# jannerm/ddpo

Hardware: AMD Instinct MI355X
Metric: sampled images/sec (512^2, 50 DDIM steps) (higher is better)
Workload: dtype f32 (f16mx: f16 MFMA + MX-fp8 cross terms on the long-reduction conv/GEMM layers, bf16x3-split MFMA elsewhere); 1 GPU; BASELINE configs[1]: compressed-animals geometry, sd15 U-Net+VAE (random init), 512x512, 50 DDIM steps, CFG 5.0, eta 1.0, sample_batch_size 8/GPU, VAE decode included; parallelism=dp1, global_batch=8

## Files before the change

### ddpo_amd/csrc/common.h

```cpp
#pragma once
#include <hip/hip_runtime.h>
#include <stdint.h>
#include "../../include/ddpo_hip.h"

#define DDPO_LAUNCH_CHECK()                                   \
  do {                                                        \
    hipError_t e__ = hipGetLastError();                       \
    if (e__ != hipSuccess) return DDPO_ELAUNCH;               \
  } while (0)

__device__ __forceinline__ float wave_sum(float v) {
#pragma unroll
  for (int o = 32; o > 0; o >>= 1) v += __shfl_xor(v, o, 64);
  return v;
}
__device__ __forceinline__ uint32_t lane_xor1_u32(uint32_t x) { return __shfl_xor(x, 1, 64); }
__device__ __forceinline__ double wave_sum_d(double v) {
#pragma unroll
  for (int o = 32; o > 0; o >>= 1) v += __shfl_xor(v, o, 64);
  return v;
}
__device__ __forceinline__ float wave_max(float v) {
#pragma unroll
  for (int o = 32; o > 0; o >>= 1) v = fmaxf(v, __shfl_xor(v, o, 64));
// ... 13 lines not shown

__device__ __forceinline__ float silu_f(float x) { return x / (1.f + __expf(-x)); }

__device__ __forceinline__ float sigmoid_2u_fast(float u) { return __builtin_amdgcn_rcpf(1.0f + __builtin_amdgcn_exp2f(-2.8853900817779268f * u)); }
__device__ __forceinline__ float gelu_tanh_f(float x) {
  const float k0 = 0.7978845608028654f, k1 = 0.044715f;
  float u = k0 * (x + k1 * x * x * x);
  return x * sigmoid_2u_fast(u);
}

__device__ __forceinline__ uint32_t cvt_pk_bf16(float lo, float hi) {
  uint32_t r;
  asm("v_cvt_pk_bf16_f32 %0, %1, %2" : "=v"(r) : "v"(lo), "v"(hi));
  return r;
}

__device__ __forceinline__ void split4(const float4 v, uint2& hi, uint2& lo) {
  hi.x = cvt_pk_bf16(v.x, v.y);
  hi.y = cvt_pk_bf16(v.z, v.w);
  const float r0 = v.x - __uint_as_float(hi.x << 16), r1 = v.y - __uint_as_float(hi.x & 0xFFFF0000u);
  const float r2 = v.z - __uint_as_float(hi.y << 16), r3 = v.w - __uint_as_float(hi.y & 0xFFFF0000u);
  lo.x = cvt_pk_bf16(r0, r1);
  lo.y = cvt_pk_bf16(r2, r3);
}

__host__ __device__ __forceinline__ int64_t plane_off(int64_t row, int c, int ld, int64_t rows) {
  return ld ? row * ld + c : ((int64_t)(c >> 5) * rows + row) * 32 + (c & 31);
}

typedef _Float16 mx_half2 __attribute__((ext_vector_type(2)));
__device__ __forceinline__ void mx_split4(const float4 v, uint2& h16, uint32_t& h8, uint32_t& l8) {
  const float lim = 65504.f, lim8 = 57344.f;
  const float vx = fminf(fmaxf(v.x, -lim), lim), vy = fminf(fmaxf(v.y, -lim), lim), vz = fminf(fmaxf(v.z, -lim), lim), vw = fminf(fmaxf(v.w, -lim), lim);
  const _Float16 a = (_Float16)vx, b = (_Float16)vy, c = (_Float16)vz, e = (_Float16)vw;
  h16.x = __builtin_bit_cast(uint32_t, mx_half2{a, b});
  h16.y = __builtin_bit_cast(uint32_t, mx_half2{c, e});
  const float ha = (float)a, hb = (float)b, hc = (float)c, he = (float)e;
  int p = __builtin_amdgcn_cvt_pk_bf8_f32(fminf(fmaxf(ha, -lim8), lim8), fminf(fmaxf(hb, -lim8), lim8), 0, false);
  h8 = (uint32_t)__builtin_amdgcn_cvt_pk_bf8_f32(fminf(fmaxf(hc, -lim8), lim8), fminf(fmaxf(he, -lim8), lim8), p, true);
  p = __builtin_amdgcn_cvt_pk_bf8_f32((vx - ha) * 2048.f, (vy - hb) * 2048.f, 0, false);
  l8 = (uint32_t)__builtin_amdgcn_cvt_pk_bf8_f32((vz - hc) * 2048.f, (vw - he) * 2048.f, p, true);
}
__device__ __forceinline__ void mx_store4(uint16_t* __restrict__ p16, uint16_t* __restrict__ p8, int64_t row, int c, int ld, int64_t rows,
                                          const float4 v) {
  uint2 h16;
  uint32_t h8, l8;
  mx_split4(v, h16, h8, l8);
  *reinterpret_cast<uint2*>(p16 + plane_off(row, c, ld, rows)) = h16;
  char* b = reinterpret_cast<char*>(p8 + plane_off(row, c & ~31, ld, rows)) + 2 * (c & 16) + (c & 15);
  *reinterpret_cast<uint32_t*>(b) = h8;
  *reinterpret_cast<uint32_t*>(b + 16) = l8;
}

static inline hipStream_t as_stream(void* s) { return reinterpret_cast<hipStream_t>(s); }
```

### ddpo_amd/csrc/gemm_bf16.hip

```cpp
#include "gemm_bf16_common.h"
#include <cstdlib>
#include <type_traits>

#ifdef DDPO_KLOOP_TIMING
__device__ unsigned long long ddpo_dbg_t[2 * 16384 * 8];
#define DBG_T(i)                                                                                      \
  do {                                                                                                \
    if (threadIdx.x == 0) {                                                                           \
      const int w_ = (blockIdx.x + gridDim.x * blockIdx.y) & 16383;                                   \
      ddpo_dbg_t[w_ * 8 + (i)] = __builtin_amdgcn_s_memtime();                                        \
      ddpo_dbg_t[w_ * 8 + 4 + (i)] = __builtin_amdgcn_s_memrealtime();                                \
    }                                                                                                 \
  } while (0)
#define DBG_ABL(bit) ((d.splits >> 4) & (bit))
#define DBG_WDECL unsigned long long dbg_w0_ = 0, dbg_wacc_ = 0, dbg_bacc_ = 0
#define DBG_W0() do { dbg_w0_ = __builtin_amdgcn_s_memtime(); } while (0)
#define DBG_WMID() do { const unsigned long long n_ = __builtin_amdgcn_s_memtime(); dbg_wacc_ += n_ - dbg_w0_; dbg_w0_ = n_; } while (0)
#define DBG_W1() do { dbg_bacc_ += __builtin_amdgcn_s_memtime() - dbg_w0_; } while (0)
#define DBG_WSTORE()                                                                 \
  do {                                                                               \
    if (threadIdx.x == 0) {                                                          \
      const int w_ = (blockIdx.x + gridDim.x * blockIdx.y) & 16383;                  \
      ddpo_dbg_t[(16384 + w_) * 8 + 0] = dbg_wacc_;                                  \
      ddpo_dbg_t[(16384 + w_) * 8 + 1] = dbg_bacc_;                                  \
// ... 105 lines not shown
      const int rowc = min(row_base + rr, d.M - 1) % d.res_rows, colc = min(col_base + (e - rr * LPR) * 4, d.N - 4);
      ex[i] = *reinterpret_cast<const float4*>(d.residual + (int64_t)rowc * d.ld_res + colc);
    }
  }
  __device__ __forceinline__ void combine(const ddpo_gemm_desc& d, float* cw, int b0, int row_base, int col_base, int lane) {
    const bool both = d.residual && d.rowbias;
    asm volatile("" : "+v"(lane));
#pragma unroll
    for (int i = 0; i < NB; ++i) {
      const int it = b0 + i;
      const int e = it * 64 + lane, rr = e / LPR, lcol = (e - rr * LPR) * 4;
      float4 v = *reinterpret_cast<const float4*>(cw + rr * WTN + lcol);
      const float4 b4 = bv[it % PER];
      v.x = d.alpha * v.x + b4.x; v.y = d.alpha * v.y + b4.y; v.z = d.alpha * v.z + b4.z; v.w = d.alpha * v.w + b4.w;
      if (both) {
        const int rowc = min(row_base + rr, d.M - 1), colc = min(col_base + lcol, d.N - 4);
        const float4 rb = *reinterpret_cast<const float4*>(d.rowbias + (int64_t)(rowc / d.rows_per_batch) * d.ld_rowbias + colc);
        v.x += rb.x; v.y += rb.y; v.z += rb.z; v.w += rb.w;
      }
      if (d.residual || d.rowbias) { v.x += ex[i].x; v.y += ex[i].y; v.z += ex[i].z; v.w += ex[i].w; }
      *reinterpret_cast<float4*>(cw + rr * WTN + lcol) = v;
    }
  }
  __device__ __forceinline__ void combine_all(const ddpo_gemm_desc& d, float* cw, int row_base, int col_base, int lane) {
    if (!any) return;
#pragma unroll
    for (int b0 = 0; b0 < NIT; b0 += NB) {
      if (b0) fetch(d, b0, row_base, col_base, lane);
      combine(d, cw, b0, row_base, col_base, lane);
    }
  }
  template <bool FOLD = false>
  __device__ __forceinline__ static void emit(const ddpo_gemm_desc& d, const float* cw, int row_base, int col_base, int lane, int ph = 0) {
#pragma unroll
    for (int b0 = 0; b0 < NIT; b0 += LB) {
      asm volatile("" : "+v"(lane));
      float4 v[LB];
#pragma unroll
      for (int i = 0; i < LB; ++i) {
        const int e = (b0 + i) * 64 + lane, rr = e / LPR;
        v[i] = *reinterpret_cast<const float4*>(cw + rr * WTN + (e - rr * LPR) * 4);
      }
#pragma unroll
      for (int i = 0; i < LB; ++i) {
        const int e = (b0 + i) * 64 + lane, rr = e / LPR;
        const int row = row_base + rr, col = col_base + (e - rr * LPR) * 4;
        if (row >= d.M || col >= d.N) continue;
        if constexpr (FOLD) { st_out4(d.out + fold_row(d, row, ph) * d.ld_out + col, v[i]); continue; }
        if (d.out) st_out4(d.out + (int64_t)row * d.ld_out + col, v[i]);
        if (d.out_hi) store_planes4(d, row, col, v[i]);
      }
    }
  }
  __device__ __forceinline__ static void partials(const ddpo_gemm_desc& d, const float* cw, float* pp, int row_base, int col_base, int lane) {
#pragma unroll
    for (int it = 0; it < NIT; ++it) {
      const int e = it * 64 + lane, rr = e / LPR, lcol = (e - rr * LPR) * 4;
      const int row = row_base + rr, col = col_base + lcol;
      if (row >= d.M || col >= d.N) continue;
      *reinterpret_cast<float4*>(pp + (int64_t)row * d.N + col) = *reinterpret_cast<const float4*>(cw + rr * WTN + lcol);
    }
  }
};

template <int BM, int BN, Datapath DP, bool AFFINE>
__global__ void __launch_bounds__(BF_THREADS) gemm_conv_bf16_kernel(const ddpo_gemm_desc d, const uint16_t* __restrict__ w_hi,
                                                                   const uint16_t* __restrict__ w_lo, int ldw, int tiles_m,
                                                                   int tiles_n, int nblk, int kt_per_split,
                                                                   float* __restrict__ part) {
  constexpr int BK = BF_BK;
  constexpr int TM = BM / 64, TN = BN / 64;
  constexpr int AROWS = BM / 32;
  constexpr int BCH = BN / 64;
  constexpr int NPL = (DP == Datapath::bf16x3) ? 2 : 1;
  constexpr int A_BYTES = BM * 64, B_BYTES = BN * 64;
  extern __shared__ __attribute__((aligned(16))) char smem[];
  constexpr int STAGE = NPL * (A_BYTES + B_BYTES);
  const int t = threadIdx.x, lane = t & 63, wid = t >> 6;
  const int wm = wid >> 1, wn = wid & 1;

  int bid = blockIdx.x;
  {
    const int xcd = bid & 7, idx = bid >> 3;
    const int q = nblk >> 3, r = nblk & 7;
    bid = (xcd < r ? xcd * (q + 1) : r * (q + 1) + (xcd - r) * q) + idx;
  }
  constexpr int GROUP_M = 8;
  const int per_group = GROUP_M * tiles_n;
  const int group = bid / per_group, in_group = bid - group * per_group;
  const int gm0 = group * GROUP_M;
  const int gsz = min(tiles_m - gm0, GROUP_M);
  const int tile_n = in_group / gsz, tile_m = gm0 + (in_group - tile_n * gsz);
  const int m0 = tile_m * BM, n0 = tile_n * BN;

  const bool conv = d.ksize > 0;
  const int VH = d.upsample ? d.H * 2 : d.H, VW = d.upsample ? d.W * 2 : d.W;
  const bool zins = d.upsample == 2;

  const int kq = t & 7;
  const float* arow_ptr[AROWS];
  uint32_t amask[AROWS];
  int aiy0[AROWS], aix0[AROWS];
  int64_t abase[AROWS];
#pragma unroll
  for (int i = 0; i < AROWS; ++i) {
    const int m = m0 + (t >> 3) + 32 * i;
    const bool valid = m < d.M;
    amask[i] = 0;
    if (conv) {
      const int ohw = d.OH * d.OW;
      const int mm = valid ? m : 0;
      const int b = mm / ohw, rem = mm - b * ohw;
      const int oy = rem / d.OW, ox = rem - oy * d.OW;
      const int iy0 = oy * d.stride - d.pad, ix0 = ox * d.stride - d.pad;
      abase[i] = (int64_t)b * d.H * d.W;
      aiy0[i] = iy0; aix0[i] = ix0;
// ... 159 lines not shown
  store_tile(0, s0);
  load_tile(1, s0);
  __syncthreads();
  const int nk2 = (nk + 1) & ~1;
#pragma unroll 1
  for (int kt = 0; kt < nk2; kt += 2) {
    load_tile(kt + 2, s1);
    compute(0);
    store_tile(1, s0);
    __syncthreads();
    load_tile(kt + 3, s0);
    compute(1);
    store_tile(0, s1);
    __syncthreads();
  }

  if (part) {
    float* pp = part + (int64_t)blockIdx.y * d.M * d.N;
#pragma unroll
    for (int i = 0; i < TM; ++i)
#pragma unroll
      for (int j = 0; j < TN; ++j) {
        const int col = n0 + wn * (BN / 2) + j * 32 + (lane & 31);
        if (col >= d.N) continue;
#pragma unroll
        for (int r = 0; r < 16; ++r) {
          const int row = m0 + wm * (BM / 2) + i * 32 + (r & 3) + 8 * (r >> 2) + 4 * khalf;
          if (row < d.M) pp[(int64_t)row * d.N + col] = acc[i][j][r];
        }
      }
    return;
  }
#pragma unroll
  for (int i = 0; i < TM; ++i) {
#pragma unroll
    for (int j = 0; j < TN; ++j) {
      const int col = n0 + wn * (BN / 2) + j * 32 + (lane & 31);
      if (col >= d.N) continue;
      const float bv = d.bias ? d.bias[col] : 0.f;
#pragma unroll
      for (int r = 0; r < 16; ++r) {
        const int row = m0 + wm * (BM / 2) + i * 32 + (r & 3) + 8 * (r >> 2) + 4 * khalf;
        if (row >= d.M) continue;
        float v = d.alpha * acc[i][j][r] + bv;
        if (d.rowbias) v += d.rowbias[(int64_t)(row / d.rows_per_batch) * d.ld_rowbias + col];
        if (d.residual) v += d.residual[(int64_t)res_row(d, row) * d.ld_res + col];
        d.out[(int64_t)row * d.ld_out + col] = v;
      }
    }
  }
}

template <int BM, int BN, Datapath DP, int WM = 2, int WN = 2, KLoop KL = KLoop::regs, bool FOLD = false>
__global__ void __launch_bounds__(64 * WM * WN, (BM * BN <= 128 * 64 ? 3 : 1)) gemm_conv_bf16_buf_kernel(const ddpo_gemm_desc d, const uint16_t* __restrict__ w_hi_,
                                                                       const uint16_t* __restrict__ w_lo_, int ldw, int tiles_m,
                                                                       int tiles_n, int nblk, int kt_per_split,
                                                                       float* __restrict__ part) {
  constexpr int BK = BF_BK;
  constexpr int THREADS = 64 * WM * WN;
  constexpr int WTM = BM / WM, WTN = BN / WN;
  constexpr int TM = WTM / 32, TN = WTN / 32;
  constexpr int AR = THREADS / 8, BR = THREADS / 4;
  constexpr int AROWS = BM / AR;
  constexpr int BCH = (BN + BR - 1) / BR;
  constexpr bool BFULL = (BN % BR) == 0;
  static_assert(BM % AR == 0 && WTM % 32 == 0 && WTN % 32 == 0, "tile / wave-grid mismatch");
  constexpr bool MX = DP == Datapath::f16mx;
  static_assert(!MX || KL == KLoop::planes3w || KL == KLoop::tall_mx, "the f16mx datapath exists on the plane-fed 128-row tiles and on the tall tile");
  static_assert(!FOLD || (KL != KLoop::regs && KL != KLoop::tall_geglu), "folded up-sampler phases exist on the plane-fed kernels");
  const int ph = FOLD ? (int)blockIdx.z : 0;
  const uint16_t* __restrict__ w_hi = FOLD ? w_hi_ + (int64_t)ph * d.K * d.N : w_hi_;
  const uint16_t* __restrict__ w_lo = (FOLD && w_lo_) ? w_lo_ + (int64_t)ph * d.K * d.N : w_lo_;
  constexpr int NPL = (DP == Datapath::bf16x3 || DP == Datapath::f16mx) ? 2 : 1;
  constexpr int A_BYTES = BM * 64, B_BYTES = BN * 64;
  extern __shared__ __attribute__((aligned(16))) char smem[];
  constexpr int STAGE = NPL * (A_BYTES + B_BYTES);
  const int t = threadIdx.x, lane = t & 63, wid = t >> 6;
  const int wm = wid / WN, wn = wid % WN;
  DBG_T(0);
  DBG_WDECL;

  int bid = blockIdx.x;
  {
    const int xcd = bid & 7, idx = bid >> 3;
    const int q = nblk >> 3, r = nblk & 7;
    bid = (xcd < r ? xcd * (q + 1) : r * (q + 1) + (xcd - r) * q) + idx;
  }
  constexpr int GROUP_M = 8;
  const int per_group = GROUP_M * tiles_n;
  const int group = bid / per_group, in_group = bid - group * per_group;
  const int gm0 = group * GROUP_M;
  const int gsz = min(tiles_m - gm0, GROUP_M);
  const int tile_n = in_group / gsz, tile_m = gm0 + (in_group - tile_n * gsz);
  const int m0 = tile_m * BM, n0 = tile_n * BN;

  const bool conv = d.ksize > 0;
  const int VH = (!FOLD && d.upsample) ? d.H * 2 : d.H, VW = (!FOLD && d.upsample) ? d.W * 2 : d.W;
  const bool zins = !FOLD && d.upsample == 2;
  const int cin = conv ? d.Cin : d.K;
  const int ntaps = conv ? d.ksize * d.ksize : 1;

  f32x16 acc[TM][TN];
#pragma unroll
  for (int i = 0; i < TM; ++i)
#pragma unroll
    for (int j = 0; j < TN; ++j)
#pragma unroll
// ... 569 lines not shown
      constexpr int LPR = WTN / 4;
      constexpr int NIT = 32 * LPR / 64;
      static_assert((32 * LPR) % 64 == 0, "32-row pass must be a whole number of wave instructions");
      __syncthreads();
      float* cw = reinterpret_cast<float*>(smem) + wid * (32 * WTN);
      float* pp = part ? part + ((int64_t)ph * gridDim.y + blockIdx.y) * d.M * d.N : nullptr;
      using Epi = EpiRows<NIT, LPR, WTN, 5>;
      Epi ep;
      const int colb = n0 + wn * WTN;
      static_assert(TM == 2, "the tall tile's output stage is written for two 32-row passes per wave");
      if constexpr (KL == KLoop::tall_geglu) {
        static_assert(WN == 2 && WTN == 160, "value / gate wave pairs of 160 columns");
        const int oc0 = (n0 / 320) * 160;
        float bj[TN];
#pragma unroll
        for (int j = 0; j < TN; ++j) bj[j] = d.bias ? d.bias[colb + j * 32 + (lane & 31)] : 0.f;
        const float* ca = reinterpret_cast<const float*>(smem) + (wid & ~1) * (32 * WTN);
        const float* cg = ca + 32 * WTN;
        auto gpass = [&](auto IH) {
          constexpr int ih = decltype(IH)::value;
          if (ih > 0) __syncthreads();
#pragma unroll
          for (int j = 0; j < TN; ++j)
#pragma unroll
            for (int r = 0; r < 16; ++r) {
              cw[((r & 3) + 8 * (r >> 2) + 4 * khalf) * WTN + j * 32 + (lane & 31)] = acc[ih][j][r] + bj[j];
            }
          __syncthreads();
          constexpr int GL = WTN / 4;
          int ln = lane;
          asm volatile("" : "+v"(ln));
#pragma unroll
          for (int it = 0; it < 16 * GL / 64; ++it) {
            const int e = it * 64 + ln, rr = wn * 16 + e / GL, c4 = (e - (e / GL) * GL) * 4;
            const float4 a = *reinterpret_cast<const float4*>(ca + rr * WTN + c4);
            const float4 g = *reinterpret_cast<const float4*>(cg + rr * WTN + c4);
            const float4 o = make_float4(a.x * gelu_tanh_f(g.x), a.y * gelu_tanh_f(g.y), a.z * gelu_tanh_f(g.z), a.w * gelu_tanh_f(g.w));
            const int row = m0 + wm * WTM + ih * 32 + rr, col = oc0 + c4;
            if (row >= d.M) continue;
            if (d.aux_out) {
              float* pa = d.aux_out + (int64_t)row * d.N + col;
              *reinterpret_cast<float4*>(pa) = a;
              *reinterpret_cast<float4*>(pa + (d.N >> 1)) = g;
            }
            if (d.out) st_out4(d.out + (int64_t)row * d.ld_out + col, o);
            if (d.out_hi) store_planes4(d, row, col, o);
          }
        };
        gpass(std::integral_constant<int, 0>{});
        gpass(std::integral_constant<int, 1>{});
        DBG_T(3);
        return;
      }
      auto pass = [&](auto IH) {
        constexpr int ih = decltype(IH)::value;
        const int rowb = m0 + wm * WTM + ih * 32;
        if (ih > 0 && !pp) ep.fetch(d, 0, rowb, colb, lane);
#pragma unroll
        for (int j = 0; j < TN; ++j)
#pragma unroll
          for (int r = 0; r < 16; ++r)
            cw[((r & 3) + 8 * (r >> 2) + 4 * khalf) * WTN + j * 32 + (lane & 31)] = acc[ih][j][r];
        if (pp) {
          Epi::partials(d, cw, pp, rowb, colb, lane);
        } else {
          if (ih == 0) { ep.init(d, colb, lane); ep.fetch(d, 0, rowb, colb, lane); }
          ep.combine_all(d, cw, rowb, colb, lane);
          Epi::template emit<FOLD>(d, cw, rowb, colb, lane, ph);
        }
      };
      pass(std::integral_constant<int, 0>{});
      pass(std::integral_constant<int, 1>{});
      DBG_T(3);
      return;
    }
  }
  if (vec_ok && BM != 256) {
    constexpr int LPR = WTN / 4;
    constexpr int NIT = WTM * LPR / 64;
    static_assert((WTM * LPR) % 64 == 0, "wave sub-tile must be a whole number of 1 KiB rows");
    __syncthreads();
    float* cw = reinterpret_cast<float*>(smem) + wid * (WTM * WTN);
    using Epi = EpiRows<NIT, LPR, WTN>;
    Epi ep;
    const int rowb = m0 + wm * WTM, colb = n0 + wn * WTN;
    const bool plain = !part && !(BN == 128 && WN == 2 && WM == 2 && d.epilogue == 1);
    if (plain) { ep.init(d, colb, lane); ep.fetch(d, 0, rowb, colb, lane); }
#pragma unroll
    for (int i = 0; i < TM; ++i)
#pragma unroll
      for (int j = 0; j < TN; ++j)
#pragma unroll
        for (int r = 0; r < 16; ++r)
          cw[(i * 32 + (r & 3) + 8 * (r >> 2) + 4 * khalf) * WTN + j * 32 + (lane & 31)] = acc[i][j][r];
    if (BN == 128 && WN == 2 && WM == 2 && d.epilogue == 1) {
      const int q = (n0 + wn * 64) >> 6;
      const int gc = (lane & 7) * 4, grow = lane >> 3;
      const float4 ba = d.bias ? *reinterpret_cast<const float4*>(d.bias + q * 64 + gc) : make_float4(0.f, 0.f, 0.f, 0.f);
      const float4 bg = d.bias ? *reinterpret_cast<const float4*>(d.bias + q * 64 + 32 + gc) : make_float4(0.f, 0.f, 0.f, 0.f);
#pragma unroll
      for (int it = 0; it < 8; ++it) {
        const int rr = it * 8 + grow;
        const int row = m0 + wm * 64 + rr;
        if (row >= d.M) continue;
        const float4 a = *reinterpret_cast<const float4*>(cw + rr * 64 + gc);
        const float4 g = *reinterpret_cast<const float4*>(cw + rr * 64 + 32 + gc);
        float4 o;
        o.x = (a.x + ba.x) * gelu_tanh_f(g.x + bg.x); o.y = (a.y + ba.y) * gelu_tanh_f(g.y + bg.y);
        o.z = (a.z + ba.z) * gelu_tanh_f(g.z + bg.z); o.w = (a.w + ba.w) * gelu_tanh_f(g.w + bg.w);
        if (d.aux_out) {
          float* pa = d.aux_out + (int64_t)row * d.N + q * 32 + gc;
          *reinterpret_cast<float4*>(pa) = make_float4(a.x + ba.x, a.y + ba.y, a.z + ba.z, a.w + ba.w);
          *reinterpret_cast<float4*>(pa + (d.N >> 1)) = make_float4(g.x + bg.x, g.y + bg.y, g.z + bg.z, g.w + bg.w);
        }
        if (d.out) st_out4(d.out + (int64_t)row * d.ld_out + q * 32 + gc, o);
        if (d.out_hi) store_planes4(d, row, q * 32 + gc, o);
      }
      DBG_T(3);
      return;
    }
    if (part) {
      Epi::partials(d, cw, part + ((int64_t)ph * gridDim.y + blockIdx.y) * d.M * d.N, rowb, colb, lane);
    } else {
      ep.combine_all(d, cw, rowb, colb, lane);
      Epi::template emit<FOLD>(d, cw, rowb, colb, lane, ph);
    }
    DBG_T(3);
    return;
  }
  if (part) {
    float* pp = part + ((int64_t)ph * gridDim.y + blockIdx.y) * d.M * d.N;
#pragma unroll
    for (int i = 0; i < TM; ++i)
#pragma unroll
      for (int j = 0; j < TN; ++j) {
        const int col = n0 + wn * WTN + j * 32 + (lane & 31);
        if (col >= d.N) continue;
#pragma unroll
        for (int r = 0; r < 16; ++r) {
          const int row = m0 + wm * WTM + i * 32 + (r & 3) + 8 * (r >> 2) + 4 * khalf;
          if (row < d.M) pp[(int64_t)row * d.N + col] = acc[i][j][r];
        }
      }
    DBG_T(3);
    return;
  }
#pragma unroll
  for (int i = 0; i < TM; ++i) {
#pragma unroll
    for (int j = 0; j < TN; ++j) {
      const int col = n0 + wn * WTN + j * 32 + (lane & 31);
      if (col >= d.N) continue;
      const float bv = d.bias ? d.bias[col] : 0.f;
#pragma unroll
      for (int r = 0; r < 16; ++r) {
        const int row = m0 + wm * WTM + i * 32 + (r & 3) + 8 * (r >> 2) + 4 * khalf;
        if (row >= d.M) continue;
        float v = d.alpha * acc[i][j][r] + bv;
        if (d.rowbias) v += d.rowbias[(int64_t)(row / d.rows_per_batch) * d.ld_rowbias + col];
        if (d.residual) v += d.residual[(int64_t)res_row(d, row) * d.ld_res + col];
        d.out[(FOLD ? fold_row(d, row, ph) : (int64_t)row) * d.ld_out + col] = v;
      }
    }
  }
  DBG_T(3);
}

__global__ void __launch_bounds__(256) splitk_reduce_kernel(const ddpo_gemm_desc d, const float* __restrict__ part, int splits) {
  const int n4 = d.N >> 2;
  const int64_t total = (int64_t)d.M * n4, mn = (int64_t)d.M * d.N;
  const bool fold = d.upsample == 3;
  const int ph = blockIdx.y;
  part += (int64_t)ph * splits * mn;
  for (int64_t i = (int64_t)blockIdx.x * blockDim.x + threadIdx.x; i < total; i += (int64_t)gridDim.x * blockDim.x) {
    const int row = (int)(i / n4), col = (int)(i - (int64_t)row * n4) << 2;
    float4 a = *reinterpret_cast<const float4*>(part + (int64_t)row * d.N + col);
    for (int s = 1; s < splits; ++s) {
      const float4 b = *reinterpret_cast<const float4*>(part + s * mn + (int64_t)row * d.N + col);
      a.x += b.x; a.y += b.y; a.z += b.z; a.w += b.w;
    }
    float v[4] = {a.x, a.y, a.z, a.w};
    const int rrow = res_row(d, row);
#pragma unroll
    for (int e = 0; e < 4; ++e) {
      float x = d.alpha * v[e] + (d.bias ? d.bias[col + e] : 0.f);
      if (d.rowbias) x += d.rowbias[(int64_t)(row / d.rows_per_batch) * d.ld_rowbias + col + e];
      if (d.residual) x += d.residual[(int64_t)rrow * d.ld_res + col + e];
      v[e] = x;
      if (d.out) d.out[(fold ? fold_row(d, row, ph) : (int64_t)row) * d.ld_out + col + e] = x;
    }
    if (d.out_hi) store_planes4(d, row, col, make_float4(v[0], v[1], v[2], v[3]));
  }
}

constexpr int SPLITK_MIN_KTILES_128 = 32;
constexpr int SPLITK_MIN_KTILES_WIDE = 16;
extern "C" int ddpo_gemm_splitk_min_ktiles(void) { return SPLITK_MIN_KTILES_WIDE < SPLITK_MIN_KTILES_128 ? SPLITK_MIN_KTILES_WIDE : SPLITK_MIN_KTILES_128; }

static bool res_rows_ok(const ddpo_gemm_desc& d) {
  return d.res_rows == 0 || (d.res_rows > 0 && d.residual && d.M > 0 && d.M % d.res_rows == 0);
}

static bool planes_out_ok(const ddpo_gemm_desc& d) {
  if (!d.out_hi) return d.out != nullptr && !d.out_lo;
  if (!d.out_lo || d.ld_planes < 0 || (d.ld_planes & 3)) return false;
  if ((reinterpret_cast<uintptr_t>(d.out_hi) | reinterpret_cast<uintptr_t>(d.out_lo)) & 7) return false;
  const int ncols = d.epilogue != 0 ? d.N / 2 : d.N;
  if (d.ld_planes == 0 ? (ncols & 31) != 0 : d.ld_planes < ncols) return false;
  if (d.planes_fmt != 0 && (d.planes_fmt != 1 || (ncols & 31) || (d.ld_planes & 31))) return false;
  if (d.N & 3) return false;
  if (d.out && ((d.ld_out & 3) || (reinterpret_cast<uintptr_t>(d.out) & 15))) return false;
  if (d.residual && ((d.ld_res & 3) || (reinterpret_cast<uintptr_t>(d.residual) & 15))) return false;
  if (d.rowbias && ((d.ld_rowbias & 3) || (reinterpret_cast<uintptr_t>(d.rowbias) & 15))) return false;
  if (d.bias && (reinterpret_cast<uintptr_t>(d.bias) & 15)) return false;
  return true;
}

enum { TC_TALL = 0, TC_WIDE = 1, TC_128 = 2, TC_64 = 3, TC_GENERIC = 4, TC_SPLITK_REDUCE = 5, TC_MX = 6, TC_COUNT = 8 };
static unsigned long long g_tile_launches[TC_COUNT] = {0, 0, 0, 0, 0, 0, 0, 0};
extern "C" int ddpo_gemm_tile_launch_counts(unsigned long long* out_host, int n) {
  if (!out_host || n < TC_COUNT) return DDPO_EINVAL;
  for (int i = 0; i < TC_COUNT; ++i) out_host[i] = __atomic_load_n(&g_tile_launches[i], __ATOMIC_RELAXED);
  return DDPO_OK;
}
static inline void count_tile(int cls) { __atomic_fetch_add(&g_tile_launches[cls], 1ull, __ATOMIC_RELAXED); }

static bool g_force_generic = false;
static bool buf_path_ok(const ddpo_gemm_desc& d, int ldw) {
  if (g_force_generic) return false;
  const int64_t lim = 0x7FFFFFFF;
  if (d.w_layout == 1) ldw = (d.K + 31) / 32 * 32;
  if (d.ksize > 0) {
    if (d.Cin % BF_BK) return false;
    if ((int64_t)d.B * d.H * d.W * (d.ld_src ? d.ld_src : d.Cin) * 4 >= lim) return false;
    const int64_t wbytes = d.w_dgrad ? (int64_t)d.K * d.N * 2 : (int64_t)d.N * ldw * 2;
    if (wbytes >= lim) return false;
  } else {
    if (d.K % BF_BK) return false;
    if ((int64_t)d.M * (d.ld_src ? d.ld_src : d.K) * 4 >= lim || (int64_t)d.N * ldw * 2 >= lim) return false;
  }
  return true;
}
#ifdef DDPO_DEBUG_HOOKS
extern "C" void ddpo_debug_force_generic_gemm(int on) { g_force_generic = on != 0; }
#endif

template <int BM_, int BN_, int WM_, int WN_, int TC_, size_t EPI_BYTES_, bool SPLITK_>
struct Tile {
  static constexpr int BM = BM_, BN = BN_, WM = WM_, WN = WN_, TC = TC_;
  static constexpr bool SPLITK = SPLITK_;
  static constexpr size_t lds_bytes(Datapath dp, KLoop kl) {
    const size_t npl = (dp == Datapath::bf16x3 || dp == Datapath::f16mx) ? 2 : 1;
    const size_t stages = kl == KLoop::planes3w ? npl * (2 * BM + 3 * BN) * 64 : 2 * npl * (BM + BN) * 64;
    return stages < EPI_BYTES_ ? EPI_BYTES_ : stages;
  }
};
using Tile128x128 = Tile<128, 128, 2, 2, TC_128, 128 * 128 * 4, true>;
using Tile128x64 = Tile<128, 64, 2, 2, TC_64, 128 * 64 * 4, true>;
using TileWide = Tile<128, 320, 4, 2, TC_WIDE, 128 * 320 * 4, true>;
using TileTall = Tile<256, 320, 4, 2, TC_TALL, 8 * 32 * 160 * 4, false>;

template <class T, Datapath DP, KLoop KL, bool FOLD>
constexpr bool kernel_exists() {
  if (FOLD && (DP == Datapath::f16x1 || KL == KLoop::regs || KL == KLoop::tall_geglu)) return false;
  if (T::BM == 256) {
    if (DP == Datapath::bf16x3) return KL == KLoop::tall || KL == KLoop::tall_geglu;
    return KL == (DP == Datapath::f16mx ? KLoop::tall_mx : KLoop::tall_ring);
  }
  return KL == KLoop::planes3w || (KL == KLoop::regs && (DP == Datapath::bf16x1 || DP == Datapath::bf16x3));
}

static int splits_128(const ddpo_gemm_desc& d, int ngrid, bool have_ws, size_t ws_bytes, int nph) {
  const int nk_total = (d.K + BF_BK - 1) / BF_BK;
  int splits = 1;
  if (have_ws && ngrid < 192 && nk_total >= SPLITK_MIN_KTILES_128 && (d.N & 3) == 0 && d.epilogue == 0) {
    splits = (384 + ngrid - 1) / ngrid;
    if (splits > 8) splits = 8;
    if (splits > nk_total / 8) splits = nk_total / 8;
    while (splits > 1 && (size_t)nph * splits * d.M * d.N * sizeof(float) > ws_bytes) --splits;
  }
  return splits;
}
static int wide_splits(const ddpo_gemm_desc& d, bool have_ws, size_t ws_bytes, int nph = 1) {
  const int nblk = nph * ((d.M + 127) / 128) * ((d.N + 319) / 320);
  const int nk_total = d.K / BF_BK;
  int splits = 1;
  if (have_ws && nblk <= 192 && nk_total >= SPLITK_MIN_KTILES_WIDE) {
    splits = (256 + nblk / 2) / nblk;
    if (splits > 8) splits = 8;
    if (splits > nk_total / 8) splits = nk_total / 8;
    if (splits < 1) splits = 1;
    while (splits > 1 && (size_t)nph * splits * d.M * d.N * sizeof(float) > ws_bytes) --splits;
  }
  return splits;
}
static int ktiles_per_split(int nk_total, int& splits) {
  int ktps = (nk_total + splits - 1) / splits;
  ktps = (ktps + 1) & ~1;
  splits = (nk_total + ktps - 1) / ktps;
  return ktps;
}

static int launch_splitk_reduce(const ddpo_gemm_desc& d, const float* part, int splits, int nph, hipStream_t st) {
  int64_t blocks = ((int64_t)d.M * (d.N >> 2) + 255) / 256;
  if (blocks > 4096) blocks = 4096;
  count_tile(TC_SPLITK_REDUCE);
  hipLaunchKernelGGL(splitk_reduce_kernel, dim3((int)blocks, nph), dim3(256), 0, st, d, part, splits);
  DDPO_LAUNCH_CHECK();
  return DDPO_OK;
}

template <class T, Datapath DP, KLoop KL, bool FOLD>
static int launch_tile(const ddpo_gemm_desc& d, const uint16_t* w_hi, const uint16_t* w_lo, int ldw, float* ws, int splits, hipStream_t st) {
  if constexpr (!kernel_exists<T, DP, KL, FOLD>()) {
    return DDPO_EINVAL;
  } else {
    constexpr int NPH = FOLD ? 4 : 1;
    constexpr bool GENERIC = KL == KLoop::regs && T::BN <= 128;
    constexpr size_t lds = T::lds_bytes(DP, KL);
    const auto kernel = &gemm_conv_bf16_buf_kernel<T::BM, T::BN, DP, T::WM, T::WN, KL, FOLD>;
    const int tiles_m = (d.M + T::BM - 1) / T::BM, tiles_n = (d.N + T::BN - 1) / T::BN;
    const int nblk = tiles_m * tiles_n;
    const int nk_total = (d.K + BF_BK - 1) / BF_BK;
    if (!T::SPLITK) splits = 1;
    const int ktps = T::SPLITK ? ktiles_per_split(nk_total, splits) : nk_total;
    float* part = splits > 1 ? ws : nullptr;
    static bool attr_set = false;
    if (!attr_set) {
      if constexpr (GENERIC) {
        (void)hipFuncSetAttribute(reinterpret_cast<const void*>(&gemm_conv_bf16_kernel<T::BM, T::BN, DP, true>), hipFuncAttributeMaxDynamicSharedMemorySize, (int)lds);
        (void)hipFuncSetAttribute(reinterpret_cast<const void*>(&gemm_conv_bf16_kernel<T::BM, T::BN, DP, false>), hipFuncAttributeMaxDynamicSharedMemorySize, (int)lds);
      }
      (void)hipFuncSetAttribute(reinterpret_cast<const void*>(kernel), hipFuncAttributeMaxDynamicSharedMemorySize, (int)lds);
      attr_set = true;
    }
    count_tile(T::TC);
    if constexpr (DP == Datapath::f16mx) count_tile(TC_MX);
    bool generic = false;
    if constexpr (GENERIC) generic = !buf_path_ok(d, ldw);
    if (!generic) {
      hipLaunchKernelGGL(kernel, dim3(nblk, splits, NPH), dim3(64 * T::WM * T::WN), lds, st, d, w_hi, w_lo, ldw, tiles_m, tiles_n, nblk, ktps, part);
    } else if constexpr (GENERIC) {
      count_tile(TC_GENERIC);
      if (d.upsample == 0)
        hipLaunchKernelGGL((gemm_conv_bf16_kernel<T::BM, T::BN, DP, true>), dim3(nblk, splits), dim3(BF_THREADS), lds, st, d, w_hi, w_lo, ldw, tiles_m, tiles_n, nblk, ktps, part);
      else
        hipLaunchKernelGGL((gemm_conv_bf16_kernel<T::BM, T::BN, DP, false>), dim3(nblk, splits), dim3(BF_THREADS), lds, st, d, w_hi, w_lo, ldw, tiles_m, tiles_n, nblk, ktps, part);
    }
    DDPO_LAUNCH_CHECK();
    return splits > 1 ? launch_splitk_reduce(d, part, splits, NPH, st) : DDPO_OK;
  }
}

enum RouteTile { RT_TALL, RT_TALL_GEGLU, RT_WIDE, RT_128, RT_64 };
struct Route { RouteTile tile; int splits; };

template <bool PLANES, bool FOLD, Datapath DP>
static int launch_route(const Route& r, const ddpo_gemm_desc& d, const uint16_t* w_hi, const uint16_t* w_lo, int ldw, float* ws, hipStream_t st) {
  constexpr KLoop KL = PLANES ? KLoop::planes3w : KLoop::regs;
  constexpr KLoop KT = !PLANES ? KLoop::regs : (DP == Datapath::bf16x3 ? KLoop::tall : (DP == Datapath::f16mx ? KLoop::tall_mx : KLoop::tall_ring));
  switch (r.tile) {
    case RT_TALL: return launch_tile<TileTall, DP, KT, FOLD>(d, w_hi, w_lo, ldw, ws, r.splits, st);
    case RT_TALL_GEGLU: return launch_tile<TileTall, DP, PLANES && DP == Datapath::bf16x3 ? KLoop::tall_geglu : KLoop::regs, FOLD>(d, w_hi, w_lo, ldw, ws, r.splits, st);
    case RT_WIDE: return launch_tile<TileWide, DP, KL, FOLD>(d, w_hi, w_lo, ldw, ws, r.splits, st);
    case RT_128: return launch_tile<Tile128x128, DP, KL, FOLD>(d, w_hi, w_lo, ldw, ws, r.splits, st);
    default: return launch_tile<Tile128x64, DP, KL, FOLD>(d, w_hi, w_lo, ldw, ws, r.splits, st);
  }
}
template <bool PLANES, bool FOLD>
static int launch_npass(int npass, const Route& r, const ddpo_gemm_desc& d, const uint16_t* w_hi, const uint16_t* w_lo, int ldw, float* ws, hipStream_t st) {
  switch (npass) {
    case 1: return launch_route<PLANES, FOLD, Datapath::bf16x1>(r, d, w_hi, w_lo, ldw, ws, st);
    case 3: return launch_route<PLANES, FOLD, Datapath::bf16x3>(r, d, w_hi, w_lo, ldw, ws, st);
    case 4: return launch_route<PLANES, FOLD, Datapath::f16mx>(r, d, w_hi, w_lo, ldw, ws, st);
    case 5: return launch_route<PLANES, FOLD, Datapath::f16x1>(r, d, w_hi, w_lo, ldw, ws, st);
    default: return DDPO_EINVAL;
  }
}

template <bool PLANES, bool FOLD = false>
static int dispatch_bf16(const ddpo_gemm_desc& d, const uint16_t* w_hi, const uint16_t* w_lo, int ldw, int npass, void* ws, size_t ws_bytes,
                         hipStream_t st) {
  static_assert(!FOLD || PLANES, "folded up-sampler phases exist on the plane-fed kernels");
  constexpr int NPH = FOLD ? 4 : 1;
  if (FOLD && (d.epilogue != 0 || (npass != 1 && npass != 3 && npass != 4))) return DDPO_EINVAL;
  if (d.epilogue != 0) {
    if ((d.epilogue != 1 && d.epilogue != 2) || (d.N & 127) || !buf_path_ok(d, ldw) || d.rowbias || d.residual || d.alpha != 1.0f || d.w_dgrad) return DDPO_EINVAL;
    if ((d.ld_out & 3) || (reinterpret_cast<uintptr_t>(d.out) & 15) || (d.bias && (reinterpret_cast<uintptr_t>(d.bias) & 15))) return DDPO_EINVAL;
    if (reinterpret_cast<uintptr_t>(d.aux_out) & 15) return DDPO_EINVAL;
    if (d.epilogue == 2 && (!PLANES || npass != 3 || d.N % 320 || ((d.N >> 1) & 3))) return DDPO_EINVAL;
    return launch_npass<PLANES, FOLD>(npass, Route{d.epilogue == 2 ? RT_TALL_GEGLU : RT_128, 1}, d, w_hi, w_lo, ldw, nullptr, st);
  }
  float* wsf = (ws && !(reinterpret_cast<uintptr_t>(ws) & 15)) ? reinterpret_cast<float*>(ws) : nullptr;
  Route r;
  const long ntall = (long)NPH * ((d.M + 255) / 256) * (d.N / 320), nwide = (long)NPH * ((d.M + 127) / 128) * (d.N / 320);
  const double eff_tall = (double)ntall / (double)(((ntall + 255) / 256) * 256), eff_wide = (double)nwide / (double)(((nwide + 255) / 256) * 256);
  bool tall = PLANES && d.N % 320 == 0 && ntall >= 200 && eff_tall * 1.08 >= eff_wide;
  if (tall && npass == 4) {
    const char* mx_tall_env = getenv("DDPO_MX_TALL");
    tall = !(mx_tall_env && mx_tall_env[0] == '0');
  }
  const int wsplits = wide_splits(d, wsf != nullptr, ws_bytes, NPH);
  if (tall) {
    r = Route{RT_TALL, 1};
  } else if (d.N % 320 == 0 && (long)NPH * d.M >= 512 && buf_path_ok(d, ldw) && !(d.K / BF_BK < 16 && d.N > 1280) &&
             (long)NPH * ((d.M + 127) / 128) * (d.N / 320) * wsplits >= 200 &&
             !(wsplits > 1 && d.K / BF_BK < 64)) {
    r = Route{RT_WIDE, wsplits};
  } else {
    const long t128 = (long)NPH * ((d.M + 127) / 128) * ((d.N + 127) / 128);
    const bool mid_short = t128 < 512 && d.K / BF_BK <= 64;
    const bool big = (d.N % 128 == 0) && t128 >= 256 && !mid_short;
    const int ngrid = NPH * ((d.M + 127) / 128) * ((d.N + (big ? 127 : 63)) / (big ? 128 : 64));
    r = Route{big ? RT_128 : RT_64, splits_128(d, ngrid, wsf != nullptr, ws_bytes, NPH)};
  }
  return launch_npass<PLANES, FOLD>(npass, r, d, w_hi, w_lo, ldw, wsf, st);
}

static bool conv_geometry_ok(const ddpo_gemm_desc& d) {
  if (d.M <= 0 || d.N <= 0 || d.K <= 0 || !planes_out_ok(d) || !res_rows_ok(d)) return false;
  if (d.ksize > 0) {
    if (d.ksize != 1 && d.ksize != 3) return false;
    if (d.K != d.ksize * d.ksize * d.Cin || d.M != d.B * d.OH * d.OW || d.upsample < 0 || d.upsample > 2) return false;
  }
  return true;
}

extern "C" int ddpo_gemm_conv_fwd_bf16(const ddpo_gemm_desc* dp, const uint16_t* w_hi, const uint16_t* w_lo, int ldw, int npass,
                                       void* ws, size_t ws_bytes, void* stream) {
  if (!dp || !w_hi) return DDPO_EINVAL;
  const ddpo_gemm_desc& d = *dp;
  if (npass != 1 && npass != 3) return DDPO_EINVAL;
  if (npass == 3 && !w_lo) return DDPO_EINVAL;
  if (!d.src || d.ld_src <= 0 || (d.ld_src & 3) || (reinterpret_cast<uintptr_t>(d.src) & 15)) return DDPO_EINVAL;
  if ((reinterpret_cast<uintptr_t>(w_hi) & 15) || (w_lo && (reinterpret_cast<uintptr_t>(w_lo) & 15))) return DDPO_EINVAL;
  if (!conv_geometry_ok(d) || (d.out_hi && !buf_path_ok(d, ldw))) return DDPO_EINVAL;
  if ((d.ksize > 0 ? d.Cin : d.K) & 7) return DDPO_EINVAL;
  if (d.w_layout != 0 && (d.w_layout != 1 || d.w_dgrad)) return DDPO_EINVAL;
  if (d.w_dgrad) {
    if (d.ksize <= 0) return DDPO_EINVAL;
  } else if (d.w_layout == 0 && (ldw < d.K || (ldw & 7))) {
    return DDPO_EINVAL;
  }
  return dispatch_bf16<false>(d, w_hi, w_lo, ldw, npass, ws, ws_bytes, as_stream(stream));
}

static bool plane_operands_ok(ddpo_gemm_desc& d, const uint16_t* a0, const uint16_t* a1, int lda, int lda_mult, const uint16_t* w0, const uint16_t* w1, int ldw) {
  if (!a0 || !w0 || (a1 == nullptr) != (w1 == nullptr)) return false;
  if ((reinterpret_cast<uintptr_t>(a0) | reinterpret_cast<uintptr_t>(a1) | reinterpret_cast<uintptr_t>(w0) | reinterpret_cast<uintptr_t>(w1)) & 15) return false;
  if (lda < 0 || (lda & (lda_mult - 1)) || (lda && lda < (d.ksize > 0 ? d.Cin : d.K))) return false;
  d.src = reinterpret_cast<const float*>(a0);
  d.w = reinterpret_cast<const float*>(a1);
  d.ld_src = lda;
  d.splits = 1;
  return buf_path_ok(d, ldw);
}

extern "C" int ddpo_gemm_conv_fwd_bf16_planes(const ddpo_gemm_desc* dp, const uint16_t* a_hi, const uint16_t* a_lo, int lda,
                                              const uint16_t* w_hi, const uint16_t* w_lo, int ldw, void* ws, size_t ws_bytes,
                                              void* stream) {
  if (!dp) return DDPO_EINVAL;
  const int npass = a_lo ? 3 : 1;
  ddpo_gemm_desc d = *dp;
  if (!conv_geometry_ok(d) || d.w_dgrad || (d.w_layout != 0 && d.w_layout != 1)) return DDPO_EINVAL;
  if (d.w_layout == 0 && (ldw < d.K || (ldw & 7))) return DDPO_EINVAL;
  if (npass == 1 && d.epilogue == 2) return DDPO_EINVAL;
  if (!plane_operands_ok(d, a_hi, a_lo, lda, 8, w_hi, w_lo, ldw)) return DDPO_EINVAL;
  dbg_abl_from_env(d);
  return dispatch_bf16<true>(d, w_hi, w_lo, ldw, npass, ws, ws_bytes, as_stream(stream));
}

extern "C" int ddpo_gemm_conv_fwd_f16mx_planes(const ddpo_gemm_desc* dp, const uint16_t* a16, const uint16_t* a8, int lda,
                                               const uint16_t* w16, const uint16_t* w8, void* ws, size_t ws_bytes, void* stream) {
  if (!dp || (a8 && !dp->w_scale)) return DDPO_EINVAL;
  const int npass = a8 ? 4 : 5;
  ddpo_gemm_desc d = *dp;
  if (!conv_geometry_ok(d) || d.w_dgrad || d.w_layout != 1) return DDPO_EINVAL;
  if (npass == 5 && d.epilogue == 2) return DDPO_EINVAL;
  if (!plane_operands_ok(d, a16, a8, lda, 32, w16, w8, 0)) return DDPO_EINVAL;
  dbg_abl_from_env(d);
  return dispatch_bf16<true>(d, w16, w8, 0, npass, ws, ws_bytes, as_stream(stream));
}

extern "C" int ddpo_conv_up2x_folded_fwd(const ddpo_gemm_desc* dp, const uint16_t* a_hi, const uint16_t* a_lo, int lda, const uint16_t* w_hi,
                                         const uint16_t* w_lo, int f16mx, void* ws, size_t ws_bytes, void* stream) {
  if (!dp) return DDPO_EINVAL;
  if (f16mx && (!a_lo || !dp->w_scale)) return DDPO_EINVAL;
  const int npass = f16mx ? 4 : (a_lo ? 3 : 1);
  ddpo_gemm_desc d = *dp;
  if (d.B <= 0 || d.H <= 0 || d.W <= 0 || d.Cin <= 0 || d.N <= 0 || (d.Cin % BF_BK) || (d.N & 3)) return DDPO_EINVAL;
  if ((int64_t)d.B * d.H * d.W * 4 > 0x7FFFFFFF || (int64_t)d.Cin * 4 > 0x7FFFFFFF) return DDPO_EINVAL;
  if (!d.out || d.out_hi || d.out_lo || d.rowbias || d.residual || d.res_rows || d.epilogue || d.w_dgrad || d.aux_out) return DDPO_EINVAL;
  if (d.ld_out < d.N || (d.ld_out & 3) || (reinterpret_cast<uintptr_t>(d.out) & 15) || (d.bias && (reinterpret_cast<uintptr_t>(d.bias) & 15))) return DDPO_EINVAL;
  d.M = d.B * d.H * d.W; d.K = 4 * d.Cin;
  d.alpha = 1.0f;
  d.OH = d.H; d.OW = d.W;
  d.ksize = 2; d.stride = 1; d.pad = 1; d.upsample = 3;
  d.w_layout = 1; d.planes_fmt = 0; d.ld_planes = 0;
  if (!f16mx) d.w_scale = nullptr;
  if (!plane_operands_ok(d, a_hi, a_lo, lda, f16mx ? 32 : 8, w_hi, w_lo, 0) || (int64_t)4 * d.K * d.N * 2 >= 0x7FFFFFFF) return DDPO_EINVAL;
  return dispatch_bf16<true, true>(d, w_hi, w_lo, 0, npass, ws, ws_bytes, as_stream(stream));
}
```

### ddpo_amd/csrc/norm.hip

```cpp
#include "common.h"

#define GN_THREADS 256
#define GN_MAXCOL 4
#define GN_MAXC 4096
#define GN_MAXG 64
#define GN_PPB 32

__global__ void __launch_bounds__(GN_THREADS) gn_stats_kernel(const float* __restrict__ x, int ldx, int HW, int C, int G,
                                                              int pix_per_block, double* __restrict__ part) {
  __shared__ float s_sum[GN_MAXC], s_sq[GN_MAXC];
  const int b = blockIdx.y;
  const int C4 = C >> 2;
  const int cpg = C / G;
  const int t = threadIdx.x;
  const int p0 = blockIdx.x * pix_per_block;
  const int p1 = min(p0 + pix_per_block, HW);
  float sum[GN_MAXCOL][4], sq[GN_MAXCOL][4];
#pragma unroll
  for (int j = 0; j < GN_MAXCOL; ++j)
#pragma unroll
    for (int e = 0; e < 4; ++e) { sum[j][e] = 0.f; sq[j][e] = 0.f; }
  int ppi, col0, poff, ncol;
  if (C4 <= GN_THREADS) {
    ppi = GN_THREADS / C4;
// ... 150 lines not shown
  if (var < 0.0) var = 0.0;
  const float rstd = (float)(1.0 / sqrt(var + (double)eps));
  const float meanf = (float)mean;
  if (t == 0) { mr[2 * (b * G + g)] = meanf; mr[2 * (b * G + g) + 1] = rstd; }
  if (!lane_on) return;
  const float4 gm = *reinterpret_cast<const float4*>(gamma + c);
  const float4 bt = *reinterpret_cast<const float4*>(beta + c);
  const float kx = rstd * gm.x, ky = rstd * gm.y, kz = rstd * gm.z, kw = rstd * gm.w;
  const float sx = bt.x - meanf * kx, sy = bt.y - meanf * ky, sz = bt.z - meanf * kz, sw = bt.w - meanf * kw;
  if (ps == 0) {
    float* o = ab + 2 * ((int64_t)b * C + c);
    *reinterpret_cast<float4*>(o) = make_float4(kx, sx, ky, sy);
    *reinterpret_cast<float4*>(o + 4) = make_float4(kz, sz, kw, sw);
  }
#pragma unroll
  for (int i = 0; i < GNF_MAXP; ++i) {
    const int p = ps + i * pps;
    if (p >= HW) continue;
    const int64_t row = (int64_t)b * HW + p;
    float4 o;
    o.x = v[i].x * kx + sx; o.y = v[i].y * ky + sy; o.z = v[i].z * kz + sz; o.w = v[i].w * kw + sw;
    if (SILU) { o.x = silu_f(o.x); o.y = silu_f(o.y); o.z = silu_f(o.z); o.w = silu_f(o.w); }
    if (MODE == 2) {
      mx_store4(y_hi, y_lo, row, c, ldy, rows_total, o);
    } else if (MODE == 1) {
      uint2 h, l;
      split4(o, h, l);
      *reinterpret_cast<uint2*>(y_hi + plane_off(row, c, ldy, rows_total)) = h;
      *reinterpret_cast<uint2*>(y_lo + plane_off(row, c, ldy, rows_total)) = l;
    } else {
      *reinterpret_cast<float4*>(y + row * ldy + c) = o;
    }
  }
}
static inline bool gn_fused_small_ok(int HW, int C, int G) {
  const int cpg = C / G;
  return HW <= 256 && (cpg & 3) == 0 && cpg <= 4 * GNF_MAXQ && (C & 3) == 0;
}

static inline int gn_ppb(int C) {
  const int C4 = C >> 2;
  const int ppi = C4 <= GN_THREADS ? GN_THREADS / C4 : 1;
  int ppb = GN_PPB < ppi ? ppi : GN_PPB;
  return ((ppb + ppi - 1) / ppi) * ppi;
}

extern "C" size_t ddpo_groupnorm_ws_bytes(int B, int HW, int C, int G) {
  if (B <= 0 || HW <= 0 || C <= 0 || G <= 0) return 0;
  const int chunks = (HW + gn_ppb(C) - 1) / gn_ppb(C);
  return (size_t)B * chunks * G * 2 * sizeof(double);
}
extern "C" size_t ddpo_groupnorm_stats_floats(int B, int C, int G) { return (size_t)B * C * 2 + (size_t)B * G * 2; }

static int groupnorm_fwd_impl(const float* x, int ldx, float* y, uint16_t* y_hi, uint16_t* y_lo, int ldy, const float* gamma,
                              const float* beta, int B, int HW, int C, int G, float eps, int fuse_silu, void* ws, float* stats,
                              void* stream) {
  const bool planes = y == nullptr;
  const bool mx = (fuse_silu & 2) != 0;
  fuse_silu &= 1;
  if (mx && (!planes || (C & 31) || (ldy & 31))) return DDPO_EINVAL;
  if (!x || !gamma || !beta || !ws || !stats || B <= 0 || HW <= 0 || C <= 0 || G <= 0 || G > GN_MAXG) return DDPO_EINVAL;
  if (planes ? (!y_hi || !y_lo) : false) return DDPO_EINVAL;
  if ((C & 3) || (C % G) || (ldx & 3) || (ldy & 3) || C > GN_MAXC || B > 65535) return DDPO_EINVAL;
  if (ldy == 0 && (!planes || (C & 31))) return DDPO_EINVAL;
  if ((reinterpret_cast<uintptr_t>(x) | reinterpret_cast<uintptr_t>(ws) | reinterpret_cast<uintptr_t>(stats)) & 15) return DDPO_EINVAL;
  if (planes ? ((reinterpret_cast<uintptr_t>(y_hi) | reinterpret_cast<uintptr_t>(y_lo)) & 7) != 0 : (reinterpret_cast<uintptr_t>(y) & 15) != 0)
    return DDPO_EINVAL;
  hipStream_t st = as_stream(stream);
  const int C4 = C >> 2;
  const int ppb = gn_ppb(C);
  const int chunks = (HW + ppb - 1) / ppb;
  double* part = reinterpret_cast<double*>(ws);
  float* ab = stats;
  float* mr = stats + (size_t)B * C * 2;
  if (gn_fused_small_ok(HW, C, G) && ((reinterpret_cast<uintptr_t>(gamma) | reinterpret_cast<uintptr_t>(beta)) & 15) == 0) {
    const dim3 grid(G, B), blk(256);
    const int64_t rt = (int64_t)B * HW;
    const int mode = planes ? (mx ? 2 : 1) : 0;
#define GNF_LAUNCH(S, M) hipLaunchKernelGGL((gn_fused_small_kernel<S, M>), grid, blk, 0, st, x, ldx, y, y_hi, y_lo, ldy, gamma, beta, ab, mr, HW, C, G, eps, rt)
    if (fuse_silu) { if (mode == 0) GNF_LAUNCH(true, 0); else if (mode == 1) GNF_LAUNCH(true, 1); else GNF_LAUNCH(true, 2); }
    else { if (mode == 0) GNF_LAUNCH(false, 0); else if (mode == 1) GNF_LAUNCH(false, 1); else GNF_LAUNCH(false, 2); }
#undef GNF_LAUNCH
    DDPO_LAUNCH_CHECK();
    return DDPO_OK;
  }
  hipLaunchKernelGGL(gn_stats_kernel, dim3(chunks, B), dim3(GN_THREADS), 0, st, x, ldx, HW, C, G, ppb, part);
  DDPO_LAUNCH_CHECK();
  hipLaunchKernelGGL(gn_finalize_kernel, dim3(B * G), dim3(64), 0, st, part, gamma, beta, ab, mr, chunks, C, G, HW, eps);
  DDPO_LAUNCH_CHECK();
  int64_t blocks = ((int64_t)B * HW * C4 + 255) / 256;
  if (blocks > 16384) blocks = 16384;
  uint16_t* const no = nullptr;
  if (planes) {
    const int pair = mx ? 2 : ((C & 7) == 0 && (ldy & 7) == 0 &&
                                ((reinterpret_cast<uintptr_t>(y_hi) | reinterpret_cast<uintptr_t>(y_lo)) & 15) == 0) ? 1 : 0;
    if (fuse_silu)
      hipLaunchKernelGGL((gn_apply_kernel<true, true>), dim3((int)blocks), dim3(256), 0, st, x, ldx, y, ldy, ab, B, HW, C, y_hi, y_lo, pair);
    else
      hipLaunchKernelGGL((gn_apply_kernel<false, true>), dim3((int)blocks), dim3(256), 0, st, x, ldx, y, ldy, ab, B, HW, C, y_hi, y_lo, pair);
  } else if (fuse_silu) {
    hipLaunchKernelGGL((gn_apply_kernel<true, false>), dim3((int)blocks), dim3(256), 0, st, x, ldx, y, ldy, ab, B, HW, C, no, no, 0);
  } else {
    hipLaunchKernelGGL((gn_apply_kernel<false, false>), dim3((int)blocks), dim3(256), 0, st, x, ldx, y, ldy, ab, B, HW, C, no, no, 0);
  }
  DDPO_LAUNCH_CHECK();
  return DDPO_OK;
}

extern "C" int ddpo_groupnorm_fwd(const float* x, int ldx, float* y, int ldy, const float* gamma, const float* beta, int B,
                                  int HW, int C, int G, float eps, int fuse_silu, void* ws, float* stats, void* stream) {
  if (!y) return DDPO_EINVAL;
  return groupnorm_fwd_impl(x, ldx, y, nullptr, nullptr, ldy, gamma, beta, B, HW, C, G, eps, fuse_silu, ws, stats, stream);
}

extern "C" int ddpo_groupnorm_fwd_planes(const float* x, int ldx, uint16_t* y_hi, uint16_t* y_lo, int ldy, const float* gamma,
                                         const float* beta, int B, int HW, int C, int G, float eps, int fuse_silu, void* ws,
                                         float* stats, void* stream) {
  if (!y_hi || !y_lo) return DDPO_EINVAL;
  return groupnorm_fwd_impl(x, ldx, nullptr, y_hi, y_lo, ldy, gamma, beta, B, HW, C, G, eps, fuse_silu, ws, stats, stream);
}

#define LN_MAXV 10
#define LN_RPW 4
template <bool PL, int NV>
__device__ __forceinline__ void ln_row(const float4 (&v)[NV], int lane, int C4, int C, float eps, int64_t row, int64_t rows, float* __restrict__ y,
                                       const float* __restrict__ gamma, const float* __restrict__ beta, uint16_t* __restrict__ y_hi,
                                       uint16_t* __restrict__ y_lo, int pair, int ldy) {
  float s = 0.f;
#pragma unroll
  for (int j = 0; j < NV; ++j) {
    const int c4 = lane + j * 64;
    if (c4 < C4) s += (v[j].x + v[j].y) + (v[j].z + v[j].w);
  }
  const float mean = wave_sum(s) / (float)C;
  float q = 0.f;
#pragma unroll
  for (int j = 0; j < NV; ++j) {
    const int c4 = lane + j * 64;
    if (c4 < C4) {
      const float a = v[j].x - mean, b = v[j].y - mean, c = v[j].z - mean, d = v[j].w - mean;
      q += (a * a + b * b) + (c * c + d * d);
    }
  }
  const float rstd = rsqrtf(wave_sum(q) / (float)C + eps);
  float* yr = PL ? nullptr : y + row * C;
#pragma unroll
  for (int j = 0; j < NV; ++j) {
    const int c4 = lane + j * 64;
    if (c4 < C4) {
      const float4 g = *reinterpret_cast<const float4*>(gamma + (c4 << 2));
      const float4 bt = *reinterpret_cast<const float4*>(beta + (c4 << 2));
      float4 o;
      o.x = (v[j].x - mean) * rstd * g.x + bt.x;
      o.y = (v[j].y - mean) * rstd * g.y + bt.y;
      o.z = (v[j].z - mean) * rstd * g.z + bt.z;
      o.w = (v[j].w - mean) * rstd * g.w + bt.w;
      if (PL && pair == 2) {
        mx_store4(y_hi, y_lo, row, c4 << 2, ldy, rows, o);
      } else if (PL) {
        uint2 h, l;
        split4(o, h, l);
        if (pair) {
          const bool odd = lane & 1;
          const uint32_t rx = lane_xor1_u32(odd ? h.x : l.x), ry = lane_xor1_u32(odd ? h.y : l.y);
          if (!odd) *reinterpret_cast<uint4*>(y_hi + plane_off(row, c4 << 2, ldy, rows)) = make_uint4(h.x, h.y, rx, ry);
          else *reinterpret_cast<uint4*>(y_lo + plane_off(row, (c4 << 2) - 4, ldy, rows)) = make_uint4(rx, ry, l.x, l.y);
        } else {
          *reinterpret_cast<uint2*>(y_hi + plane_off(row, c4 << 2, ldy, rows)) = h;
          *reinterpret_cast<uint2*>(y_lo + plane_off(row, c4 << 2, ldy, rows)) = l;
        }
      } else {
        *reinterpret_cast<float4*>(yr + (c4 << 2)) = o;
// ... 171 lines not shown
```

### ddpo_amd/lib.py

```python
import contextlib
import ctypes
import functools
import math
import os
import threading
from ctypes import c_void_p, c_int, c_int32, c_int64, c_uint32, c_float, c_double, c_size_t, POINTER, byref

import torch

_HERE = os.path.dirname(os.path.abspath(__file__))
LIB_PATH = os.path.join(_HERE, "libddpo_hip.so")

PRED_TYPES = {"epsilon": 0, "v_prediction": 1, "sample": 2}


class LoraLayer(ctypes.Structure):
    _fields_ = [("w0", c_void_p), ("w", c_void_p), ("a", c_void_p), ("b", c_void_p), ("K", c_int), ("N", c_int), ("r", c_int), ("s", c_float)]


class DdimConsts(ctypes.Structure):
    _fields_ = [("alphas_cumprod", c_void_p), ("num_train_timesteps", c_int), ("step_ratio", c_int),
                ("final_alpha_cumprod", c_float), ("eta", c_float), ("pred_type", c_int)]


# ... 10 lines not shown
                ("B", c_int), ("H", c_int), ("W", c_int), ("Cin", c_int),
                ("OH", c_int), ("OW", c_int),
                ("w_dgrad", c_int), ("ld_w", c_int), ("splits", c_int), ("accumulate", c_int), ("epilogue", c_int),
                ("out_hi", c_void_p), ("out_lo", c_void_p), ("ld_planes", c_int), ("w_layout", c_int),
                ("w_scale", c_void_p), ("planes_fmt", c_int), ("colsum", c_void_p), ("aux_out", c_void_p), ("res_rows", c_int)]


ABI_VERSION = 14

_SIGS = {
    "ddpo_abi_version": (c_int, []),
    "ddpo_sizeof_gemm_desc": (c_size_t, []),
    "ddpo_sizeof_ddim_consts": (c_size_t, []),
    "ddpo_gemm_tile_launch_counts": (c_int, [c_void_p, c_int]),
    "ddpo_gemm_splitk_min_ktiles": (c_int, []),
    "ddpo_threefry_bits_host": (c_int, [c_uint32, c_uint32, c_int64, c_void_p]),
    "ddpo_threefry_normal": (c_int, [c_uint32, c_uint32, c_void_p, c_void_p, c_int64, c_void_p]),
    "ddpo_ddim_step_fwd": (c_int, [c_void_p, c_void_p, c_void_p, c_void_p, c_void_p, c_float, POINTER(DdimConsts),
                                   c_void_p, c_void_p, c_int, c_int, c_void_p]),
    "ddpo_ddim_logprob_ppo_fwd_bwd": (c_int, [c_void_p, c_void_p, c_void_p, c_void_p, c_void_p, c_void_p, c_void_p,
                                              c_float, c_float, c_int, POINTER(DdimConsts), c_void_p, c_void_p,
                                              c_void_p, c_void_p, c_int, c_int, c_void_p]),
    "ddpo_ddim_logprob_ppo_fwd_bwd_grouped": (c_int, [c_void_p, c_void_p, c_void_p, c_void_p, c_void_p, c_void_p, c_void_p,
                                                      c_float, c_float, c_int, POINTER(DdimConsts), c_void_p, c_void_p,
                                                      c_void_p, c_void_p, c_int, c_int, c_int, c_void_p]),
    "ddpo_rwr_noisy_latents": (c_int, [c_void_p, c_void_p, c_void_p, c_void_p, c_void_p, c_int, c_float, c_void_p, c_void_p, c_int, c_int, c_int,
                                       c_void_p]),
    "ddpo_rwr_mse_fwd_bwd": (c_int, [c_void_p, c_void_p, c_void_p, c_void_p, c_float, c_int, c_void_p, c_void_p, c_void_p, c_void_p, c_int, c_int,
                                     c_void_p]),
    "ddpo_grad_sqnorm": (c_int, [c_void_p, c_int64, c_void_p, c_int, c_void_p]),
    "ddpo_adamw_bf16mu_step": (c_int, [c_void_p, c_void_p, c_void_p, c_void_p, c_int64, c_void_p, c_double, c_double,
                                       c_double, c_double, c_double, c_double, c_double, c_int, c_int, c_int, c_void_p]),
    "ddpo_groupnorm_ws_bytes": (c_size_t, [c_int, c_int, c_int, c_int]),
    "ddpo_groupnorm_fwd": (c_int, [c_void_p, c_int, c_void_p, c_int, c_void_p, c_void_p, c_int, c_int, c_int, c_int,
                                   c_float, c_int, c_void_p, c_void_p, c_void_p]),
    "ddpo_layernorm_fwd": (c_int, [c_void_p, c_void_p, c_void_p, c_void_p, c_int, c_int, c_float, c_void_p]),
    "ddpo_gemm_conv_fwd": (c_int, [POINTER(GemmDesc), c_void_p]),
    "ddpo_gemm_conv_wgrad": (c_int, [POINTER(GemmDesc), c_void_p]),
    "ddpo_gemm_conv_fwd_bf16": (c_int, [POINTER(GemmDesc), c_void_p, c_void_p, c_int, c_int, c_void_p, c_size_t, c_void_p]),
    "ddpo_gemm_conv_wgrad_bf16x3": (c_int, [POINTER(GemmDesc), c_void_p]),
    "ddpo_gemm_conv_wgrad_bf16x3_planes": (c_int, [POINTER(GemmDesc), c_void_p, c_void_p, c_void_p, c_void_p, c_void_p]),
    "ddpo_gemm_conv_fwd_bf16_planes": (c_int, [POINTER(GemmDesc), c_void_p, c_void_p, c_int, c_void_p, c_void_p, c_int, c_void_p, c_size_t,
                                               c_void_p]),
    "ddpo_split_planes_bf16": (c_int, [c_void_p, c_int, c_void_p, c_void_p, c_int, c_int64, c_int, c_void_p]),
    "ddpo_groupnorm_fwd_planes": (c_int, [c_void_p, c_int, c_void_p, c_void_p, c_int, c_void_p, c_void_p, c_int, c_int, c_int, c_int,
                                          c_float, c_int, c_void_p, c_void_p, c_void_p]),
    "ddpo_layernorm_fwd_planes": (c_int, [c_void_p, c_void_p, c_void_p, c_void_p, c_void_p, c_int, c_int, c_float, c_int, c_void_p]),
    "ddpo_pack_weights_bf16": (c_int, [c_void_p, c_int, c_int, c_int, c_void_p, c_void_p, c_void_p, c_void_p, c_void_p]),
    "ddpo_pack_weights_bf16_kblocked": (c_int, [c_void_p, c_int, c_int, c_void_p, c_void_p, c_void_p]),
    "ddpo_pack_weights_bf16_kblocked_dgrad": (c_int, [c_void_p, c_int, c_int, c_int, c_void_p, c_void_p, c_void_p]),
    "ddpo_pack_weights_f16mx": (c_int, [c_void_p, c_int, c_int, c_void_p, c_void_p, c_void_p, c_void_p]),
    "ddpo_split_planes_f16mx": (c_int, [c_void_p, c_int, c_void_p, c_void_p, c_int, c_int64, c_int, c_void_p]),
    "ddpo_gemm_conv_fwd_f16mx_planes": (c_int, [POINTER(GemmDesc), c_void_p, c_void_p, c_int, c_void_p, c_void_p, c_void_p, c_size_t, c_void_p]),
    "ddpo_fold_up2x_weights": (c_int, [c_void_p, c_int, c_int, c_void_p, c_void_p]),
    "ddpo_conv_up2x_folded_fwd": (c_int, [POINTER(GemmDesc), c_void_p, c_void_p, c_int, c_void_p, c_void_p, c_int, c_void_p, c_size_t, c_void_p]),
    "ddpo_attention_fwd": (c_int, [c_void_p, c_int, c_void_p, c_int, c_void_p, c_int, c_void_p, c_int, c_void_p, c_int, c_int,
                                   c_int, c_int, c_int, c_float, c_void_p]),
    "ddpo_attention_kv_images_bytes": (c_size_t, [c_int, c_int, c_int, c_int]),
    "ddpo_attention_pack_kv_bf16x3": (c_int, [c_void_p, c_int, c_void_p, c_int, c_void_p, c_size_t, c_int, c_int, c_int, c_int, c_void_p]),
    "ddpo_attention_fwd_bf16x3_images": (c_int, [c_void_p, c_int, c_void_p, c_size_t, c_void_p, c_int, c_void_p, c_int, c_int, c_int, c_int, c_int,
                                                 c_float, c_void_p]),
    "ddpo_attention_fwd_bf16x3": (c_int, [c_void_p, c_int, c_void_p, c_int, c_void_p, c_int, c_void_p, c_int, c_void_p, c_int, c_int,
                                          c_int, c_int, c_int, c_float, c_void_p, c_size_t, c_void_p]),
    "ddpo_attention_fwd_bf16x3_ws_bytes": (c_size_t, [c_int, c_int, c_int, c_int]),
    "ddpo_attention_fwd_f16p": (c_int, [c_void_p, c_int, c_void_p, c_int, c_void_p, c_int, c_void_p, c_int, c_void_p, c_int, c_int,
                                        c_int, c_int, c_int, c_float, c_void_p, c_size_t, c_void_p]),
    "ddpo_attention_pack_kv_f16p": (c_int, [c_void_p, c_int, c_void_p, c_int, c_void_p, c_size_t, c_int, c_int, c_int, c_int, c_void_p]),
    "ddpo_attention_fwd_f16p_images": (c_int, [c_void_p, c_int, c_void_p, c_size_t, c_void_p, c_int, c_void_p, c_int, c_int, c_int, c_int, c_int,
                                               c_float, c_void_p]),
    **{f"ddpo_attention_fwd_{v}_po": (c_int, [c_void_p, c_int, c_void_p, c_int, c_void_p, c_int, c_void_p, c_void_p, c_int, c_void_p, c_int, c_int,
                                              c_int, c_int, c_int, c_float, c_void_p, c_size_t, c_void_p]) for v in ("bf16x3", "f16p")},
    **{f"ddpo_attention_fwd_{v}_images_po": (c_int, [c_void_p, c_int, c_void_p, c_size_t, c_void_p, c_void_p, c_int, c_void_p, c_int, c_int, c_int,
                                                     c_int, c_int, c_float, c_void_p]) for v in ("bf16x3", "f16p")},
    "ddpo_attention_fwd_shared_q": (c_int, [c_void_p, c_int, c_int, c_void_p, c_int, c_void_p, c_int, c_void_p, c_int, c_void_p, c_int, c_int,
                                            c_int, c_int, c_int, c_float, c_void_p]),
    "ddpo_attention_fwd_x16_shared_q": (c_int, [c_int, c_void_p, c_int, c_int, c_void_p, c_int, c_void_p, c_int, c_void_p, c_int, c_void_p, c_void_p,
                                                c_int, c_void_p, c_int, c_int, c_int, c_int, c_int, c_float, c_void_p, c_size_t, c_void_p]),
    "ddpo_attention_fwd_images_shared_q": (c_int, [c_int, c_void_p, c_int, c_int, c_void_p, c_size_t, c_void_p, c_int, c_void_p, c_void_p, c_int,
                                                   c_void_p, c_int, c_int, c_int, c_int, c_int, c_float, c_void_p]),
    "ddpo_attention_bwd_f16p": (c_int, [c_void_p, c_int, c_void_p, c_int, c_void_p, c_int, c_void_p, c_void_p, c_void_p, c_void_p,
                                        c_void_p, c_void_p, c_void_p, c_int, c_int, c_int, c_int, c_int, c_float, c_void_p]),
    "ddpo_attention_bwd": (c_int, [c_void_p, c_int, c_void_p, c_int, c_void_p, c_int, c_void_p, c_void_p, c_void_p, c_void_p,
                                   c_void_p, c_void_p, c_void_p, c_int, c_int, c_int, c_int, c_int, c_float, c_void_p]),
    "ddpo_attention_bwd_bf16x3": (c_int, [c_void_p, c_int, c_void_p, c_int, c_void_p, c_int, c_void_p, c_void_p, c_void_p, c_void_p,
                                          c_void_p, c_void_p, c_void_p, c_int, c_int, c_int, c_int, c_int, c_float, c_void_p]),
    "ddpo_groupnorm_stats_floats": (c_size_t, [c_int, c_int, c_int]),
    "ddpo_groupnorm_bwd_ws_bytes": (c_size_t, [c_int, c_int, c_int, c_int]),
    "ddpo_groupnorm_bwd": (c_int, [c_void_p, c_int, c_void_p, c_int, c_void_p, c_void_p, c_int, c_int, c_int, c_int, c_int,
                                   c_void_p, c_int, c_void_p, c_int, c_void_p, c_void_p, c_void_p, c_void_p]),
    "ddpo_layernorm_bwd": (c_int, [c_void_p, c_void_p, c_void_p, c_int, c_int, c_float, c_void_p, c_void_p, c_void_p, c_void_p, c_void_p, c_void_p]),
    "ddpo_layernorm_bwd_ws_bytes": (c_size_t, [c_int, c_int]),
    "ddpo_geglu_bwd": (c_int, [c_void_p, c_void_p, c_void_p, c_int64, c_int, c_void_p]),
    "ddpo_silu_bwd": (c_int, [c_void_p, c_void_p, c_void_p, c_int64, c_void_p]),
    "ddpo_colsum_accum": (c_int, [c_void_p, c_int, c_int64, c_int, c_int, c_void_p, c_void_p]),
    "ddpo_sumpool2x2": (c_int, [c_void_p, c_void_p, c_int, c_int, c_int, c_int, c_void_p]),
    "ddpo_add": (c_int, [c_void_p, c_void_p, c_void_p, c_int64, c_void_p]),
    "ddpo_geglu_fwd": (c_int, [c_void_p, c_void_p, c_int64, c_int, c_void_p]),
    "ddpo_silu_fwd": (c_int, [c_void_p, c_void_p, c_int64, c_void_p]),
    "ddpo_quick_gelu_fwd": (c_int, [c_void_p, c_void_p, c_int64, c_void_p]),
    "ddpo_l2_normalize_rows": (c_int, [c_void_p, c_void_p, c_int, c_int, c_void_p]),
    "ddpo_timestep_embedding": (c_int, [c_void_p, c_void_p, c_int, c_int, c_void_p]),
    "ddpo_nchw_to_nhwc": (c_int, [c_void_p, c_void_p, c_int, c_int, c_int, c_void_p]),
    "ddpo_nhwc_to_nchw": (c_int, [c_void_p, c_void_p, c_int, c_int, c_int, c_void_p]),
    "ddpo_copy_cols": (c_int, [c_void_p, c_int, c_void_p, c_int, c_int64, c_int, c_void_p]),
    "ddpo_stage_cfg_inputs": (c_int, [c_void_p, c_void_p, c_int64, c_void_p, c_void_p, c_int, c_void_p, c_void_p, c_int, c_void_p]),
    "ddpo_softmax_rows": (c_int, [c_void_p, c_int64, c_int, c_float, c_void_p]),
# ... 413 lines not shown
                      mu_decay_in_bf16=True, zero_grad=True):
    assert mu.dtype == torch.bfloat16 and nu.dtype == torch.float32 and sqnorm.dtype == torch.float64
    _check(load().ddpo_adamw_bf16mu_step(_p(p), _p(g), _p(mu), _p(nu), p.numel(), _p(sqnorm), float(inv_n_acc), float(lr),
                                         float(b1), float(b2), float(eps), float(weight_decay), float(max_grad_norm),
                                         int(step_t), int(mu_decay_in_bf16), int(zero_grad), _stream()), "ddpo_adamw_bf16mu_step")


_ws_cache = {}


def _scratch(nbytes, device, tag):
    key = (tag, str(device), torch.cuda.current_stream().cuda_stream)
    ws = _ws_cache.get(key)
    if ws is None or ws.numel() < nbytes:
        ws = torch.empty(max(int(nbytes), 1 << 20), dtype=torch.uint8, device=device)
        _ws_cache[key] = ws
    return ws


def _conv_geom(B, H, W, Cin, ksize, stride, pad, upsample):
    if pad is None:
        pad = ksize // 2
    VH, VW = (2 * H, 2 * W) if upsample else (H, W)
    OH = (VH + 2 * pad - ksize) // stride + 1
    OW = (VW + 2 * pad - ksize) // stride + 1
    return dict(ksize=ksize, stride=stride, pad=pad, upsample=int(upsample), B=B, H=H, W=W, Cin=Cin, OH=OH, OW=OW)


def _gemm_desc(M, N, K, *, conv=None, src=None, ld_src=0, out=None, ld_out=None, bias=None, residual=None, ld_res=None, res_rows=0, alpha=1.0,
               out_planes=None, aux_out=None, **fields):
    d = GemmDesc()
    d.M, d.N, d.K = int(M), int(N), int(K)
    d.alpha = float(alpha)
    for k, v in (conv or {}).items():
        setattr(d, k, int(v))
    if src is not None:
        d.src = src.data_ptr()
    d.ld_src = int(ld_src)
    if out is not None:
        d.out = out.data_ptr(); d.ld_out = int(ld_out if ld_out is not None else N)
    d.bias = bias.data_ptr() if bias is not None else None
    if residual is not None:
        d.residual = residual.data_ptr(); d.ld_res = int(ld_res if ld_res is not None else N)
    d.res_rows = int(res_rows)
    if out_planes is not None:
        hi, lo, d.ld_planes, d.planes_fmt = out_planes
        d.out_hi, d.out_lo = hi.data_ptr(), lo.data_ptr()
    d.aux_out = aux_out.data_ptr() if aux_out is not None else None
    for k, v in fields.items():
        setattr(d, k, v)
    return d


def _launch_fwd(d, act, weights, *, w_layout=0, cross=None, ws_device=None, tag=""):
    lib = load()
    a_hi, a_lo, a_ld = (act.hi, act.lo, act.ld) if isinstance(act, Planes) else (act or (None, None, 0))
    ws = None if ws_device is None else _scratch(SPLITK_WS_BYTES, ws_device, "splitk")
    ws_args = (_p(ws), SPLITK_WS_BYTES if ws is not None else 0, _stream())
    if weights is None:
        name, rc = "ddpo_gemm_conv_fwd", lib.ddpo_gemm_conv_fwd(byref(d), _stream())
    elif isinstance(weights, dict):
        cross = MX_CROSS if cross is None else cross
        d.w_layout = 1
        d.w_scale = weights["scale"].data_ptr()
        name, rc = "ddpo_gemm_conv_fwd_f16mx_planes", lib.ddpo_gemm_conv_fwd_f16mx_planes(
            byref(d), _p(a_hi), _p(a_lo) if cross else None, a_ld, _p(weights["w16"]), _p(weights["w8"]) if cross else None, *ws_args)
    else:
        hi, lo, ldw, npass = weights
        d.w_layout = w_layout
        if a_hi is None:
            name, rc = "ddpo_gemm_conv_fwd_bf16", lib.ddpo_gemm_conv_fwd_bf16(byref(d), _p(hi), _p(lo), ldw, npass, *ws_args)
        else:
            one = npass == 1
            name, rc = "ddpo_gemm_conv_fwd_bf16_planes", lib.ddpo_gemm_conv_fwd_bf16_planes(
                byref(d), _p(a_hi), None if one else _p(a_lo), a_ld, _p(hi), None if one else _p(lo), ldw, *ws_args)
    _check(rc, name + tag)


def _family(fp32=False, mx=False):
    return "fp32" if fp32 else ("f16mx" if mx else ("bf16x3" if _x3() else current_datapath()))


@contextlib.contextmanager
def _profiled(flops, io_bytes, family):
    if PROFILE is None:
        yield
        return
    e0, e1 = torch.cuda.Event(enable_timing=True), torch.cuda.Event(enable_timing=True)
    e0.record()
    yield
    e1.record()
    PROFILE.append((e0, e1, flops, family, io_bytes))


def groupnorm(x, B, HW, gamma, beta, groups, eps, silu, out=None, ld_x=None, ld_out=None, return_stats=False, planes=False):
    C = gamma.numel()
    if ld_x is None and x.dim() == 2 and x.stride(0) != C:
        ld_x = x.stride(0)
    if planes:
        pl = Planes(B * HW, C, x.device, fmt=1 if planes == 2 else 0)
        ws = _scratch(load().ddpo_groupnorm_ws_bytes(B, HW, C, groups), x.device, "gn")
        stats = torch.empty(load().ddpo_groupnorm_stats_floats(B, C, groups), dtype=torch.float32, device=x.device)
        _check(load().ddpo_groupnorm_fwd_planes(_pr(x, ld_x), int(ld_x or C), _p(pl.hi), _p(pl.lo), pl.ld, _p(gamma), _p(beta), B, HW, C, groups,
                                                float(eps), int(bool(silu)) | (2 * pl.fmt), _p(ws), _p(stats), _stream()), "ddpo_groupnorm_fwd_planes")
        return (pl, stats) if return_stats else pl
    if out is None:
        out = torch.empty(B * HW, C, dtype=torch.float32, device=x.device)
    ws = _scratch(load().ddpo_groupnorm_ws_bytes(B, HW, C, groups), x.device, "gn")
    stats = torch.empty(load().ddpo_groupnorm_stats_floats(B, C, groups), dtype=torch.float32, device=x.device)
    _check(load().ddpo_groupnorm_fwd(_pr(x, ld_x), int(ld_x or C), _p(out), int(ld_out or C), _p(gamma), _p(beta), B, HW, C, groups,
                                     float(eps), int(bool(silu)), _p(ws), _p(stats), _stream()), "ddpo_groupnorm_fwd")
    return (out, stats) if return_stats else out


def groupnorm_bwd(x, dy, stats, gamma, B, HW, groups, silu, dgamma, dbeta, dx_add=None, ld_x=None, ld_dy=None):
    C = gamma.numel()
    dx = torch.empty(B * HW, C, dtype=torch.float32, device=x.device)
    ws = _scratch(load().ddpo_groupnorm_bwd_ws_bytes(B, HW, C, groups), x.device, "gnb")
    _check(load().ddpo_groupnorm_bwd(_p(x), int(ld_x or C), _p(dy), int(ld_dy or C), _p(stats), _p(gamma), B, HW, C, groups,
                                     int(bool(silu)), _p(dx_add), C, _p(dx), C, _p(dgamma), _p(dbeta), _p(ws), _stream()),
           "ddpo_groupnorm_bwd")
    return dx


def layernorm(x, gamma, beta, eps=1e-5, out=None, planes=False):
    rows, C = x.shape
    if planes:
        pl = Planes(rows, C, x.device, fmt=1 if planes == 2 else 0)
        _check(load().ddpo_layernorm_fwd_planes(_p(x), _p(pl.hi), _p(pl.lo), _p(gamma), _p(beta), rows, C, float(eps), int(pl.kblocked) | (2 * pl.fmt), _stream()),
               "ddpo_layernorm_fwd_planes")
        return pl
    if out is None:
        out = torch.empty_like(x)
    _check(load().ddpo_layernorm_fwd(_p(x), _p(out), _p(gamma), _p(beta), rows, C, float(eps), _stream()), "ddpo_layernorm_fwd")
    return out


def pack_weights(w, bwd=True):
    N = w.shape[-1]
    K = w.numel() // N
    Kp = (K + 7) // 8 * 8
    ent = PACKED.get(w.data_ptr())
    mk = lambda *s: torch.zeros(*s, dtype=torch.int16, device=w.device)
    lay = 1 if (W_KBLOCKED and N % 4 == 0) else 0
    if lay:
        Kp = (K + 31) // 32 * 32
    if ent is None or ent["K"] != K or ent["N"] != N or ent.get("w_layout", 0) != lay:
        ent = dict(K=K, N=N, fwd=(mk(N, Kp), mk(N, Kp), Kp), bwd=None, w_layout=lay)
        PACKED[w.data_ptr()] = ent
    n_dg = w.shape[2] if w.dim() == 4 else K
    dg_ok = bool(bwd and DGRAD_FWD and _x3() and W_KBLOCKED and w.dim() in (2, 4) and N % 32 == 0 and n_dg % 4 == 0)
# ... 251 lines not shown
    N = w.shape[1]
    if not _fits_buf(M * K * 4):
        return None
    pl = x if isinstance(x, Planes) else None
    mxl = _mx() and "mx" in g
    if pl is None and mxl:
        pl = x = split_planes(x, fmt=1)
    if pl is not None and (not _planes_dp() or K % 32 or (pl.fmt == 1) != mxl):
        raise DdpoHipError("plane-fed linear_geglu needs the bf16x3 / f16mx datapath, K % 32 == 0 and planes of the layer's format "
                           "(ask planes_pay / norm_planes for it)")
    opl = None
    if planes_out:
        if not _planes_dp():
            raise DdpoHipError("plane-emitting linear_geglu needs the bf16x3 / f16mx datapath")
        opl = Planes(M, N // 2, x.device, fmt=1 if planes_out == 2 else 0)
    elif out is None:
        out = torch.empty(M, N // 2, dtype=torch.float32, device=x.device)
    tall = pl is not None and pl.fmt == 0 and geglu_tall_pays(w, M)
    gw = g["tall"] if tall else g
    pre = torch.empty(M, N, dtype=torch.float32, device=x.device) if pre_out else None
    d = _gemm_desc(M, N, K, src=x, ld_src=K, out=None if planes_out else out, ld_out=N // 2, bias=gw["bias"], aux_out=pre,
                   out_planes=opl and (opl.hi, opl.lo, opl.ld, opl.fmt), epilogue=2 if tall else 1)
    with _profiled(2.0 * M * N * K, 4.0 * (M * K + K * N + M * N // 2), _family(mx=mxl)):
        if mxl:
            _launch_fwd(d, pl, g["mx"])
        elif pl is not None:
            _launch_fwd(d, pl, (gw["hi"], gw["lo"], K, 3 if _x3() else 1), w_layout=1 if tall else g["w_layout"])
        else:
            _launch_fwd(d, None, (g["hi"], g["lo"], K, 3 if _x3() else 1), w_layout=g["w_layout"])
    res = opl if planes_out else out
    return (res, pre) if pre_out else res


def _bf16_route(w, K, N, conv, dgrad):
    if current_datapath() == "fp32":
        return None
    ent = PACKED.get(w.data_ptr())
    if ent is None:
        return None
    cin = conv["Cin"] if conv else K
    if cin % 8:
        return None
    npass = 3 if _x3() else 1
    if dgrad:
        if ent["bwd"] is None or not conv:
            return None
        return ent["bwd"][0], ent["bwd"][1], 0, npass
    if ent["K"] != K or ent["N"] != N:
        return None
    return ent["fwd"][0], ent["fwd"][1], ent["fwd"][2], npass


def gemm_conv(src, w, *, M, N, K, bias=None, rowbias=None, rows_per_batch=0, residual=None, out=None, alpha=1.0,
              w_trans=False, ld_src=None, ld_out=None, ld_res=None, conv=None, planes_out=None, planes_fmt=0, res_rows=0):
    pl = src if isinstance(src, Planes) else None
    mxl = (not w_trans) and mx_layer(w)
    if mxl:
        cin_ = conv["Cin"] if conv else K
        rows_ = conv["B"] * conv["H"] * conv["W"] if conv else M
        if not planes_ok(w, cin_, rows_):
            mxl = False
        elif pl is None:
            if not (src.dim() == 2 and src.shape[0] == rows_ and src.shape[1] == cin_ and src.stride(1) == 1 and
                    (ld_src is None or ld_src == src.stride(0))):
                raise DdpoHipError("an f16mx layer needs its fp32 input as a (rows, channels) tensor or row-strided view")
            pl = src = split_planes(src, fmt=1)
            ld_src = None
    if pl is not None and (pl.fmt == 1) != bool(mxl):
        raise DdpoHipError("activation planes of the wrong format for this layer (ask planes_pay / norm_planes: 1 = bf16 hi / lo, 2 = f16mx)")
    opl = None
    if planes_out is not None:
        if planes_out not in ("both", "only"):
            raise ValueError(planes_out)
        opl = Planes(M, N, src.device, fmt=1 if planes_fmt == 2 else 0)
    if out is None and planes_out != "only":
        out = torch.empty(M, N, dtype=torch.float32, device=src.device)
    cin = conv["Cin"] if conv else K
    d = _gemm_desc(M, N, K, conv=conv, src=src, ld_src=ld_src if ld_src is not None else cin, out=out, ld_out=ld_out, bias=bias, residual=residual,
                   ld_res=ld_res, res_rows=res_rows, alpha=alpha, out_planes=opl and (opl.hi, opl.lo, opl.ld, opl.fmt),
                   w=w.data_ptr(), w_trans=int(bool(w_trans)))
    if rowbias is not None:
        d.rowbias = rowbias.data_ptr(); d.rows_per_batch = int(rows_per_batch); d.ld_rowbias = int(rowbias.shape[-1])
    route = None if w_trans else _bf16_route(w, K, N, conv, False)
    if opl is not None and (route is None or not _planes_dp()):
        raise DdpoHipError("a plane-emitting GEMM needs the bf16x3 / f16mx datapath and registered weight planes (check planes_out_ok)")
    if pl is not None and (route is None or not _planes_dp() or cin % 32 or ld_src is not None):
        raise DdpoHipError("a plane-fed GEMM needs the bf16x3 / f16mx datapath, registered weight planes (of the planes' format) and 32-channel "
                           "k-tiles (check planes_ok before asking a producer for planes)")
    a_bytes = 4.0 * (conv["B"] * conv["H"] * conv["W"] * conv["Cin"] if conv else M * K)
    w_bytes = (4.0 if route is None else (4.0 if _x3() else 2.0)) * K * N
    io_bytes = a_bytes + w_bytes + 4.0 * N * (M + (0 if residual is None else (res_rows or M)))
    with _profiled(2.0 * M * N * K, io_bytes, _family(fp32=route is None, mx=mxl)):
        if mxl:
            _launch_fwd(d, pl, PACKED[w.data_ptr()]["mx"], ws_device=src.device)
        elif route is None:
            _launch_fwd(d, None, None)
        else:
            _launch_fwd(d, pl, route, w_layout=PACKED[w.data_ptr()].get("w_layout", 0), ws_device=src.device)
    if planes_out == "only":
        return opl
    return (out, opl) if planes_out == "both" else out


def conv2d(x, w, bias, B, H, W, Cin, Cout, ksize, stride=1, pad=None, upsample=False, **kw):
    conv = _conv_geom(B, H, W, Cin, ksize, stride, pad, upsample)
    out = gemm_conv(x, w, M=B * conv["OH"] * conv["OW"], N=Cout, K=ksize * ksize * Cin, bias=bias, conv=conv, **kw)
    return out, conv["OH"], conv["OW"]


def linear(x, w, bias=None, **kw):
    M, K = x.shape
    N = w.shape[0] if kw.get("w_trans") else w.shape[1]
    return gemm_conv(x, w, M=M, N=N, K=K, bias=bias, **kw)


def attention_planes_ok(d):
    return current_datapath() != "fp32" and _x3() and d in (8, 16, 40, 64, 80)


def attention(q, k, v, B, heads, Nq, Nk, d, scale=None, out=None, ldq=None, ldk=None, ldv=None, ldo=None, return_lse=False, planes_out=False,
              q_batches=None):
    sc = float(scale if scale is not None else d ** -0.5)
    return _attention_shared_q(q, B if q_batches is None else q_batches, k, v, None, B, heads, Nq, Nk, d, sc, out, ldq, ldk, ldv, ldo, return_lse,
                               planes_out)


def _attention_shared_q(q, q_batches, k, v, images, B, heads, Nq, Nk, d, sc, out, ldq, ldk, ldv, ldo, return_lse, planes_out):
    C = heads * d
    x16 = current_datapath() != "fp32" and d in (8, 16, 40, 64, 80)
    if planes_out and (not attention_planes_ok(d) or out is not None or return_lse):
        raise DdpoHipError("plane-emitting attention needs the bf16x3 / f16mx datapath and a supported head dim, and writes planes only")
    opl = Planes(B * Nq, C, q.device) if planes_out else None
    if opl is None and out is None:
        out = torch.empty(B * Nq, C, dtype=torch.float32, device=q.device)
    lse = torch.empty(B * heads * Nq, dtype=torch.float32, device=q.device) if return_lse else None
    o_args = (None, 0, _p(opl.hi), _p(opl.lo), opl.ld) if opl is not None else (_p(out), int(ldo or C), None, None, 0)
    if images is not None:
        _check(load().ddpo_attention_fwd_images_shared_q(int(_mx()), _pr(q, ldq), int(ldq or C), int(q_batches), _p(images), images.numel(), *o_args,
                                                         _p(lse), B, heads, Nq, Nk, d, sc, _stream()), "ddpo_attention_fwd_images_shared_q")
    elif x16:
        nb = int(load().ddpo_attention_fwd_bf16x3_ws_bytes(B, heads, Nk, d))
        ws = _scratch(nb, q.device, "attn_kv") if nb else None
        _check(load().ddpo_attention_fwd_x16_shared_q(int(_mx()), _pr(q, ldq), int(ldq or C), int(q_batches), _pr(k, ldk), int(ldk or C), _pr(v, ldv),
                                                      int(ldv or C), *o_args, _p(lse), B, heads, Nq, Nk, d, sc, _p(ws), nb, _stream()),
               "ddpo_attention_fwd_x16_shared_q")
    else:
        _check(load().ddpo_attention_fwd_shared_q(_pr(q, ldq), int(ldq or C), int(q_batches), _pr(k, ldk), int(ldk or C), _pr(v, ldv), int(ldv or C),
                                                  _p(out), int(ldo or C), _p(lse), B, heads, Nq, Nk, d, sc, _stream()), "ddpo_attention_fwd_shared_q")
    res = opl if opl is not None else out
    return (res, lse) if return_lse else res


CAUSAL_MAX_N = 80

# ... 764 lines not shown
```

### ddpo_amd/models/unet.py

```python
import math
import re
from collections import OrderedDict
from dataclasses import dataclass
from typing import Tuple

import os

import torch

from .. import lib as L


@dataclass(frozen=True)
class UNetConfig:
    in_channels: int = 4
    out_channels: int = 4
    block_out_channels: Tuple[int, ...] = (320, 640, 1280, 1280)
    cross_attn_down: Tuple[bool, ...] = (True, True, True, False)
    layers_per_block: int = 2
    num_heads: Tuple[int, ...] = (8, 8, 8, 8)
    cross_attention_dim: int = 768
    use_linear_projection: bool = False
    norm_groups: int = 32
    prediction_type: str = "epsilon"
# ... 127 lines not shown
        _add_dense(d, f"{tb}.{attn}.to_q", c, c, bias=False)
        _add_dense(d, f"{tb}.{attn}.to_k", kv, c, bias=False)
        _add_dense(d, f"{tb}.{attn}.to_v", kv, c, bias=False)
        _add_dense(d, f"{tb}.{attn}.to_out_0", c, c)
    _add_dense(d, tb + ".ff.net_0.proj", c, 8 * c)
    _add_dense(d, tb + ".ff.net_2", 4 * c, c)
    for n in ("norm1", "norm2", "norm3"):
        _add_norm(d, f"{tb}.{n}", c)
    (_add_dense if linear else lambda dd, n, a, b: _add_conv(dd, n, a, b, 1))(d, name + ".proj_out", c, c)


def unet_param_shapes(cfg: UNetConfig):
    d = OrderedDict()
    boc = cfg.block_out_channels
    nlev = len(boc)
    temb = 4 * boc[0]
    _add_conv(d, "conv_in", cfg.in_channels, boc[0], 3)
    _add_dense(d, "time_embedding.linear_1", boc[0], temb)
    _add_dense(d, "time_embedding.linear_2", temb, temb)
    ch = boc[0]
    for i in range(nlev):
        for j in range(cfg.layers_per_block):
            add_resnet(d, f"down_blocks_{i}.resnets_{j}", ch, boc[i], temb)
            ch = boc[i]
            if cfg.cross_attn_down[i]:
                _add_transformer(d, f"down_blocks_{i}.attentions_{j}", ch, cfg.cross_attention_dim, cfg.use_linear_projection)
        if i < nlev - 1:
            _add_conv(d, f"down_blocks_{i}.downsamplers_0.conv", ch, ch, 3)
    add_resnet(d, "mid_block.resnets_0", ch, ch, temb)
    _add_transformer(d, "mid_block.attentions_0", ch, cfg.cross_attention_dim, cfg.use_linear_projection)
    add_resnet(d, "mid_block.resnets_1", ch, ch, temb)
    rev = boc[::-1]
    for i in range(nlev):
        out_c = rev[i]
        skip_last = rev[min(i + 1, nlev - 1)]
        for j in range(cfg.layers_per_block + 1):
            skip = skip_last if j == cfg.layers_per_block else out_c
            add_resnet(d, f"up_blocks_{i}.resnets_{j}", ch + skip, out_c, temb)
            ch = out_c
            if cfg.cross_attn_down[nlev - 1 - i]:
                _add_transformer(d, f"up_blocks_{i}.attentions_{j}", ch, cfg.cross_attention_dim, cfg.use_linear_projection)
        if i < nlev - 1:
            _add_conv(d, f"up_blocks_{i}.upsamplers_0.conv", ch, ch, 3)
    _add_norm(d, "conv_norm_out", boc[0])
    _add_conv(d, "conv_out", boc[0], cfg.out_channels, 3)
    return d


SKIP_INPLACE = os.environ.get("DDPO_SKIP_INPLACE", "1") == "1"
H3_PLANES = os.environ.get("DDPO_H3_PLANES", "1") == "1"
ATTN_PLANES = os.environ.get("DDPO_ATTN_PLANES", "1") == "1"
CFG_SHARED_FRONT = os.environ.get("DDPO_CFG_SHARED_FRONT", "1") == "1"
QKV_FUSED = os.environ.get("DDPO_QKV_FUSED", "1") == "1"


class Act:
    __slots__ = ("t", "B", "H", "W", "C", "pl")

    def __init__(self, t, B, H, W, C, pl=None):
        self.t, self.B, self.H, self.W, self.C, self.pl = t, B, H, W, C, pl

    @property
    def ld(self):
        return int(self.t.stride(0)) if (self.t.dim() == 2 and self.t.shape[0] > 1 and self.t.stride(0) != self.C) else None

    @property
    def HW(self):
        return self.H * self.W

    @property
    def M(self):
        return self.B * self.H * self.W


def resnet_forward(P, name, x: Act, temb_act, groups, eps, tape=None, emit_planes=0, dest=None):
    cout = P[name + ".conv1.bias"].numel()
    ldx = x.ld
    okw = {} if dest is None else dict(out=dest, ld_out=int(dest.stride(0)))
    pl1 = L.norm_planes(P[name + ".conv1.kernel"], x.C, x.M, tape is not None)
    pl2 = L.norm_planes(P[name + ".conv2.kernel"], cout, x.M, tape is not None)
    h1, st1 = L.groupnorm(x.t, x.B, x.HW, P[name + ".norm1.scale"], P[name + ".norm1.bias"], groups, eps, True, return_stats=True,
                          planes=pl1)
    rowbias, rpb = None, x.HW
    if isinstance(temb_act, dict):
        rowbias, rpb = temb_act[name], x.M
    elif temb_act is not None:
        rowbias = L.linear(temb_act, P[name + ".time_emb_proj.kernel"], P[name + ".time_emb_proj.bias"])
    c1, _, _ = L.conv2d(h1, P[name + ".conv1.kernel"], P[name + ".conv1.bias"], x.B, x.H, x.W, x.C, cout, 3,
                        rowbias=rowbias, rows_per_batch=rpb)
    h2, st2 = L.groupnorm(c1, x.B, x.HW, P[name + ".norm2.scale"], P[name + ".norm2.bias"], groups, eps, True, return_stats=True,
                          planes=pl2)
    res = x.t
    shortcut = (name + ".conv_shortcut.kernel") in P
    if shortcut:
        res, _, _ = L.conv2d(x.t, P[name + ".conv_shortcut.kernel"], P[name + ".conv_shortcut.bias"], x.B, x.H, x.W, x.C, cout, 1,
                             **({} if ldx is None else dict(ld_src=ldx)))
    elif ldx is not None:
        okw["ld_res"] = ldx
    opl = None
    if emit_planes and tape is None and L.planes_out_ok(P[name + ".conv2.kernel"], cout, x.M, cout):
        (out, opl), _, _ = L.conv2d(h2, P[name + ".conv2.kernel"], P[name + ".conv2.bias"], x.B, x.H, x.W, cout, cout, 3, residual=res,
                                    planes_out="both", planes_fmt=emit_planes, **okw)
    else:
        out, _, _ = L.conv2d(h2, P[name + ".conv2.kernel"], P[name + ".conv2.bias"], x.B, x.H, x.W, cout, cout, 3, residual=res, **okw)
    if tape is not None:
        tape.append(("resnet", dict(name=name, x=x, st1=st1, h1=h1, c1=c1, st2=st2, h2=h2, cout=cout, shortcut=shortcut,
                                    temb=temb_act is not None, groups=groups)))
    return Act(out, x.B, x.H, x.W, cout, opl)


class LoraGrads:

    def __init__(self, shapes, device):
        self.shapes = shapes
        cmax = max(s[0] for n, s in shapes.items() if n.endswith(".scale"))
        self.sink = torch.zeros(2, cmax, dtype=torch.float32, device=device)

    def trains(self, name):
        return False

    def __getitem__(self, name):
        stem, leaf = name.rsplit(".", 1)
        if leaf == "scale" or (leaf == "bias" and stem + ".scale" in self.shapes):
            return self.sink[0 if leaf == "scale" else 1, :self.shapes[name][0]]
        raise KeyError(f"{name}: frozen under LoRA (no gradient)")


def _trains(G):
    return not isinstance(G, LoraGrads)


def resnet_backward(P, G, r, d_out, tctx):
    name, x, cout = r["name"], r["x"], r["cout"]
    B, H, W, HW = x.B, x.H, x.W, x.HW
    tr = _trains(G)
    if tr:
        L.conv2d_wgrad(r["h2"], d_out, G[name + ".conv2.kernel"], B, H, W, cout, cout, 3, dbias=G[name + ".conv2.bias"])
    d_h2 = L.conv2d_dgrad(d_out, P[name + ".conv2.kernel"], B, H, W, cout, cout, 3)
    if r["shortcut"]:
        if tr:
            L.conv2d_wgrad(x.t, d_out, G[name + ".conv_shortcut.kernel"], B, H, W, x.C, cout, 1, dbias=G[name + ".conv_shortcut.bias"])
        d_res = L.conv2d_dgrad(d_out, P[name + ".conv_shortcut.kernel"], B, H, W, x.C, cout, 1)
    else:
        d_res = d_out
    d_c1 = L.groupnorm_bwd(r["c1"], d_h2, r["st2"], P[name + ".norm2.scale"], B, HW, r["groups"], True,
                           G[name + ".norm2.scale"], G[name + ".norm2.bias"])
    if tr:
        L.conv2d_wgrad(r["h1"], d_c1, G[name + ".conv1.kernel"], B, H, W, x.C, cout, 3)
        if r["temb"]:
            d_tproj = torch.zeros(B, cout, dtype=torch.float32, device=d_c1.device)
            L.colsum_accum(d_c1, d_tproj, rows_per_seg=HW)
            L.colsum_accum(d_tproj, G[name + ".conv1.bias"])
            L.linear_wgrad(tctx["temb_act"], d_tproj, G[name + ".time_emb_proj.kernel"], dbias=G[name + ".time_emb_proj.bias"])
            tctx["d_temb_act"] = L.linear_dgrad(d_tproj, P[name + ".time_emb_proj.kernel"], residual=tctx["d_temb_act"])
        else:
            L.colsum_accum(d_c1, G[name + ".conv1.bias"])
    d_h1 = L.conv2d_dgrad(d_c1, P[name + ".conv1.kernel"], B, H, W, x.C, cout, 3)
    return L.groupnorm_bwd(x.t, d_h1, r["st1"], P[name + ".norm1.scale"], B, HW, r["groups"], True,
                           G[name + ".norm1.scale"], G[name + ".norm1.bias"], dx_add=d_res)


# ... 20 lines not shown
        if self.grads is None:
            self.grads = ParamStore(self.params.shapes, self.device)
        return self.grads

    def _attention(self, name, x, B, N, C, heads, ctx, ctx_len, rec=None, q_batches=None, plan_B=None):
        P = self.params
        po = bool(rec is None and ATTN_PLANES and L.PLANES_OUT and L.attention_planes_ok(C // heads) and
                  L.planes_pay(P[name + ".to_out_0.kernel"], C, (plan_B or B) * N) == 1)
        qkw = {} if q_batches is None else dict(q_batches=q_batches)
        fq = P.fused_qkv.get(name + ".") if (QKV_FUSED and ctx is None and rec is None and L.current_datapath() != "fp32") else None
        if fq is not None and L.PACKED.get(fq.data_ptr()) is not None:
            qkv = L.linear(x, fq)
            return L.attention(qkv[:, :C], qkv[:, C:2 * C], qkv[:, 2 * C:], B, heads, N, N, C // heads, planes_out=po, ldq=3 * C, ldk=3 * C, ldv=3 * C)
        q = L.linear(x, P[name + ".to_q.kernel"])
        cached = self._ctx_kv.get((name, ctx.shape[0])) if (ctx is not None and rec is None and self._ctx_kv_active) else None
        if cached is not None:
            k, v = cached[0], cached[1]
            if len(cached) > 2 and L.kv_images_valid(cached[2]):
                return L.attention_from_images(q, cached[2], B, heads, N, ctx_len, C // heads, planes_out=po, **qkw)
        else:
            kv_src = x if ctx is None else ctx
            k = L.linear(kv_src, P[name + ".to_k.kernel"])
            v = L.linear(kv_src, P[name + ".to_v.kernel"])
        Nk = N if ctx is None else ctx_len
        if rec is None:
            return L.attention(q, k, v, B, heads, N, Nk, C // heads, planes_out=po, **qkw)
        o, lse = L.attention(q, k, v, B, heads, N, Nk, C // heads, return_lse=True)
        rec.update(q=q, k=k, v=v, o=o, lse=lse, Nk=Nk)
        return o

    def _attention_backward(self, name, rec, x_in, kv_in, d_o, B, N, C, heads, self_attn):
        P, G = self.params, self._grad_view()
        dq, dk, dv = L.attention_bwd(rec["q"], rec["k"], rec["v"], rec["o"], d_o, rec["lse"], B, heads, N, rec["Nk"], C // heads)
        if _trains(G):
            L.linear_wgrad(x_in, dq, G[name + ".to_q.kernel"])
            L.linear_wgrad(kv_in, dk, G[name + ".to_k.kernel"])
            L.linear_wgrad(kv_in, dv, G[name + ".to_v.kernel"])
        else:
            self._lora_wgrad(x_in, dq, name + ".to_q.kernel")
            self._lora_wgrad(kv_in, dk, name + ".to_k.kernel")
            self._lora_wgrad(kv_in, dv, name + ".to_v.kernel")
        d_x = L.linear_dgrad(dq, P[name + ".to_q.kernel"])
        if self_attn:
            d_x = L.linear_dgrad(dk, P[name + ".to_k.kernel"], residual=d_x)
            d_x = L.linear_dgrad(dv, P[name + ".to_v.kernel"], residual=d_x)
        return d_x

    def _lora_wgrad(self, x, dy, kernel_name):
        A, B_, dA, dB = self.lora.layer(kernel_name)
        if isinstance(x, L.Planes) and x.fmt != 0:
            x = x.float()
        L.lora_wgrad(x, dy, A, B_, dA, dB, self.lora.scale)

    def _transformer(self, name, x: Act, ctx, ctx_len, heads, tape=None, emit_planes=0, dest=None, full_B=None):
        P, cfg = self.params, self.cfg
        C, Bx, N = x.C, x.B, x.HW
        B = Bx if full_B is None else full_B
        if full_B is not None and (tape is not None or ctx is None or full_B % Bx):
            raise ValueError("full_B: sampling forward only, a multiple of x.B")
        qb = dict(q_batches=Bx) if B != Bx else {}
        rr = dict(res_rows=Bx * N) if B != Bx else {}
        rec = None if tape is None else dict(name=name, x=x, heads=heads, ctx=ctx, ctx_len=ctx_len)
        tb = name + ".transformer_blocks_0"
        inf = tape is None
        npf = lambda n: L.norm_planes(P[n], C, B * N, not inf)
        pl_in = npf(name + ".proj_in.kernel")
        pl_1 = min(npf(f"{tb}.attn1.{n}.kernel") for n in ("to_q", "to_k", "to_v"))
        if len({npf(f"{tb}.attn1.{n}.kernel") for n in ("to_q", "to_k", "to_v")}) > 1:
            pl_1 = 0
        pl_2 = npf(tb + ".attn2.to_q.kernel")
        pl_3 = npf(tb + ".ff.net_0.proj.kernel")
        if inf and pl_3 != 1 and L.geglu_tall_pays(P[tb + ".ff.net_0.proj.kernel"], B * N):
            pl_3 = 1
        F = P[tb + ".ff.net_2.kernel"].shape[0]
        pl_ff2 = inf and L.PLANES_OUT and L.planes_pay(P[tb + ".ff.net_2.kernel"], F, B * N)
        pl_out = inf and emit_planes and L.planes_out_ok(P[name + ".proj_out.kernel"], C, B * N, C)
        pl_h3 = L.planes_pay(P[name + ".proj_out.kernel"], C, B * N) if inf and L.PLANES_OUT and H3_PLANES else 0
        if pl_h3 and not L.planes_out_ok(P[tb + ".ff.net_2.kernel"], F, B * N, C):
            pl_h3 = 0
        hn, st = L.groupnorm(x.t, Bx, N, P[name + ".norm.scale"], P[name + ".norm.bias"], cfg.norm_groups, 1e-5, False, return_stats=True,
                             planes=pl_in)
        if cfg.use_linear_projection:
            h0 = L.linear(hn, P[name + ".proj_in.kernel"], P[name + ".proj_in.bias"])
        else:
            h0, _, _ = L.conv2d(hn, P[name + ".proj_in.kernel"], P[name + ".proj_in.bias"], Bx, x.H, x.W, C, C, 1)
        ln = lambda n, t, pl=False: L.layernorm(t, P[f"{tb}.{n}.scale"], P[f"{tb}.{n}.bias"], 1e-5, planes=pl)
        a1r = None if rec is None else {}
        a2r = None if rec is None else {}
        l1 = ln("norm1", h0, pl_1)
        a1 = self._attention(tb + ".attn1", l1, Bx, N, C, heads, None, 0, a1r, plan_B=B)
        h1 = L.linear(a1, P[tb + ".attn1.to_out_0.kernel"], P[tb + ".attn1.to_out_0.bias"], residual=h0)
        l2 = ln("norm2", h1, pl_2)
        a2 = self._attention(tb + ".attn2", l2, B, N, C, heads, ctx, ctx_len, a2r, **qb)
        h2 = L.linear(a2, P[tb + ".attn2.to_out_0.kernel"], P[tb + ".attn2.to_out_0.bias"], residual=h1, **rr)
        l3 = ln("norm3", h2, pl_3)
        f = None
        if tape is None:
            gg = L.linear_geglu(l3, P[tb + ".ff.net_0.proj.kernel"], planes_out=pl_ff2)
        else:
            r_ = L.linear_geglu(l3, P[tb + ".ff.net_0.proj.kernel"], pre_out=True)
            gg, f = r_ if r_ is not None else (None, None)
        if gg is None:
            f = L.linear(l3, P[tb + ".ff.net_0.proj.kernel"], P[tb + ".ff.net_0.proj.bias"])
            gg = L.geglu(f)
        h3 = L.linear(gg, P[tb + ".ff.net_2.kernel"], P[tb + ".ff.net_2.bias"], residual=h2,
                      **(dict(planes_out="only", planes_fmt=pl_h3) if pl_h3 else {}))
        po = dict(planes_out="both", planes_fmt=emit_planes) if pl_out else {}
        if dest is not None:
            po.update(out=dest, ld_out=int(dest.stride(0)))
        if x.ld is not None:
            po["ld_res"] = x.ld
        po.update(rr)
        if cfg.use_linear_projection:
            out = L.linear(h3, P[name + ".proj_out.kernel"], P[name + ".proj_out.bias"], residual=x.t, **po)
        else:
            out, _, _ = L.conv2d(h3, P[name + ".proj_out.kernel"], P[name + ".proj_out.bias"], B, x.H, x.W, C, C, 1, residual=x.t, **po)
        out, opl = out if pl_out else (out, None)
        if rec is not None:
            rec.update(st=st, hn=hn, h0=h0, l1=l1, a1r=a1r, h1=h1, l2=l2, a2r=a2r, h2=h2, l3=l3, f=f, gg=gg, h3=h3)
            tape.append(("transformer", rec))
        return Act(out, B, x.H, x.W, C, opl)

    def _transformer_backward(self, r, d_out):
        P, G, cfg = self.params, self._grad_view(), self.cfg
        name, x, heads = r["name"], r["x"], r["heads"]
        C, B, N, H, W = x.C, x.B, x.HW, x.H, x.W
        tb = name + ".transformer_blocks_0"
        gw = lambda n: G[n + ".kernel"]
        tr = _trains(G)
        if cfg.use_linear_projection:
            if tr:
                L.linear_wgrad(r["h3"], d_out, gw(name + ".proj_out"), dbias=G[name + ".proj_out.bias"])
            d_h3 = L.linear_dgrad(d_out, P[name + ".proj_out.kernel"])
        else:
            if tr:
                L.conv2d_wgrad(r["h3"], d_out, gw(name + ".proj_out"), B, H, W, C, C, 1, dbias=G[name + ".proj_out.bias"])
            d_h3 = L.conv2d_dgrad(d_out, P[name + ".proj_out.kernel"], B, H, W, C, C, 1)
        if tr:
            L.linear_wgrad(r["gg"], d_h3, gw(tb + ".ff.net_2"), dbias=G[tb + ".ff.net_2.bias"])
        d_gg = L.linear_dgrad(d_h3, P[tb + ".ff.net_2.kernel"])
        d_f = L.geglu_bwd(r["f"], d_gg)
        if tr:
            L.linear_wgrad(r["l3"], d_f, gw(tb + ".ff.net_0.proj"), dbias=G[tb + ".ff.net_0.proj.bias"])
        d_l3 = L.linear_dgrad(d_f, P[tb + ".ff.net_0.proj.kernel"])
        d_h2 = L.layernorm_bwd(r["h2"], d_l3, P[tb + ".norm3.scale"], G[tb + ".norm3.scale"], G[tb + ".norm3.bias"], 1e-5, dx_add=d_h3)
        if tr:
            L.linear_wgrad(r["a2r"]["o"], d_h2, gw(tb + ".attn2.to_out_0"), dbias=G[tb + ".attn2.to_out_0.bias"])
        else:
            self._lora_wgrad(r["a2r"]["o"], d_h2, tb + ".attn2.to_out_0.kernel")
        d_a2 = L.linear_dgrad(d_h2, P[tb + ".attn2.to_out_0.kernel"])
        d_l2 = self._attention_backward(tb + ".attn2", r["a2r"], r["l2"], r["ctx"], d_a2, B, N, C, heads, False)
        d_h1 = L.layernorm_bwd(r["h1"], d_l2, P[tb + ".norm2.scale"], G[tb + ".norm2.scale"], G[tb + ".norm2.bias"], 1e-5, dx_add=d_h2)
        if tr:
            L.linear_wgrad(r["a1r"]["o"], d_h1, gw(tb + ".attn1.to_out_0"), dbias=G[tb + ".attn1.to_out_0.bias"])
        else:
            self._lora_wgrad(r["a1r"]["o"], d_h1, tb + ".attn1.to_out_0.kernel")
        d_a1 = L.linear_dgrad(d_h1, P[tb + ".attn1.to_out_0.kernel"])
        d_l1 = self._attention_backward(tb + ".attn1", r["a1r"], r["l1"], r["l1"], d_a1, B, N, C, heads, True)
        d_h0 = L.layernorm_bwd(r["h0"], d_l1, P[tb + ".norm1.scale"], G[tb + ".norm1.scale"], G[tb + ".norm1.bias"], 1e-5, dx_add=d_h1)
        if cfg.use_linear_projection:
            if tr:
                L.linear_wgrad(r["hn"], d_h0, gw(name + ".proj_in"), dbias=G[name + ".proj_in.bias"])
            d_hn = L.linear_dgrad(d_h0, P[name + ".proj_in.kernel"])
        else:
            if tr:
                L.conv2d_wgrad(r["hn"], d_h0, gw(name + ".proj_in"), B, H, W, C, C, 1, dbias=G[name + ".proj_in.bias"])
            d_hn = L.conv2d_dgrad(d_h0, P[name + ".proj_in.kernel"], B, H, W, C, C, 1)
        return L.groupnorm_bwd(x.t, d_hn, r["st"], P[name + ".norm.scale"], B, N, cfg.norm_groups, False,
                               G[name + ".norm.scale"], G[name + ".norm.bias"], dx_add=d_out)

    def forward(self, sample, timesteps, context, tape=None, cfg_dup=False):
        P, cfg = self.params, self.cfg
        B, Cin, H, W = sample.shape
        boc = cfg.block_out_channels
# ... 14 lines not shown
        else:
            emb = L.timestep_embedding(timesteps, boc[0])
            t1 = L.linear(emb, P["time_embedding.linear_1.kernel"], P["time_embedding.linear_1.bias"])
            s1 = L.silu(t1)
            temb = L.linear(s1, P["time_embedding.linear_2.kernel"], P["time_embedding.linear_2.bias"])
            temb_act = L.silu(temb)

        dup = bool(cfg_dup) and tape is None and B % 2 == 0 and cfg.cross_attn_down[0]
        Bh = B // 2 if dup else B
        front = dup and CFG_SHARED_FRONT and boc[0] // 32 < L.splitk_min_ktiles()
        def twice(a):
            if not dup:
                return a
            n, c = a.shape
            out2 = torch.empty(2 * n, c, dtype=a.dtype, device=a.device)
            L.copy_cols(a, out2[:n], 0, n, c)
            L.copy_cols(a, out2[n:], 0, n, c)
            return out2
        inplace = tape is None and SKIP_INPLACE
        plan = self._concat_plan() if inplace else None
        cat_bufs = []

        def skip_dest(rows):
            if not inplace:
                return None
            c0, c1 = plan[len(plan) - 1 - len(cat_bufs)]
            buf = torch.empty(rows, c0 + c1, dtype=torch.float32, device=self.device)
            cat_bufs.append(buf)
            return buf[:, c0:]

        def up_dest(k):
            if not inplace or k >= len(plan):
                return None
            return cat_bufs[-1][:, :plan[k][0]]

        x = L.nchw_to_nhwc(sample[:Bh].contiguous())
        d0 = skip_dest(B * H * W)
        if d0 is not None:
            t, _, _ = L.conv2d(x, P["conv_in.kernel"], P["conv_in.bias"], Bh, H, W, Cin, boc[0], 3, out=d0[:Bh * H * W], ld_out=int(d0.stride(0)))
            if dup:
                n0 = Bh * H * W
                L.copy_cols(d0[:n0], d0[n0:], 0, n0, boc[0], ld_src=int(d0.stride(0)), ld_dst=int(d0.stride(0)))
            t_full = d0
        else:
            t, _, _ = L.conv2d(x, P["conv_in.kernel"], P["conv_in.bias"], Bh, H, W, Cin, boc[0], 3)
            t_full = twice(t)
        if tape is not None:
            tape.append(("head", dict(emb=emb, t1=t1, s1=s1, temb=temb, temb_act=temb_act, x=Act(x, B, H, W, Cin))))
        h_half = Act(t, Bh, H, W, boc[0])
        h = Act(t_full, B, H, W, boc[0])
        skips = [h]
        for i in range(nlev):
            for j in range(cfg.layers_per_block):
                if dup and i == 0 and j == 0:
                    r = resnet_forward(P, "down_blocks_0.resnets_0", h_half, temb_act if shared_t else temb_act[:Bh], G, 1e-5, None)
                    h = r if front else Act(twice(r.t), B, r.H, r.W, r.C)
                else:
                    emit = 0
                    if tape is None and i < nlev - 1 and j == cfg.layers_per_block - 1:
                        emit = L.planes_pay(P[f"down_blocks_{i}.downsamplers_0.conv.kernel"], boc[i], h.M)
                    h = resnet_forward(P, f"down_blocks_{i}.resnets_{j}", h, temb_act, G, 1e-5, tape,
                                       emit_planes=0 if cfg.cross_attn_down[i] else emit,
                                       dest=None if cfg.cross_attn_down[i] else skip_dest(h.M))
                if cfg.cross_attn_down[i]:
                    emit_t = 0
                    if tape is None and i < nlev - 1 and j == cfg.layers_per_block - 1:
                        emit_t = L.planes_pay(P[f"down_blocks_{i}.downsamplers_0.conv.kernel"], boc[i], B * h.HW)
                    h = self._transformer(f"down_blocks_{i}.attentions_{j}", h, ctx, Lc, cfg.num_heads[i], tape, emit_planes=emit_t,
                                          dest=skip_dest(B * h.HW), full_B=B if h.B != B else None)
                skips.append(h)
                if tape is not None:
                    tape.append(("skip_push", None))
            if i < nlev - 1:
                name = f"down_blocks_{i}.downsamplers_0.conv"
                src = h.pl if (h.pl is not None and L.planes_pay(P[name + ".kernel"], h.C, h.M) == h.pl.fmt + 1) else h.t
                skw = {} if (src is not h.t or h.ld is None) else dict(ld_src=h.ld)
                dd = skip_dest(B * (h.H // 2) * (h.W // 2))
                if dd is not None:
                    skw.update(out=dd, ld_out=int(dd.stride(0)))
                t, OH, OW = L.conv2d(src, P[name + ".kernel"], P[name + ".bias"], B, h.H, h.W, h.C, h.C, 3, stride=2, pad=1, **skw)
                if tape is not None:
                    tape.append(("down", dict(name=name, x=h)))
                    tape.append(("skip_push", None))
                h = Act(t, B, OH, OW, h.C)
                skips.append(h)
        h = resnet_forward(P, "mid_block.resnets_0", h, temb_act, G, 1e-5, tape)
        h = self._transformer("mid_block.attentions_0", h, ctx, Lc, cfg.num_heads[-1], tape)
        h = resnet_forward(P, "mid_block.resnets_1", h, temb_act, G, 1e-5, tape, dest=up_dest(0))
        kblk = 0
        for i in range(nlev):
            lvl = nlev - 1 - i
            for j in range(cfg.layers_per_block + 1):
                s = skips.pop()
                if inplace:
                    cat = cat_bufs.pop()
                    assert cat.shape == (B * h.HW, h.C + s.C) and h.t.data_ptr() == cat.data_ptr() and s.t.data_ptr() == cat.data_ptr() + 4 * h.C
                else:
                    cat = torch.empty(B * h.HW, h.C + s.C, dtype=torch.float32, device=self.device)
                    L.copy_cols(h.t, cat, 0, B * h.HW, h.C)
                    L.copy_cols(s.t, cat, h.C, B * h.HW, s.C)
                if tape is not None:
                    tape.append(("concat", dict(c0=h.C, c1=s.C)))
                kblk += 1
                emit = 0
                last_of_level = j == cfg.layers_per_block
                if tape is None and i < nlev - 1 and last_of_level:
                    emit = L.up2x_planes_pay(P[f"up_blocks_{i}.upsamplers_0.conv.kernel"], boc[lvl], B * h.HW)
                nxt = None if last_of_level else up_dest(kblk)
                h = resnet_forward(P, f"up_blocks_{i}.resnets_{j}", Act(cat, B, h.H, h.W, h.C + s.C), temb_act, G, 1e-5, tape,
                                   emit_planes=0 if cfg.cross_attn_down[lvl] else emit, dest=None if cfg.cross_attn_down[lvl] else nxt)
                if cfg.cross_attn_down[lvl]:
                    h = self._transformer(f"up_blocks_{i}.attentions_{j}", h, ctx, Lc, cfg.num_heads[lvl], tape, emit_planes=emit, dest=nxt)
            if i < nlev - 1:
                name = f"up_blocks_{i}.upsamplers_0.conv"
                src = h.pl if (h.pl is not None and L.up2x_planes_pay(P[name + ".kernel"], h.C, h.M) == h.pl.fmt + 1) else h.t
                dd = up_dest(kblk)
                dkw = {} if dd is None else dict(out=dd, ld_out=int(dd.stride(0)))
                if L.up2x_fold_ok(P[name + ".kernel"], h.C, h.M):
                    t, OH, OW = L.conv2d_up2x_folded(src, P[name + ".kernel"], P[name + ".bias"], B, h.H, h.W, h.C, h.C, **dkw)
                else:
                    t, OH, OW = L.conv2d(src, P[name + ".kernel"], P[name + ".bias"], B, h.H, h.W, h.C, h.C, 3, upsample=True, **dkw)
                if tape is not None:
                    tape.append(("up", dict(name=name, x=h)))
                h = Act(t, B, OH, OW, h.C)
        hn, st = L.groupnorm(h.t, B, h.HW, P["conv_norm_out.scale"], P["conv_norm_out.bias"], G, 1e-5, True, return_stats=True,
                             planes=L.norm_planes(P["conv_out.kernel"], h.C, h.M, tape is not None) if tape is None else 0)
        t, _, _ = L.conv2d(hn, P["conv_out.kernel"], P["conv_out.bias"], B, h.H, h.W, h.C, cfg.out_channels, 3)
        if tape is not None:
            tape.append(("tail", dict(x=h, hn=hn, st=st)))
        return L.nhwc_to_nchw(t, B, cfg.out_channels, h.H, h.W)

    __call__ = forward

    def _concat_plan(self):
        cfg = self.cfg
        boc = cfg.block_out_channels
        nlev = len(boc)
        pushed = [boc[0]]
        for i in range(nlev):
            pushed += [boc[i]] * cfg.layers_per_block
            if i < nlev - 1:
                pushed.append(boc[i])
        plan, ch, rev = [], boc[-1], boc[::-1]
        for i in range(nlev):
            for _ in range(cfg.layers_per_block + 1):
                plan.append((ch, pushed.pop()))
                ch = rev[i]
        assert not pushed
        return plan

    def cross_attention_names(self):
        return [n[:-len(".to_k.kernel")] for n in self.params.views if n.endswith(".attn2.to_k.kernel")]

    def precompute_context(self, context):
        B, Lc, D = context.shape
        ctx = context.reshape(B * Lc, D).contiguous()
        for name in self.cross_attention_names():
            wk, wv = self.params[name + ".to_k.kernel"], self.params[name + ".to_v.kernel"]
            ent = self._ctx_kv.get((name, B * Lc))
            heads = self._heads_of(name)
            nb = 0
            if L.current_datapath() != "fp32" and (wk.shape[1] // heads) in (8, 16, 40, 64, 80) and os.environ.get("DDPO_CTX_IMAGES", "1") != "0":
                nb = int(L.load().ddpo_attention_kv_images_bytes(B, heads, Lc, wk.shape[1] // heads))
            if ent is None:
                kbuf = torch.empty(B * Lc, wk.shape[1], dtype=torch.float32, device=self.device)
                vbuf = torch.empty(B * Lc, wv.shape[1], dtype=torch.float32, device=self.device)
                ent = (kbuf, vbuf, torch.empty(nb, dtype=torch.uint8, device=self.device) if nb else None)
                self._ctx_kv[(name, B * Lc)] = ent
            elif ent[2] is None and nb:
                ent = (ent[0], ent[1], torch.empty(nb, dtype=torch.uint8, device=self.device))
                self._ctx_kv[(name, B * Lc)] = ent
            L.linear(ctx, wk, out=ent[0])
            L.linear(ctx, wv, out=ent[1])
            if ent[2] is not None:
                L.attention_kv_images(ent[0], ent[1], B, heads, Lc, wk.shape[1] // heads, out=ent[2])
        self._ctx_kv_active = True

    def release_context(self):
# ... 194 lines not shown
```

### include/ddpo_hip.h

```cpp
#ifndef DDPO_HIP_H
#define DDPO_HIP_H
#include <stddef.h>
#include <stdint.h>
#ifdef __cplusplus
extern "C" {
#endif

#define DDPO_OK 0
#define DDPO_EINVAL (-1)
#define DDPO_ELAUNCH (-2)

#define DDPO_PRED_EPSILON 0
#define DDPO_PRED_V 1
#define DDPO_PRED_SAMPLE 2

int ddpo_abi_version(void);
size_t ddpo_sizeof_gemm_desc(void);
size_t ddpo_sizeof_ddim_consts(void);
int ddpo_gemm_tile_launch_counts(unsigned long long* out_host, int n);
int ddpo_gemm_splitk_min_ktiles(void);

int ddpo_threefry_bits_host(uint32_t k0, uint32_t k1, int64_t n, uint32_t* out_host);
int ddpo_threefry_normal(uint32_t k0, uint32_t k1, float* out, uint32_t* bits_out, int64_t n, void* stream);

typedef struct {
  const float* alphas_cumprod;
  int num_train_timesteps;
  int step_ratio;
  float final_alpha_cumprod;
  float eta;
  int pred_type;
} ddpo_ddim_consts;

int ddpo_ddim_step_fwd(const float* eps_u, const float* eps_c, const float* x, const float* z,
                       const int32_t* ts, float guidance_scale, const ddpo_ddim_consts* c,
                       float* x_next, float* logp, int B, int chw, void* stream);

int ddpo_ddim_logprob_ppo_fwd_bwd(const float* eps_c, const float* eps_u, const float* x,
                                  const float* x_next, const int32_t* ts, const float* old_logp,
                                  const float* advantages, float guidance_scale, float clip_range,
                                  int train_cfg, const ddpo_ddim_consts* c, float* d_eps_c,
                                  float* d_eps_u, float* per_sample, float* info, int B, int chw,
                                  void* stream);
int ddpo_ddim_logprob_ppo_fwd_bwd_grouped(const float* eps_c, const float* eps_u, const float* x,
                                          const float* x_next, const int32_t* ts, const float* old_logp,
                                          const float* advantages, float guidance_scale, float clip_range,
                                          int train_cfg, const ddpo_ddim_consts* c, float* d_eps_c,
                                          float* d_eps_u, float* per_sample, float* info, int B, int group,
                                          int chw, void* stream);

int ddpo_rwr_noisy_latents(const float* moments, const float* e1, const float* noise, const int32_t* ts,
                           const float* alphas_cumprod, int num_train_timesteps, float scale, float* latents, float* noisy,
                           int B, int C, int hw, void* stream);
int ddpo_rwr_mse_fwd_bwd(const float* eps_c, const float* eps_u, const float* noise, const float* weights, float guidance_scale,
                         int train_cfg, float* d_eps_c, float* d_eps_u, float* per_sample, float* loss, int B, int chw,
                         void* stream);
int ddpo_grad_sqnorm(const float* g, int64_t n, double* out_sq, int zero_first, void* stream);
int ddpo_adamw_bf16mu_step(float* p, float* g, uint16_t* mu, float* nu, int64_t n,
                           const double* sqnorm_of_sum, double inv_n_acc, double lr, double b1, double b2,
                           double eps, double weight_decay, double max_grad_norm, int step_t,
                           int mu_decay_in_bf16, int zero_grad, void* stream);


size_t ddpo_groupnorm_ws_bytes(int B, int HW, int C, int G);
size_t ddpo_groupnorm_stats_floats(int B, int C, int G);
int ddpo_groupnorm_fwd(const float* x, int ldx, float* y, int ldy, const float* gamma, const float* beta,
                       int B, int HW, int C, int G, float eps, int fuse_silu, void* ws, float* stats, void* stream);
int ddpo_groupnorm_fwd_planes(const float* x, int ldx, uint16_t* y_hi, uint16_t* y_lo, int ldy, const float* gamma,
                              const float* beta, int B, int HW, int C, int G, float eps, int fuse_silu, void* ws,
                              float* stats, void* stream);
size_t ddpo_groupnorm_bwd_ws_bytes(int B, int HW, int C, int G);
int ddpo_groupnorm_bwd(const float* x, int ldx, const float* dy, int lddy, const float* stats, const float* gamma,
                       int B, int HW, int C, int G, int fuse_silu, const float* dx_add, int ld_add, float* dx, int lddx,
                       float* dgamma, float* dbeta, void* ws, void* stream);
int ddpo_layernorm_fwd(const float* x, float* y, const float* gamma, const float* beta, int rows, int C,
                       float eps, void* stream);
int ddpo_layernorm_fwd_planes(const float* x, uint16_t* y_hi, uint16_t* y_lo, const float* gamma, const float* beta,
                              int rows, int C, float eps, int kblocked, void* stream);
size_t ddpo_layernorm_bwd_ws_bytes(int rows, int C);
int ddpo_layernorm_bwd(const float* x, const float* dy, const float* gamma, int rows, int C, float eps,
                       const float* dx_add, float* dx, float* dgamma, float* dbeta, void* ws, void* stream);

typedef struct {
  const float* src; int ld_src;
  const float* w; int w_trans;
  const float* bias;
  const float* rowbias; int rows_per_batch; int ld_rowbias;
  const float* residual; int ld_res;
  float* out; int ld_out;
  float alpha;
  int M, N, K;
  int ksize, stride, pad, upsample;
  int B, H, W, Cin;
  int OH, OW;
  int w_dgrad;
  int ld_w;
  int splits;
  int accumulate;
  int epilogue;
  uint16_t* out_hi; uint16_t* out_lo; int ld_planes;
  int w_layout;
  const uint8_t* w_scale;
  int planes_fmt;
  float* colsum;
  float* aux_out;
  int res_rows;
} ddpo_gemm_desc;
int ddpo_gemm_conv_fwd(const ddpo_gemm_desc* d, void* stream);
int ddpo_gemm_conv_wgrad(const ddpo_gemm_desc* d, void* stream);

int ddpo_gemm_conv_fwd_bf16(const ddpo_gemm_desc* d, const uint16_t* w_hi, const uint16_t* w_lo, int ldw, int npass,
                            void* ws, size_t ws_bytes, void* stream);
int ddpo_gemm_conv_fwd_bf16_planes(const ddpo_gemm_desc* d, const uint16_t* a_hi, const uint16_t* a_lo, int lda,
                                   const uint16_t* w_hi, const uint16_t* w_lo, int ldw, void* ws, size_t ws_bytes,
                                   void* stream);
int ddpo_gemm_conv_fwd_f16mx_planes(const ddpo_gemm_desc* d, const uint16_t* a16, const uint16_t* a8, int lda,
                                    const uint16_t* w16, const uint16_t* w8, void* ws, size_t ws_bytes, void* stream);
int ddpo_fold_up2x_weights(const float* w, int Cin, int Cout, float* wf, void* stream);
int ddpo_conv_up2x_folded_fwd(const ddpo_gemm_desc* d, const uint16_t* a_hi, const uint16_t* a_lo, int lda, const uint16_t* w_hi,
                              const uint16_t* w_lo, int f16mx, void* ws, size_t ws_bytes, void* stream);
int ddpo_pack_weights_f16mx(const float* w, int K, int N, uint16_t* w16, uint16_t* w8, uint8_t* scale, void* stream);
int ddpo_split_planes_f16mx(const float* x, int ldx, uint16_t* p16, uint16_t* p8, int ld_out, int64_t rows, int cols, void* stream);
int ddpo_pack_weights_bf16_kblocked(const float* w, int K, int N, uint16_t* fwd_hi, uint16_t* fwd_lo, void* stream);
int ddpo_pack_weights_bf16_kblocked_dgrad(const float* w, int taps, int Cin, int Cout, uint16_t* hi, uint16_t* lo, void* stream);
int ddpo_split_planes_bf16(const float* x, int ldx, uint16_t* hi, uint16_t* lo, int ld_out, int64_t rows, int cols,
                           void* stream);
int ddpo_gemm_conv_wgrad_bf16x3(const ddpo_gemm_desc* d, void* stream);
int ddpo_gemm_conv_wgrad_bf16x3_planes(const ddpo_gemm_desc* d, const uint16_t* a_hi, const uint16_t* a_lo,
                                       const uint16_t* dy_hi, const uint16_t* dy_lo, void* stream);
int ddpo_pack_weights_bf16(const float* w, int K, int N, int Kp, uint16_t* fwd_hi, uint16_t* fwd_lo,
                           uint16_t* bwd_hi, uint16_t* bwd_lo, void* stream);

int ddpo_attention_fwd(const float* q, int ldq, const float* k, int ldk, const float* v, int ldv,
                       float* o, int ldo, float* lse, int B, int heads, int Nq, int Nk, int d, float scale,
                       void* stream);
size_t ddpo_attention_fwd_bf16x3_ws_bytes(int B, int heads, int Nk, int d);
size_t ddpo_attention_kv_images_bytes(int B, int heads, int Nk, int d);
int ddpo_attention_pack_kv_bf16x3(const float* k, int ldk, const float* v, int ldv, void* images, size_t images_bytes,
                                  int B, int heads, int Nk, int d, void* stream);
int ddpo_attention_fwd_bf16x3_images(const float* q, int ldq, const void* images, size_t images_bytes, float* o, int ldo,
                                     float* lse, int B, int heads, int Nq, int Nk, int d, float scale, void* stream);
int ddpo_attention_fwd_bf16x3(const float* q, int ldq, const float* k, int ldk, const float* v, int ldv,
                              float* o, int ldo, float* lse, int B, int heads, int Nq, int Nk, int d, float scale,
                              void* ws, size_t ws_bytes, void* stream);
int ddpo_attention_bwd(const float* q, int ldq, const float* k, int ldk, const float* v, int ldv, const float* o,
                       const float* d_o, const float* lse, float* dvec, float* dq, float* dk, float* dv,
                       int B, int heads, int Nq, int Nk, int d, float scale, void* stream);

int ddpo_attention_bwd_bf16x3(const float* q, int ldq, const float* k, int ldk, const float* v, int ldv, const float* o,
                              const float* d_o, const float* lse, float* dvec, float* dq, float* dk, float* dv,
                              int B, int heads, int Nq, int Nk, int d, float scale, void* stream);

int ddpo_attention_fwd_f16p(const float* q, int ldq, const float* k, int ldk, const float* v, int ldv,
                            float* o, int ldo, float* lse, int B, int heads, int Nq, int Nk, int d, float scale,
                            void* ws, size_t ws_bytes, void* stream);
int ddpo_attention_pack_kv_f16p(const float* k, int ldk, const float* v, int ldv, void* images, size_t images_bytes, int B, int heads,
                                int Nk, int d, void* stream);
int ddpo_attention_fwd_f16p_images(const float* q, int ldq, const void* images, size_t images_bytes, float* o, int ldo,
                                   float* lse, int B, int heads, int Nq, int Nk, int d, float scale, void* stream);
int ddpo_attention_bwd_f16p(const float* q, int ldq, const float* k, int ldk, const float* v, int ldv, const float* o,
                            const float* d_o, const float* lse, float* dvec, float* dq, float* dk, float* dv,
                            int B, int heads, int Nq, int Nk, int d, float scale, void* stream);


int ddpo_attention_fwd_bf16x3_po(const float* q, int ldq, const float* k, int ldk, const float* v, int ldv, uint16_t* o_hi, uint16_t* o_lo,
                                 int ld_planes, float* lse, int B, int heads, int Nq, int Nk, int d, float scale, void* ws, size_t ws_bytes,
                                 void* stream);
int ddpo_attention_fwd_f16p_po(const float* q, int ldq, const float* k, int ldk, const float* v, int ldv, uint16_t* o_hi, uint16_t* o_lo,
                               int ld_planes, float* lse, int B, int heads, int Nq, int Nk, int d, float scale, void* ws, size_t ws_bytes,
                               void* stream);
// ... 82 lines not shown
```

Before: 4.531 images/sec.

## Fuse GroupNorm column statistics into conv GEMM epilogues

The GEMM epilogue now accumulates per-column sums and sums of squares over 128-row slabs and writes them to a colstats buffer. A following GroupNorm can then build its group mean and variance from these partials instead of making a separate reduction pass over the activation. The U-Net forward passes emit_cs where a GroupNorm follows. The cost is extra epilogue work, an added LDS sync and a small stats write per tile, plus new restrictions that fall back when split-K, folded or generic paths are used.

```diff
diff --git a/ddpo_amd/csrc/common.h b/ddpo_amd/csrc/common.h
--- a/ddpo_amd/csrc/common.h
+++ b/ddpo_amd/csrc/common.h
@@ -89,4 +89,20 @@
   *reinterpret_cast<uint32_t*>(b + 16) = l8;
 }
 
+__device__ __forceinline__ void cs_acc(float4& s, float4& q, const float4 v) {
+  s.x = __fadd_rn(s.x, v.x); s.y = __fadd_rn(s.y, v.y); s.z = __fadd_rn(s.z, v.z); s.w = __fadd_rn(s.w, v.w);
+  q.x = __fadd_rn(q.x, __fmul_rn(v.x, v.x)); q.y = __fadd_rn(q.y, __fmul_rn(v.y, v.y));
+  q.z = __fadd_rn(q.z, __fmul_rn(v.z, v.z)); q.w = __fadd_rn(q.w, __fmul_rn(v.w, v.w));
+}
+__device__ __forceinline__ float4 cs_add(const float4 a, const float4 b) {
+  return make_float4(__fadd_rn(a.x, b.x), __fadd_rn(a.y, b.y), __fadd_rn(a.z, b.z), __fadd_rn(a.w, b.w));
+}
+__device__ __forceinline__ void cs_store_slab(float* __restrict__ o, const float4 (&s)[4], const float4 (&q)[4]) {
+  const float4 a = cs_add(cs_add(cs_add(s[0], s[1]), s[2]), s[3]), b = cs_add(cs_add(cs_add(q[0], q[1]), q[2]), q[3]);
+  *reinterpret_cast<float4*>(o) = make_float4(a.x, b.x, a.y, b.y);
+  *reinterpret_cast<float4*>(o + 4) = make_float4(a.z, b.z, a.w, b.w);
+}
+#define CS_SLAB 128
+#define CS_STRIP 32
+
 static inline hipStream_t as_stream(void* s) { return reinterpret_cast<hipStream_t>(s); }
diff --git a/ddpo_amd/csrc/gemm_bf16.hip b/ddpo_amd/csrc/gemm_bf16.hip
--- a/ddpo_amd/csrc/gemm_bf16.hip
+++ b/ddpo_amd/csrc/gemm_bf16.hip
@@ -181,6 +181,20 @@
       }
     }
   }
+  template <int STRIPS>
+  __device__ __forceinline__ static void strip_sums(const float* cw, int lane, float4& s, float4& q) {
+    static_assert(STRIPS * LPR <= 64, "one lane per column quad and strip");
+    const int l = min(lane, STRIPS * LPR - 1), st = l / LPR;
+    const float* p = cw + st * (CS_STRIP * WTN) + (l - st * LPR) * 4;
+    s = make_float4(0.f, 0.f, 0.f, 0.f); q = s;
+#pragma unroll 4
+    for (int r = 0; r < CS_STRIP; ++r) cs_acc(s, q, *reinterpret_cast<const float4*>(p + r * WTN));
+  }
+  __device__ __forceinline__ static void put_strip_sums(float* cw, int idx, int n, const float4 s, const float4 q) {
+    if (idx >= n) return;
+    reinterpret_cast<float4*>(cw)[2 * idx] = s;
+    reinterpret_cast<float4*>(cw)[2 * idx + 1] = q;
+  }
   __device__ __forceinline__ static void partials(const ddpo_gemm_desc& d, const float* cw, float* pp, int row_base, int col_base, int lane) {
 #pragma unroll
     for (int it = 0; it < NIT; ++it) {
@@ -191,6 +205,42 @@
     }
   }
 };
+
+struct GemmArgs : ddpo_gemm_desc {
+  float* colstats;
+  int ld_colstats;
+};
+
+constexpr size_t CS_ARG_OFF = sizeof(ddpo_gemm_desc);
+static_assert(sizeof(ddpo_gemm_desc) % 8 == 0 && sizeof(GemmArgs) == CS_ARG_OFF + 16, "GemmArgs = the descriptor, a pointer, an int");
+__device__ __forceinline__ void cs_args_late(float*& cs, int& ld) {
+#if defined(__HIP_DEVICE_COMPILE__)
+  const __attribute__((address_space(4))) char* ka = (const __attribute__((address_space(4))) char*)__builtin_amdgcn_kernarg_segment_ptr();
+  asm volatile("" : "+s"(ka));
+  cs = *(float* const __attribute__((address_space(4)))*)(ka + CS_ARG_OFF);
+  ld = *(const __attribute__((address_space(4))) int*)(ka + CS_ARG_OFF + 8);
+#else
+  cs = nullptr; ld = 0;
+#endif
+}
+
+template <int BM, int BN, int WM, int WN, int SLICE>
+__device__ __forceinline__ void cs_write_slabs(const ddpo_gemm_desc& d, float* cs, int ld_cs, const float* sm, int t, int m0, int n0) {
+  constexpr int WTN = BN / WN, LPR = WTN / 4, SPW = BM / WM / CS_STRIP, QT = BN / 4;
+  for (int i = t; i < (BM / CS_SLAB) * QT; i += 64 * WM * WN) {
+    const int slab = i / QT, cqt = i - slab * QT, wn = cqt / LPR, cq = cqt - wn * LPR;
+    const int row0 = m0 + slab * CS_SLAB, col = n0 + cqt * 4;
+    if (row0 >= d.M || col >= d.N) continue;
+    float4 s[4], q[4];
+#pragma unroll
+    for (int k = 0; k < 4; ++k) {
+      const int sg = slab * 4 + k, wm = sg / SPW, sl = sg - wm * SPW;
+      const float4* p = reinterpret_cast<const float4*>(sm + (wm * WN + wn) * SLICE) + 2 * (sl * LPR + cq);
+      s[k] = p[0]; q[k] = p[1];
+    }
+    cs_store_slab(cs + ((int64_t)(row0 / CS_SLAB) * ld_cs + col) * 2, s, q);
+  }
+}
 
 template <int BM, int BN, Datapath DP, bool AFFINE>
 __global__ void __launch_bounds__(BF_THREADS) gemm_conv_bf16_kernel(const ddpo_gemm_desc d, const uint16_t* __restrict__ w_hi,
@@ -456,7 +506,7 @@
 }
 
 template <int BM, int BN, Datapath DP, int WM = 2, int WN = 2, KLoop KL = KLoop::regs, bool FOLD = false>
-__global__ void __launch_bounds__(64 * WM * WN, (BM * BN <= 128 * 64 ? 3 : 1)) gemm_conv_bf16_buf_kernel(const ddpo_gemm_desc d, const uint16_t* __restrict__ w_hi_,
+__global__ void __launch_bounds__(64 * WM * WN, (BM * BN <= 128 * 64 ? 3 : 1)) gemm_conv_bf16_buf_kernel(const GemmArgs d, const uint16_t* __restrict__ w_hi_,
                                                                        const uint16_t* __restrict__ w_lo_, int ldw, int tiles_m,
                                                                        int tiles_n, int nblk, int kt_per_split,
                                                                        float* __restrict__ part) {
@@ -1132,6 +1182,10 @@
         DBG_T(3);
         return;
       }
+      float4 cs_s0, cs_q0, cs_s1, cs_q1;
+      float* csp = nullptr;
+      int ld_cs = 0;
+      if constexpr (!FOLD) cs_args_late(csp, ld_cs);
       auto pass = [&](auto IH) {
         constexpr int ih = decltype(IH)::value;
         const int rowb = m0 + wm * WTM + ih * 32;
@@ -1146,11 +1200,25 @@
         } else {
           if (ih == 0) { ep.init(d, colb, lane); ep.fetch(d, 0, rowb, colb, lane); }
           ep.combine_all(d, cw, rowb, colb, lane);
+          if constexpr (!FOLD) {
+            if (csp) {
+              if constexpr (ih == 0) Epi::template strip_sums<1>(cw, lane, cs_s0, cs_q0);
+              else Epi::template strip_sums<1>(cw, lane, cs_s1, cs_q1);
+            }
+          }
           Epi::template emit<FOLD>(d, cw, rowb, colb, lane, ph);
         }
       };
       pass(std::integral_constant<int, 0>{});
       pass(std::integral_constant<int, 1>{});
+      if constexpr (!FOLD) {
+        if (csp) {
+          Epi::put_strip_sums(cw, lane, LPR, cs_s0, cs_q0);
+          Epi::put_strip_sums(cw, LPR + lane, 2 * LPR, cs_s1, cs_q1);
+          __syncthreads();
+          cs_write_slabs<BM, BN, WM, WN, 32 * WTN>(d, csp, ld_cs, reinterpret_cast<const float*>(smem), t, m0, n0);
+        }
+      }
       DBG_T(3);
       return;
     }
@@ -1203,7 +1271,18 @@
       Epi::partials(d, cw, part + ((int64_t)ph * gridDim.y + blockIdx.y) * d.M * d.N, rowb, colb, lane);
     } else {
       ep.combine_all(d, cw, rowb, colb, lane);
+      constexpr int SPW = BM == 256 ? 1 : WTM / CS_STRIP;
+      float* csp = nullptr;
+      int ld_cs = 0;
+      if constexpr (!FOLD) cs_args_late(csp, ld_cs);
+      float4 cs_s, cs_q;
+      if (csp) Epi::template strip_sums<SPW>(cw, lane, cs_s, cs_q);
       Epi::template emit<FOLD>(d, cw, rowb, colb, lane, ph);
+      if (csp) {
+        Epi::put_strip_sums(cw, lane, SPW * LPR, cs_s, cs_q);
+        __syncthreads();
+        cs_write_slabs<BM, BN, WM, WN, WTM * WTN>(d, csp, ld_cs, reinterpret_cast<const float*>(smem), t, m0, n0);
+      }
     }
     DBG_T(3);
     return;
@@ -1296,6 +1375,13 @@
   return true;
 }
 
+static bool colstats_ok(const GemmArgs& d) {
+  if (d.epilogue != 0 || d.w_dgrad || (d.M % CS_SLAB) || (d.N & 3) || d.ld_colstats < d.N || (d.ld_colstats & 3)) return false;
+  if ((reinterpret_cast<uintptr_t>(d.colstats) | reinterpret_cast<uintptr_t>(d.out) | reinterpret_cast<uintptr_t>(d.bias)) & 15) return false;
+  if ((d.ld_out & 3) || (d.residual && ((d.ld_res & 3) || (reinterpret_cast<uintptr_t>(d.residual) & 15)))) return false;
+  return !d.rowbias || ((d.ld_rowbias & 3) == 0 && (reinterpret_cast<uintptr_t>(d.rowbias) & 15) == 0);
+}
+
 enum { TC_TALL = 0, TC_WIDE = 1, TC_128 = 2, TC_64 = 3, TC_GENERIC = 4, TC_SPLITK_REDUCE = 5, TC_MX = 6, TC_COUNT = 8 };
 static unsigned long long g_tile_launches[TC_COUNT] = {0, 0, 0, 0, 0, 0, 0, 0};
 extern "C" int ddpo_gemm_tile_launch_counts(unsigned long long* out_host, int n) {
@@ -1391,7 +1477,7 @@
 }
 
 template <class T, Datapath DP, KLoop KL, bool FOLD>
-static int launch_tile(const ddpo_gemm_desc& d, const uint16_t* w_hi, const uint16_t* w_lo, int ldw, float* ws, int splits, hipStream_t st) {
+static int launch_tile(const GemmArgs& d, const uint16_t* w_hi, const uint16_t* w_lo, int ldw, float* ws, int splits, hipStream_t st) {
   if constexpr (!kernel_exists<T, DP, KL, FOLD>()) {
     return DDPO_EINVAL;
   } else {
@@ -1405,6 +1491,9 @@
     if (!T::SPLITK) splits = 1;
     const int ktps = T::SPLITK ? ktiles_per_split(nk_total, splits) : nk_total;
     float* part = splits > 1 ? ws : nullptr;
+    bool generic = false;
+    if constexpr (GENERIC) generic = !buf_path_ok(d, ldw);
+    if (d.colstats && (FOLD || splits > 1 || generic)) return DDPO_EINVAL;
     static bool attr_set = false;
     if (!attr_set) {
       if constexpr (GENERIC) {
@@ -1416,8 +1505,6 @@
     }
     count_tile(T::TC);
     if constexpr (DP == Datapath::f16mx) count_tile(TC_MX);
-    bool generic = false;
-    if constexpr (GENERIC) generic = !buf_path_ok(d, ldw);
     if (!generic) {
       hipLaunchKernelGGL(kernel, dim3(nblk, splits, NPH), dim3(64 * T::WM * T::WN), lds, st, d, w_hi, w_lo, ldw, tiles_m, tiles_n, nblk, ktps, part);
     } else if constexpr (GENERIC) {
@@ -1436,7 +1523,7 @@
 struct Route { RouteTile tile; int splits; };
 
 template <bool PLANES, bool FOLD, Datapath DP>
-static int launch_route(const Route& r, const ddpo_gemm_desc& d, const uint16_t* w_hi, const uint16_t* w_lo, int ldw, float* ws, hipStream_t st) {
+static int launch_route(const Route& r, const GemmArgs& d, const uint16_t* w_hi, const uint16_t* w_lo, int ldw, float* ws, hipStream_t st) {
   constexpr KLoop KL = PLANES ? KLoop::planes3w : KLoop::regs;
   constexpr KLoop KT = !PLANES ? KLoop::regs : (DP == Datapath::bf16x3 ? KLoop::tall : (DP == Datapath::f16mx ? KLoop::tall_mx : KLoop::tall_ring));
   switch (r.tile) {
@@ -1448,7 +1535,7 @@
   }
 }
 template <bool PLANES, bool FOLD>
-static int launch_npass(int npass, const Route& r, const ddpo_gemm_desc& d, const uint16_t* w_hi, const uint16_t* w_lo, int ldw, float* ws, hipStream_t st) {
+static int launch_npass(int npass, const Route& r, const GemmArgs& d, const uint16_t* w_hi, const uint16_t* w_lo, int ldw, float* ws, hipStream_t st) {
   switch (npass) {
     case 1: return launch_route<PLANES, FOLD, Datapath::bf16x1>(r, d, w_hi, w_lo, ldw, ws, st);
     case 3: return launch_route<PLANES, FOLD, Datapath::bf16x3>(r, d, w_hi, w_lo, ldw, ws, st);
@@ -1459,10 +1546,11 @@
 }
 
 template <bool PLANES, bool FOLD = false>
-static int dispatch_bf16(const ddpo_gemm_desc& d, const uint16_t* w_hi, const uint16_t* w_lo, int ldw, int npass, void* ws, size_t ws_bytes,
+static int dispatch_bf16(const GemmArgs& d, const uint16_t* w_hi, const uint16_t* w_lo, int ldw, int npass, void* ws, size_t ws_bytes,
                          hipStream_t st) {
   static_assert(!FOLD || PLANES, "folded up-sampler phases exist on the plane-fed kernels");
   constexpr int NPH = FOLD ? 4 : 1;
+  if (d.colstats && !colstats_ok(d)) return DDPO_EINVAL;
   if (FOLD && (d.epilogue != 0 || (npass != 1 && npass != 3 && npass != 4))) return DDPO_EINVAL;
   if (d.epilogue != 0) {
     if ((d.epilogue != 1 && d.epilogue != 2) || (d.N & 127) || !buf_path_ok(d, ldw) || d.rowbias || d.residual || d.alpha != 1.0f || d.w_dgrad) return DDPO_EINVAL;
@@ -1506,10 +1594,10 @@
   return true;
 }
 
-extern "C" int ddpo_gemm_conv_fwd_bf16(const ddpo_gemm_desc* dp, const uint16_t* w_hi, const uint16_t* w_lo, int ldw, int npass,
-                                       void* ws, size_t ws_bytes, void* stream) {
+static int fwd_bf16(const ddpo_gemm_desc* dp, const uint16_t* w_hi, const uint16_t* w_lo, int ldw, int npass, void* ws, size_t ws_bytes,
+                    float* colstats, int ld_colstats, void* stream) {
   if (!dp || !w_hi) return DDPO_EINVAL;
-  const ddpo_gemm_desc& d = *dp;
+  const GemmArgs d{*dp, colstats, colstats ? ld_colstats : 0};
   if (npass != 1 && npass != 3) return DDPO_EINVAL;
   if (npass == 3 && !w_lo) return DDPO_EINVAL;
   if (!d.src || d.ld_src <= 0 || (d.ld_src & 3) || (reinterpret_cast<uintptr_t>(d.src) & 15)) return DDPO_EINVAL;
@@ -1524,6 +1612,14 @@
   }
   return dispatch_bf16<false>(d, w_hi, w_lo, ldw, npass, ws, ws_bytes, as_stream(stream));
 }
+extern "C" int ddpo_gemm_conv_fwd_bf16(const ddpo_gemm_desc* dp, const uint16_t* w_hi, const uint16_t* w_lo, int ldw, int npass,
+                                       void* ws, size_t ws_bytes, void* stream) {
+  return fwd_bf16(dp, w_hi, w_lo, ldw, npass, ws, ws_bytes, nullptr, 0, stream);
+}
+extern "C" int ddpo_gemm_conv_fwd_bf16_cs(const ddpo_gemm_desc* dp, const uint16_t* w_hi, const uint16_t* w_lo, int ldw, int npass,
+                                          void* ws, size_t ws_bytes, float* colstats, int ld_colstats, void* stream) {
+  return fwd_bf16(dp, w_hi, w_lo, ldw, npass, ws, ws_bytes, colstats, ld_colstats, stream);
+}
 
 static bool plane_operands_ok(ddpo_gemm_desc& d, const uint16_t* a0, const uint16_t* a1, int lda, int lda_mult, const uint16_t* w0, const uint16_t* w1, int ldw) {
   if (!a0 || !w0 || (a1 == nullptr) != (w1 == nullptr)) return false;
@@ -1536,12 +1632,11 @@
   return buf_path_ok(d, ldw);
 }
 
-extern "C" int ddpo_gemm_conv_fwd_bf16_planes(const ddpo_gemm_desc* dp, const uint16_t* a_hi, const uint16_t* a_lo, int lda,
-                                              const uint16_t* w_hi, const uint16_t* w_lo, int ldw, void* ws, size_t ws_bytes,
-                                              void* stream) {
+static int fwd_bf16_planes(const ddpo_gemm_desc* dp, const uint16_t* a_hi, const uint16_t* a_lo, int lda, const uint16_t* w_hi,
+                           const uint16_t* w_lo, int ldw, void* ws, size_t ws_bytes, float* colstats, int ld_colstats, void* stream) {
   if (!dp) return DDPO_EINVAL;
   const int npass = a_lo ? 3 : 1;
-  ddpo_gemm_desc d = *dp;
+  GemmArgs d{*dp, colstats, colstats ? ld_colstats : 0};
   if (!conv_geometry_ok(d) || d.w_dgrad || (d.w_layout != 0 && d.w_layout != 1)) return DDPO_EINVAL;
   if (d.w_layout == 0 && (ldw < d.K || (ldw & 7))) return DDPO_EINVAL;
   if (npass == 1 && d.epilogue == 2) return DDPO_EINVAL;
@@ -1549,25 +1644,44 @@
   dbg_abl_from_env(d);
   return dispatch_bf16<true>(d, w_hi, w_lo, ldw, npass, ws, ws_bytes, as_stream(stream));
 }
-
-extern "C" int ddpo_gemm_conv_fwd_f16mx_planes(const ddpo_gemm_desc* dp, const uint16_t* a16, const uint16_t* a8, int lda,
-                                               const uint16_t* w16, const uint16_t* w8, void* ws, size_t ws_bytes, void* stream) {
+extern "C" int ddpo_gemm_conv_fwd_bf16_planes(const ddpo_gemm_desc* dp, const uint16_t* a_hi, const uint16_t* a_lo, int lda,
+                                              const uint16_t* w_hi, const uint16_t* w_lo, int ldw, void* ws, size_t ws_bytes,
+                                              void* stream) {
+  return fwd_bf16_planes(dp, a_hi, a_lo, lda, w_hi, w_lo, ldw, ws, ws_bytes, nullptr, 0, stream);
+}
+extern "C" int ddpo_gemm_conv_fwd_bf16_planes_cs(const ddpo_gemm_desc* dp, const uint16_t* a_hi, const uint16_t* a_lo, int lda,
+                                                 const uint16_t* w_hi, const uint16_t* w_lo, int ldw, void* ws, size_t ws_bytes,
+                                                 float* colstats, int ld_colstats, void* stream) {
+  return fwd_bf16_planes(dp, a_hi, a_lo, lda, w_hi, w_lo, ldw, ws, ws_bytes, colstats, ld_colstats, stream);
+}
+
+static int fwd_f16mx_planes(const ddpo_gemm_desc* dp, const uint16_t* a16, const uint16_t* a8, int lda, const uint16_t* w16, const uint16_t* w8,
+                            void* ws, size_t ws_bytes, float* colstats, int ld_colstats, void* stream) {
   if (!dp || (a8 && !dp->w_scale)) return DDPO_EINVAL;
   const int npass = a8 ? 4 : 5;
-  ddpo_gemm_desc d = *dp;
+  GemmArgs d{*dp, colstats, colstats ? ld_colstats : 0};
   if (!conv_geometry_ok(d) || d.w_dgrad || d.w_layout != 1) return DDPO_EINVAL;
   if (npass == 5 && d.epilogue == 2) return DDPO_EINVAL;
   if (!plane_operands_ok(d, a16, a8, lda, 32, w16, w8, 0)) return DDPO_EINVAL;
   dbg_abl_from_env(d);
   return dispatch_bf16<true>(d, w16, w8, 0, npass, ws, ws_bytes, as_stream(stream));
 }
+extern "C" int ddpo_gemm_conv_fwd_f16mx_planes(const ddpo_gemm_desc* dp, const uint16_t* a16, const uint16_t* a8, int lda,
+                                               const uint16_t* w16, const uint16_t* w8, void* ws, size_t ws_bytes, void* stream) {
+  return fwd_f16mx_planes(dp, a16, a8, lda, w16, w8, ws, ws_bytes, nullptr, 0, stream);
+}
+extern "C" int ddpo_gemm_conv_fwd_f16mx_planes_cs(const ddpo_gemm_desc* dp, const uint16_t* a16, const uint16_t* a8, int lda,
+                                                  const uint16_t* w16, const uint16_t* w8, void* ws, size_t ws_bytes,
+                                                  float* colstats, int ld_colstats, void* stream) {
+  return fwd_f16mx_planes(dp, a16, a8, lda, w16, w8, ws, ws_bytes, colstats, ld_colstats, stream);
+}
 
 extern "C" int ddpo_conv_up2x_folded_fwd(const ddpo_gemm_desc* dp, const uint16_t* a_hi, const uint16_t* a_lo, int lda, const uint16_t* w_hi,
                                          const uint16_t* w_lo, int f16mx, void* ws, size_t ws_bytes, void* stream) {
   if (!dp) return DDPO_EINVAL;
   if (f16mx && (!a_lo || !dp->w_scale)) return DDPO_EINVAL;
   const int npass = f16mx ? 4 : (a_lo ? 3 : 1);
-  ddpo_gemm_desc d = *dp;
+  GemmArgs d{*dp, nullptr, 0};
   if (d.B <= 0 || d.H <= 0 || d.W <= 0 || d.Cin <= 0 || d.N <= 0 || (d.Cin % BF_BK) || (d.N & 3)) return DDPO_EINVAL;
   if ((int64_t)d.B * d.H * d.W * 4 > 0x7FFFFFFF || (int64_t)d.Cin * 4 > 0x7FFFFFFF) return DDPO_EINVAL;
   if (!d.out || d.out_hi || d.out_lo || d.rowbias || d.residual || d.res_rows || d.epilogue || d.w_dgrad || d.aux_out) return DDPO_EINVAL;
diff --git a/ddpo_amd/csrc/norm.hip b/ddpo_amd/csrc/norm.hip
--- a/ddpo_amd/csrc/norm.hip
+++ b/ddpo_amd/csrc/norm.hip
@@ -226,6 +226,9 @@
 }
 extern "C" size_t ddpo_groupnorm_stats_floats(int B, int C, int G) { return (size_t)B * C * 2 + (size_t)B * G * 2; }
 
+static int gn_launch_apply(const float* x, int ldx, float* y, uint16_t* y_hi, uint16_t* y_lo, int ldy, const float* ab, int B, int HW, int C,
+                           bool planes, bool mx, int fuse_silu, hipStream_t st);
+
 static int groupnorm_fwd_impl(const float* x, int ldx, float* y, uint16_t* y_hi, uint16_t* y_lo, int ldy, const float* gamma,
                               const float* beta, int B, int HW, int C, int G, float eps, int fuse_silu, void* ws, float* stats,
                               void* stream) {
@@ -241,7 +244,6 @@
   if (planes ? ((reinterpret_cast<uintptr_t>(y_hi) | reinterpret_cast<uintptr_t>(y_lo)) & 7) != 0 : (reinterpret_cast<uintptr_t>(y) & 15) != 0)
     return DDPO_EINVAL;
   hipStream_t st = as_stream(stream);
-  const int C4 = C >> 2;
   const int ppb = gn_ppb(C);
   const int chunks = (HW + ppb - 1) / ppb;
   double* part = reinterpret_cast<double*>(ws);
@@ -262,6 +264,12 @@
   DDPO_LAUNCH_CHECK();
   hipLaunchKernelGGL(gn_finalize_kernel, dim3(B * G), dim3(64), 0, st, part, gamma, beta, ab, mr, chunks, C, G, HW, eps);
   DDPO_LAUNCH_CHECK();
+  return gn_launch_apply(x, ldx, y, y_hi, y_lo, ldy, ab, B, HW, C, planes, mx, fuse_silu, st);
+}
+
+static int gn_launch_apply(const float* x, int ldx, float* y, uint16_t* y_hi, uint16_t* y_lo, int ldy, const float* ab, int B, int HW, int C,
+                           bool planes, bool mx, int fuse_silu, hipStream_t st) {
+  const int C4 = C >> 2;
   int64_t blocks = ((int64_t)B * HW * C4 + 255) / 256;
   if (blocks > 16384) blocks = 16384;
   uint16_t* const no = nullptr;
@@ -292,6 +300,99 @@
                                          float* stats, void* stream) {
   if (!y_hi || !y_lo) return DDPO_EINVAL;
   return groupnorm_fwd_impl(x, ldx, nullptr, y_hi, y_lo, ldy, gamma, beta, B, HW, C, G, eps, fuse_silu, ws, stats, stream);
+}
+
+__global__ void __launch_bounds__(256) colstats_kernel(const float* __restrict__ x, int ldx, int C, float* __restrict__ cs, int ld_cs) {
+  __shared__ float4 s_s[4][64], s_q[4][64];
+  const int lane = threadIdx.x & 63, strip = threadIdx.x >> 6;
+  const int cq = blockIdx.x * 64 + lane;
+  const bool on = cq < (C >> 2);
+  const int64_t slab = blockIdx.y;
+  float4 s = make_float4(0.f, 0.f, 0.f, 0.f), q = s;
+  if (on) {
+    const float* p = x + (slab * CS_SLAB + strip * CS_STRIP) * ldx + (cq << 2);
+#pragma unroll 8
+    for (int r = 0; r < CS_STRIP; ++r) cs_acc(s, q, *reinterpret_cast<const float4*>(p + (int64_t)r * ldx));
+  }
+  s_s[strip][lane] = s; s_q[strip][lane] = q;
+  __syncthreads();
+  if (strip == 0 && on) {
+    const float4 a[4] = {s_s[0][lane], s_s[1][lane], s_s[2][lane], s_s[3][lane]}, b[4] = {s_q[0][lane], s_q[1][lane], s_q[2][lane], s_q[3][lane]};
+    cs_store_slab(cs + (slab * ld_cs + (cq << 2)) * 2, a, b);
+  }
+}
+
+static bool colstats_args_ok(const void* cs, int ld_cs, int64_t M, int C) {
+  return cs && !(reinterpret_cast<uintptr_t>(cs) & 15) && M > 0 && M % CS_SLAB == 0 && M / CS_SLAB <= 65535 && C > 0 && !(C & 3) && ld_cs >= C && !(ld_cs & 3);
+}
+
+extern "C" int ddpo_colstats(const float* x, int ldx, int M, int C, float* colstats, int ld_cs, void* stream) {
+  if (!x || (reinterpret_cast<uintptr_t>(x) & 15) || ldx < C || (ldx & 3) || !colstats_args_ok(colstats, ld_cs, M, C)) return DDPO_EINVAL;
+  hipLaunchKernelGGL(colstats_kernel, dim3(((C >> 2) + 63) / 64, M / CS_SLAB), dim3(256), 0, as_stream(stream), x, ldx, C, colstats, ld_cs);
+  DDPO_LAUNCH_CHECK();
+  return DDPO_OK;
+}
+
+__global__ void __launch_bounds__(64) gn_finalize_cs_kernel(const float* __restrict__ cs, int ld_cs, const float* __restrict__ gamma,
+                                                            const float* __restrict__ beta, float* __restrict__ ab, float* __restrict__ mr,
+                                                            int C, int G, int HW, float eps) {
+  const int b = blockIdx.x / G, g = blockIdx.x - b * G;
+  const int lane = threadIdx.x;
+  const int cpg = C / G, slabs = HW / CS_SLAB, n = slabs * cpg;
+  double a = 0.0, q = 0.0;
+  for (int i = lane; i < n; i += 64) {
+    const int sl = i / cpg, c = g * cpg + (i - sl * cpg);
+    const float2 v = *reinterpret_cast<const float2*>(cs + (((int64_t)b * slabs + sl) * ld_cs + c) * 2);
+    a += (double)v.x; q += (double)v.y;
+  }
+  a = wave_sum_d(a); q = wave_sum_d(q);
+  const double cnt = (double)cpg * (double)HW;
+  const double mean = a / cnt;
+  double var = q / cnt - mean * mean;
+  if (var < 0.0) var = 0.0;
+  const float rstd = (float)(1.0 / sqrt(var + (double)eps));
+  if (lane == 0) { mr[2 * blockIdx.x] = (float)mean; mr[2 * blockIdx.x + 1] = rstd; }
+  for (int c = g * cpg + lane; c < (g + 1) * cpg; c += 64) {
+    const float k = rstd * gamma[c];
+    ab[2 * ((int64_t)b * C + c)] = k;
+    ab[2 * ((int64_t)b * C + c) + 1] = beta[c] - (float)mean * k;
+  }
+}
+
+static int groupnorm_fwd_cs_impl(const float* x, int ldx, const float* cs, int ld_cs, float* y, uint16_t* y_hi, uint16_t* y_lo, int ldy,
+                                 const float* gamma, const float* beta, int B, int HW, int C, int G, float eps, int fuse_silu, float* stats,
+                                 void* stream) {
+  const bool planes = y == nullptr;
+  const bool mx = (fuse_silu & 2) != 0;
+  fuse_silu &= 1;
+  if (mx && (!planes || (C & 31) || (ldy & 31))) return DDPO_EINVAL;
+  if (!x || !gamma || !beta || !stats || B <= 0 || HW <= 0 || C <= 0 || G <= 0 || G > GN_MAXG) return DDPO_EINVAL;
+  if (planes && (!y_hi || !y_lo)) return DDPO_EINVAL;
+  if ((C & 3) || (C % G) || (ldx & 3) || (ldy & 3) || C > GN_MAXC || B > 65535 || (HW % CS_SLAB)) return DDPO_EINVAL;
+  if (!colstats_args_ok(cs, ld_cs, (int64_t)B * HW, C)) return DDPO_EINVAL;
+  if (ldy == 0 && (!planes || (C & 31))) return DDPO_EINVAL;
+  if ((reinterpret_cast<uintptr_t>(x) | reinterpret_cast<uintptr_t>(stats)) & 15) return DDPO_EINVAL;
+  if (planes ? ((reinterpret_cast<uintptr_t>(y_hi) | reinterpret_cast<uintptr_t>(y_lo)) & 7) != 0 : (reinterpret_cast<uintptr_t>(y) & 15) != 0)
+    return DDPO_EINVAL;
+  hipStream_t st = as_stream(stream);
+  float* ab = stats;
+  float* mr = stats + (size_t)B * C * 2;
+  hipLaunchKernelGGL(gn_finalize_cs_kernel, dim3(B * G), dim3(64), 0, st, cs, ld_cs, gamma, beta, ab, mr, C, G, HW, eps);
+  DDPO_LAUNCH_CHECK();
+  return gn_launch_apply(x, ldx, y, y_hi, y_lo, ldy, ab, B, HW, C, planes, mx, fuse_silu, st);
+}
+
+extern "C" int ddpo_groupnorm_fwd_cs(const float* x, int ldx, const float* colstats, int ld_cs, float* y, int ldy, const float* gamma,
+                                     const float* beta, int B, int HW, int C, int G, float eps, int fuse_silu, float* stats, void* stream) {
+  if (!y) return DDPO_EINVAL;
+  return groupnorm_fwd_cs_impl(x, ldx, colstats, ld_cs, y, nullptr, nullptr, ldy, gamma, beta, B, HW, C, G, eps, fuse_silu, stats, stream);
+}
+
+extern "C" int ddpo_groupnorm_fwd_planes_cs(const float* x, int ldx, const float* colstats, int ld_cs, uint16_t* y_hi, uint16_t* y_lo, int ldy,
+                                            const float* gamma, const float* beta, int B, int HW, int C, int G, float eps, int fuse_silu,
+                                            float* stats, void* stream) {
+  if (!y_hi || !y_lo) return DDPO_EINVAL;
+  return groupnorm_fwd_cs_impl(x, ldx, colstats, ld_cs, nullptr, y_hi, y_lo, ldy, gamma, beta, B, HW, C, G, eps, fuse_silu, stats, stream);
 }
 
 #define LN_MAXV 10
diff --git a/ddpo_amd/lib.py b/ddpo_amd/lib.py
--- a/ddpo_amd/lib.py
+++ b/ddpo_amd/lib.py
@@ -86,6 +86,16 @@
     "ddpo_pack_weights_f16mx": (c_int, [c_void_p, c_int, c_int, c_void_p, c_void_p, c_void_p, c_void_p]),
     "ddpo_split_planes_f16mx": (c_int, [c_void_p, c_int, c_void_p, c_void_p, c_int, c_int64, c_int, c_void_p]),
     "ddpo_gemm_conv_fwd_f16mx_planes": (c_int, [POINTER(GemmDesc), c_void_p, c_void_p, c_int, c_void_p, c_void_p, c_void_p, c_size_t, c_void_p]),
+    "ddpo_gemm_conv_fwd_bf16_cs": (c_int, [POINTER(GemmDesc), c_void_p, c_void_p, c_int, c_int, c_void_p, c_size_t, c_void_p, c_int, c_void_p]),
+    "ddpo_gemm_conv_fwd_bf16_planes_cs": (c_int, [POINTER(GemmDesc), c_void_p, c_void_p, c_int, c_void_p, c_void_p, c_int, c_void_p, c_size_t,
+                                                  c_void_p, c_int, c_void_p]),
+    "ddpo_gemm_conv_fwd_f16mx_planes_cs": (c_int, [POINTER(GemmDesc), c_void_p, c_void_p, c_int, c_void_p, c_void_p, c_void_p, c_size_t,
+                                                   c_void_p, c_int, c_void_p]),
+    "ddpo_colstats": (c_int, [c_void_p, c_int, c_int, c_int, c_void_p, c_int, c_void_p]),
+    "ddpo_groupnorm_fwd_cs": (c_int, [c_void_p, c_int, c_void_p, c_int, c_void_p, c_int, c_void_p, c_void_p, c_int, c_int, c_int, c_int,
+                                      c_float, c_int, c_void_p, c_void_p]),
+    "ddpo_groupnorm_fwd_planes_cs": (c_int, [c_void_p, c_int, c_void_p, c_int, c_void_p, c_void_p, c_int, c_void_p, c_void_p, c_int, c_int, c_int,
+                                             c_int, c_float, c_int, c_void_p, c_void_p]),
     "ddpo_fold_up2x_weights": (c_int, [c_void_p, c_int, c_int, c_void_p, c_void_p]),
     "ddpo_conv_up2x_folded_fwd": (c_int, [POINTER(GemmDesc), c_void_p, c_void_p, c_int, c_void_p, c_void_p, c_int, c_void_p, c_size_t, c_void_p]),
     "ddpo_attention_fwd": (c_int, [c_void_p, c_int, c_void_p, c_int, c_void_p, c_int, c_void_p, c_int, c_void_p, c_int, c_int,
@@ -605,11 +615,30 @@
     return d
 
 
-def _launch_fwd(d, act, weights, *, w_layout=0, cross=None, ws_device=None, tag=""):
+def _launch_fwd(d, act, weights, *, w_layout=0, cross=None, ws_device=None, tag="", colstats=None):
     lib = load()
     a_hi, a_lo, a_ld = (act.hi, act.lo, act.ld) if isinstance(act, Planes) else (act or (None, None, 0))
     ws = None if ws_device is None else _scratch(SPLITK_WS_BYTES, ws_device, "splitk")
     ws_args = (_p(ws), SPLITK_WS_BYTES if ws is not None else 0, _stream())
+    if colstats is not None and weights is not None:
+        cs_args = ws_args[:2] + (colstats[0], int(colstats[1]), ws_args[2])
+        if isinstance(weights, dict):
+            cross = MX_CROSS if cross is None else cross
+            d.w_layout = 1
+            d.w_scale = weights["scale"].data_ptr()
+            rc = lib.ddpo_gemm_conv_fwd_f16mx_planes_cs(byref(d), _p(a_hi), _p(a_lo) if cross else None, a_ld, _p(weights["w16"]),
+                                                        _p(weights["w8"]) if cross else None, *cs_args)
+        else:
+            hi, lo, ldw, npass = weights
+            d.w_layout = w_layout
+            if a_hi is None:
+                rc = lib.ddpo_gemm_conv_fwd_bf16_cs(byref(d), _p(hi), _p(lo), ldw, npass, *cs_args)
+            else:
+                one = npass == 1
+                rc = lib.ddpo_gemm_conv_fwd_bf16_planes_cs(byref(d), _p(a_hi), None if one else _p(a_lo), a_ld, _p(hi), None if one else _p(lo), ldw,
+                                                           *cs_args)
+        if rc == 0:
+            return True
     if weights is None:
         name, rc = "ddpo_gemm_conv_fwd", lib.ddpo_gemm_conv_fwd(byref(d), _stream())
     elif isinstance(weights, dict):
@@ -628,6 +657,7 @@
             name, rc = "ddpo_gemm_conv_fwd_bf16_planes", lib.ddpo_gemm_conv_fwd_bf16_planes(
                 byref(d), _p(a_hi), None if one else _p(a_lo), a_ld, _p(hi), None if one else _p(lo), ldw, *ws_args)
     _check(rc, name + tag)
+    return False
 
 
 def _family(fp32=False, mx=False):
@@ -646,10 +676,59 @@
     PROFILE.append((e0, e1, flops, family, io_bytes))
 
 
-def groupnorm(x, B, HW, gamma, beta, groups, eps, silu, out=None, ld_x=None, ld_out=None, return_stats=False, planes=False):
+def colstats_ok(HW, C):
+    return HW % 128 == 0 and C % 4 == 0
+
+
+class ColStats:
+    __slots__ = ("t", "c0", "C", "emitted")
+
+    def __init__(self, t, c0, C):
+        self.t, self.c0, self.C, self.emitted = t, c0, C, None
+
+    @classmethod
+    def empty(cls, rows, C, device):
+        return cls(torch.empty(rows // 128, C, 2, dtype=torch.float32, device=device), 0, C)
+
+    @property
+    def ld(self):
+        return int(self.t.shape[1])
+
+    @property
+    def ptr(self):
+        return c_void_p(self.t.data_ptr() + 8 * self.c0)
+
+
+def column_stats(x, cs=None, ld_x=None):
+    M, C = x.shape
+    if ld_x is None and x.stride(0) != C:
+        ld_x = x.stride(0)
+    if cs is None:
+        cs = ColStats.empty(M, C, x.device)
+    _check(load().ddpo_colstats(_pr(x, ld_x), int(ld_x or C), M, C, cs.ptr, cs.ld, _stream()), "ddpo_colstats")
+    cs.emitted = False
+    return cs
+
+
+def groupnorm(x, B, HW, gamma, beta, groups, eps, silu, out=None, ld_x=None, ld_out=None, return_stats=False, planes=False, colstats=None):
     C = gamma.numel()
     if ld_x is None and x.dim() == 2 and x.stride(0) != C:
         ld_x = x.stride(0)
+    if colstats is not None:
+        if colstats.C != C or colstats.t.shape[0] * 128 != B * HW:
+            raise DdpoHipError("colstats of another activation")
+        stats = torch.empty(load().ddpo_groupnorm_stats_floats(B, C, groups), dtype=torch.float32, device=x.device)
+        if planes:
+            pl = Planes(B * HW, C, x.device, fmt=1 if planes == 2 else 0)
+            _check(load().ddpo_groupnorm_fwd_planes_cs(_pr(x, ld_x), int(ld_x or C), colstats.ptr, colstats.ld, _p(pl.hi), _p(pl.lo), pl.ld, _p(gamma),
+                                                       _p(beta), B, HW, C, groups, float(eps), int(bool(silu)) | (2 * pl.fmt), _p(stats), _stream()),
+                   "ddpo_groupnorm_fwd_planes_cs")
+            return (pl, stats) if return_stats else pl
+        if out is None:
+            out = torch.empty(B * HW, C, dtype=torch.float32, device=x.device)
+        _check(load().ddpo_groupnorm_fwd_cs(_pr(x, ld_x), int(ld_x or C), colstats.ptr, colstats.ld, _p(out), int(ld_out or C), _p(gamma), _p(beta),
+                                            B, HW, C, groups, float(eps), int(bool(silu)), _p(stats), _stream()), "ddpo_groupnorm_fwd_cs")
+        return (out, stats) if return_stats else out
     if planes:
         pl = Planes(B * HW, C, x.device, fmt=1 if planes == 2 else 0)
         ws = _scratch(load().ddpo_groupnorm_ws_bytes(B, HW, C, groups), x.device, "gn")
@@ -1007,7 +1086,7 @@
 
 
 def gemm_conv(src, w, *, M, N, K, bias=None, rowbias=None, rows_per_batch=0, residual=None, out=None, alpha=1.0,
-              w_trans=False, ld_src=None, ld_out=None, ld_res=None, conv=None, planes_out=None, planes_fmt=0, res_rows=0):
+              w_trans=False, ld_src=None, ld_out=None, ld_res=None, conv=None, planes_out=None, planes_fmt=0, res_rows=0, colstats=None):
     pl = src if isinstance(src, Planes) else None
     mxl = (not w_trans) and mx_layer(w)
     if mxl:
@@ -1030,6 +1109,14 @@
         opl = Planes(M, N, src.device, fmt=1 if planes_fmt == 2 else 0)
     if out is None and planes_out != "only":
         out = torch.empty(M, N, dtype=torch.float32, device=src.device)
+    cs = None
+    if colstats is not None and colstats is not False:
+        if planes_out == "only" or M % 128 or N % 4:
+            raise DdpoHipError("colstats need the fp32 result, whole 128-row slabs and channel quads")
+        cs = ColStats.empty(M, N, src.device) if colstats is True else colstats
+        if cs.C != N or cs.t.shape[0] * 128 != M:
+            raise DdpoHipError("colstats buffer of another geometry")
+    csa = None if cs is None else (cs.ptr, cs.ld)
     cin = conv["Cin"] if conv else K
     d = _gemm_desc(M, N, K, conv=conv, src=src, ld_src=ld_src if ld_src is not None else cin, out=out, ld_out=ld_out, bias=bias, residual=residual,
                    ld_res=ld_res, res_rows=res_rows, alpha=alpha, out_planes=opl and (opl.hi, opl.lo, opl.ld, opl.fmt),
@@ -1047,14 +1134,20 @@
     io_bytes = a_bytes + w_bytes + 4.0 * N * (M + (0 if residual is None else (res_rows or M)))
     with _profiled(2.0 * M * N * K, io_bytes, _family(fp32=route is None, mx=mxl)):
         if mxl:
-            _launch_fwd(d, pl, PACKED[w.data_ptr()]["mx"], ws_device=src.device)
+            emitted = _launch_fwd(d, pl, PACKED[w.data_ptr()]["mx"], ws_device=src.device, colstats=csa)
         elif route is None:
-            _launch_fwd(d, None, None)
+            emitted = _launch_fwd(d, None, None)
         else:
-            _launch_fwd(d, pl, route, w_layout=PACKED[w.data_ptr()].get("w_layout", 0), ws_device=src.device)
+            emitted = _launch_fwd(d, pl, route, w_layout=PACKED[w.data_ptr()].get("w_layout", 0), ws_device=src.device, colstats=csa)
     if planes_out == "only":
         return opl
-    return (out, opl) if planes_out == "both" else out
+    res = (out, opl) if planes_out == "both" else out
+    if cs is None:
+        return res
+    cs.emitted = emitted
+    if not emitted:
+        column_stats(out, cs)
+    return res, cs
 
 
 def conv2d(x, w, bias, B, H, W, Cin, Cout, ksize, stride=1, pad=None, upsample=False, **kw):
diff --git a/ddpo_amd/models/unet.py b/ddpo_amd/models/unet.py
--- a/ddpo_amd/models/unet.py
+++ b/ddpo_amd/models/unet.py
@@ -203,13 +203,18 @@
 ATTN_PLANES = os.environ.get("DDPO_ATTN_PLANES", "1") == "1"
 CFG_SHARED_FRONT = os.environ.get("DDPO_CFG_SHARED_FRONT", "1") == "1"
 QKV_FUSED = os.environ.get("DDPO_QKV_FUSED", "1") == "1"
+GN_COLSTATS = os.environ.get("DDPO_GN_COLSTATS", "1") == "1"
+
+
+def gn_colstats(HW, C):
+    return GN_COLSTATS and L._planes_dp() and HW > 256 and L.colstats_ok(HW, C)
 
 
 class Act:
-    __slots__ = ("t", "B", "H", "W", "C", "pl")
-
-    def __init__(self, t, B, H, W, C, pl=None):
-        self.t, self.B, self.H, self.W, self.C, self.pl = t, B, H, W, C, pl
+    __slots__ = ("t", "B", "H", "W", "C", "pl", "cs")
+
+    def __init__(self, t, B, H, W, C, pl=None, cs=None):
+        self.t, self.B, self.H, self.W, self.C, self.pl, self.cs = t, B, H, W, C, pl, cs
 
     @property
     def ld(self):
@@ -224,23 +229,25 @@
         return self.B * self.H * self.W
 
 
-def resnet_forward(P, name, x: Act, temb_act, groups, eps, tape=None, emit_planes=0, dest=None):
+def resnet_forward(P, name, x: Act, temb_act, groups, eps, tape=None, emit_planes=0, dest=None, emit_cs=False):
     cout = P[name + ".conv1.bias"].numel()
     ldx = x.ld
     okw = {} if dest is None else dict(out=dest, ld_out=int(dest.stride(0)))
     pl1 = L.norm_planes(P[name + ".conv1.kernel"], x.C, x.M, tape is not None)
     pl2 = L.norm_planes(P[name + ".conv2.kernel"], cout, x.M, tape is not None)
     h1, st1 = L.groupnorm(x.t, x.B, x.HW, P[name + ".norm1.scale"], P[name + ".norm1.bias"], groups, eps, True, return_stats=True,
-                          planes=pl1)
+                          planes=pl1, colstats=x.cs)
+    cs1 = gn_colstats(x.HW, cout)
     rowbias, rpb = None, x.HW
     if isinstance(temb_act, dict):
         rowbias, rpb = temb_act[name], x.M
     elif temb_act is not None:
         rowbias = L.linear(temb_act, P[name + ".time_emb_proj.kernel"], P[name + ".time_emb_proj.bias"])
     c1, _, _ = L.conv2d(h1, P[name + ".conv1.kernel"], P[name + ".conv1.bias"], x.B, x.H, x.W, x.C, cout, 3,
-                        rowbias=rowbias, rows_per_batch=rpb)
+                        rowbias=rowbias, rows_per_batch=rpb, **(dict(colstats=True) if cs1 else {}))
+    c1, cs1 = c1 if cs1 else (c1, None)
     h2, st2 = L.groupnorm(c1, x.B, x.HW, P[name + ".norm2.scale"], P[name + ".norm2.bias"], groups, eps, True, return_stats=True,
-                          planes=pl2)
+                          planes=pl2, colstats=cs1)
     res = x.t
     shortcut = (name + ".conv_shortcut.kernel") in P
     if shortcut:
@@ -248,16 +255,21 @@
                              **({} if ldx is None else dict(ld_src=ldx)))
     elif ldx is not None:
         okw["ld_res"] = ldx
-    opl = None
+    opl = ocs = None
+    if emit_cs and gn_colstats(x.HW, cout):
+        okw["colstats"] = True
     if emit_planes and tape is None and L.planes_out_ok(P[name + ".conv2.kernel"], cout, x.M, cout):
-        (out, opl), _, _ = L.conv2d(h2, P[name + ".conv2.kernel"], P[name + ".conv2.bias"], x.B, x.H, x.W, cout, cout, 3, residual=res,
-                                    planes_out="both", planes_fmt=emit_planes, **okw)
+        out, _, _ = L.conv2d(h2, P[name + ".conv2.kernel"], P[name + ".conv2.bias"], x.B, x.H, x.W, cout, cout, 3, residual=res,
+                             planes_out="both", planes_fmt=emit_planes, **okw)
+        out, ocs = out if "colstats" in okw else (out, None)
+        out, opl = out
     else:
         out, _, _ = L.conv2d(h2, P[name + ".conv2.kernel"], P[name + ".conv2.bias"], x.B, x.H, x.W, cout, cout, 3, residual=res, **okw)
+        out, ocs = out if "colstats" in okw else (out, None)
     if tape is not None:
         tape.append(("resnet", dict(name=name, x=x, st1=st1, h1=h1, c1=c1, st2=st2, h2=h2, cout=cout, shortcut=shortcut,
                                     temb=temb_act is not None, groups=groups)))
-    return Act(out, x.B, x.H, x.W, cout, opl)
+    return Act(out, x.B, x.H, x.W, cout, opl, ocs)
 
 
 class LoraGrads:
@@ -384,7 +396,7 @@
             x = x.float()
         L.lora_wgrad(x, dy, A, B_, dA, dB, self.lora.scale)
 
-    def _transformer(self, name, x: Act, ctx, ctx_len, heads, tape=None, emit_planes=0, dest=None, full_B=None):
+    def _transformer(self, name, x: Act, ctx, ctx_len, heads, tape=None, emit_planes=0, dest=None, full_B=None, emit_cs=False):
         P, cfg = self.params, self.cfg
         C, Bx, N = x.C, x.B, x.HW
         B = Bx if full_B is None else full_B
@@ -411,7 +423,7 @@
         if pl_h3 and not L.planes_out_ok(P[tb + ".ff.net_2.kernel"], F, B * N, C):
             pl_h3 = 0
         hn, st = L.groupnorm(x.t, Bx, N, P[name + ".norm.scale"], P[name + ".norm.bias"], cfg.norm_groups, 1e-5, False, return_stats=True,
-                             planes=pl_in)
+                             planes=pl_in, colstats=x.cs)
         if cfg.use_linear_projection:
             h0 = L.linear(hn, P[name + ".proj_in.kernel"], P[name + ".proj_in.bias"])
         else:
@@ -443,15 +455,19 @@
         if x.ld is not None:
             po["ld_res"] = x.ld
         po.update(rr)
+        ecs = emit_cs and gn_colstats(N, C)
+        if ecs:
+            po["colstats"] = True
         if cfg.use_linear_projection:
             out = L.linear(h3, P[name + ".proj_out.kernel"], P[name + ".proj_out.bias"], residual=x.t, **po)
         else:
             out, _, _ = L.conv2d(h3, P[name + ".proj_out.kernel"], P[name + ".proj_out.bias"], B, x.H, x.W, C, C, 1, residual=x.t, **po)
+        out, ocs = out if ecs else (out, None)
         out, opl = out if pl_out else (out, None)
         if rec is not None:
             rec.update(st=st, hn=hn, h0=h0, l1=l1, a1r=a1r, h1=h1, l2=l2, a2r=a2r, h2=h2, l3=l3, f=f, gg=gg, h3=h3)
             tape.append(("transformer", rec))
-        return Act(out, B, x.H, x.W, C, opl)
+        return Act(out, B, x.H, x.W, C, opl, ocs)
 
     def _transformer_backward(self, r, d_out):
         P, G, cfg = self.params, self._grad_view(), self.cfg
@@ -572,22 +588,26 @@
         skips = [h]
         for i in range(nlev):
             for j in range(cfg.layers_per_block):
+                gn_next = j < cfg.layers_per_block - 1 or i == nlev - 1
                 if dup and i == 0 and j == 0:
-                    r = resnet_forward(P, "down_blocks_0.resnets_0", h_half, temb_act if shared_t else temb_act[:Bh], G, 1e-5, None)
+                    r = resnet_forward(P, "down_blocks_0.resnets_0", h_half, temb_act if shared_t else temb_act[:Bh], G, 1e-5, None, emit_cs=True)
                     h = r if front else Act(twice(r.t), B, r.H, r.W, r.C)
+                    if not front and r.cs is not None:
+                        h.cs = L.column_stats(h.t)
                 else:
                     emit = 0
                     if tape is None and i < nlev - 1 and j == cfg.layers_per_block - 1:
                         emit = L.planes_pay(P[f"down_blocks_{i}.downsamplers_0.conv.kernel"], boc[i], h.M)
                     h = resnet_forward(P, f"down_blocks_{i}.resnets_{j}", h, temb_act, G, 1e-5, tape,
                                        emit_planes=0 if cfg.cross_attn_down[i] else emit,
-                                       dest=None if cfg.cross_attn_down[i] else skip_dest(h.M))
+                                       dest=None if cfg.cross_attn_down[i] else skip_dest(h.M),
+                                       emit_cs=cfg.cross_attn_down[i] or gn_next)
                 if cfg.cross_attn_down[i]:
                     emit_t = 0
                     if tape is None and i < nlev - 1 and j == cfg.layers_per_block - 1:
                         emit_t = L.planes_pay(P[f"down_blocks_{i}.downsamplers_0.conv.kernel"], boc[i], B * h.HW)
                     h = self._transformer(f"down_blocks_{i}.attentions_{j}", h, ctx, Lc, cfg.num_heads[i], tape, emit_planes=emit_t,
-                                          dest=skip_dest(B * h.HW), full_B=B if h.B != B else None)
+                                          dest=skip_dest(B * h.HW), full_B=B if h.B != B else None, emit_cs=gn_next)
                 skips.append(h)
                 if tape is not None:
                     tape.append(("skip_push", None))
@@ -598,14 +618,18 @@
                 dd = skip_dest(B * (h.H // 2) * (h.W // 2))
                 if dd is not None:
                     skw.update(out=dd, ld_out=int(dd.stride(0)))
+                dcs = gn_colstats((h.H // 2) * (h.W // 2), h.C)
+                if dcs:
+                    skw["colstats"] = True
                 t, OH, OW = L.conv2d(src, P[name + ".kernel"], P[name + ".bias"], B, h.H, h.W, h.C, h.C, 3, stride=2, pad=1, **skw)
+                t, dcs = t if dcs else (t, None)
                 if tape is not None:
                     tape.append(("down", dict(name=name, x=h)))
                     tape.append(("skip_push", None))
-                h = Act(t, B, OH, OW, h.C)
+                h = Act(t, B, OH, OW, h.C, cs=dcs)
                 skips.append(h)
-        h = resnet_forward(P, "mid_block.resnets_0", h, temb_act, G, 1e-5, tape)
-        h = self._transformer("mid_block.attentions_0", h, ctx, Lc, cfg.num_heads[-1], tape)
+        h = resnet_forward(P, "mid_block.resnets_0", h, temb_act, G, 1e-5, tape, emit_cs=True)
+        h = self._transformer("mid_block.attentions_0", h, ctx, Lc, cfg.num_heads[-1], tape, emit_cs=True)
         h = resnet_forward(P, "mid_block.resnets_1", h, temb_act, G, 1e-5, tape, dest=up_dest(0))
         kblk = 0
         for i in range(nlev):
@@ -627,10 +651,13 @@
                 if tape is None and i < nlev - 1 and last_of_level:
                     emit = L.up2x_planes_pay(P[f"up_blocks_{i}.upsamplers_0.conv.kernel"], boc[lvl], B * h.HW)
                 nxt = None if last_of_level else up_dest(kblk)
+                gn_next = last_of_level and i == nlev - 1
                 h = resnet_forward(P, f"up_blocks_{i}.resnets_{j}", Act(cat, B, h.H, h.W, h.C + s.C), temb_act, G, 1e-5, tape,
-                                   emit_planes=0 if cfg.cross_attn_down[lvl] else emit, dest=None if cfg.cross_attn_down[lvl] else nxt)
+                                   emit_planes=0 if cfg.cross_attn_down[lvl] else emit, dest=None if cfg.cross_attn_down[lvl] else nxt,
+                                   emit_cs=cfg.cross_attn_down[lvl] or gn_next)
                 if cfg.cross_attn_down[lvl]:
-                    h = self._transformer(f"up_blocks_{i}.attentions_{j}", h, ctx, Lc, cfg.num_heads[lvl], tape, emit_planes=emit, dest=nxt)
+                    h = self._transformer(f"up_blocks_{i}.attentions_{j}", h, ctx, Lc, cfg.num_heads[lvl], tape, emit_planes=emit, dest=nxt,
+                                          emit_cs=gn_next)
             if i < nlev - 1:
                 name = f"up_blocks_{i}.upsamplers_0.conv"
                 src = h.pl if (h.pl is not None and L.up2x_planes_pay(P[name + ".kernel"], h.C, h.M) == h.pl.fmt + 1) else h.t
@@ -643,7 +670,7 @@
                 if tape is not None:
                     tape.append(("up", dict(name=name, x=h)))
                 h = Act(t, B, OH, OW, h.C)
-        hn, st = L.groupnorm(h.t, B, h.HW, P["conv_norm_out.scale"], P["conv_norm_out.bias"], G, 1e-5, True, return_stats=True,
+        hn, st = L.groupnorm(h.t, B, h.HW, P["conv_norm_out.scale"], P["conv_norm_out.bias"], G, 1e-5, True, return_stats=True, colstats=h.cs,
                              planes=L.norm_planes(P["conv_out.kernel"], h.C, h.M, tape is not None) if tape is None else 0)
         t, _, _ = L.conv2d(hn, P["conv_out.kernel"], P["conv_out.bias"], B, h.H, h.W, h.C, cfg.out_channels, 3)
         if tape is not None:
diff --git a/include/ddpo_hip.h b/include/ddpo_hip.h
--- a/include/ddpo_hip.h
+++ b/include/ddpo_hip.h
@@ -69,6 +69,12 @@
 int ddpo_groupnorm_fwd_planes(const float* x, int ldx, uint16_t* y_hi, uint16_t* y_lo, int ldy, const float* gamma,
                               const float* beta, int B, int HW, int C, int G, float eps, int fuse_silu, void* ws,
                               float* stats, void* stream);
+int ddpo_colstats(const float* x, int ldx, int M, int C, float* colstats, int ld_cs, void* stream);
+int ddpo_groupnorm_fwd_cs(const float* x, int ldx, const float* colstats, int ld_cs, float* y, int ldy, const float* gamma,
+                          const float* beta, int B, int HW, int C, int G, float eps, int fuse_silu, float* stats, void* stream);
+int ddpo_groupnorm_fwd_planes_cs(const float* x, int ldx, const float* colstats, int ld_cs, uint16_t* y_hi, uint16_t* y_lo, int ldy,
+                                 const float* gamma, const float* beta, int B, int HW, int C, int G, float eps, int fuse_silu,
+                                 float* stats, void* stream);
 size_t ddpo_groupnorm_bwd_ws_bytes(int B, int HW, int C, int G);
 int ddpo_groupnorm_bwd(const float* x, int ldx, const float* dy, int lddy, const float* stats, const float* gamma,
                        int B, int HW, int C, int G, int fuse_silu, const float* dx_add, int ld_add, float* dx, int lddx,
@@ -116,6 +122,14 @@
                                    void* stream);
 int ddpo_gemm_conv_fwd_f16mx_planes(const ddpo_gemm_desc* d, const uint16_t* a16, const uint16_t* a8, int lda,
                                     const uint16_t* w16, const uint16_t* w8, void* ws, size_t ws_bytes, void* stream);
+int ddpo_gemm_conv_fwd_bf16_cs(const ddpo_gemm_desc* d, const uint16_t* w_hi, const uint16_t* w_lo, int ldw, int npass,
+                               void* ws, size_t ws_bytes, float* colstats, int ld_colstats, void* stream);
+int ddpo_gemm_conv_fwd_bf16_planes_cs(const ddpo_gemm_desc* d, const uint16_t* a_hi, const uint16_t* a_lo, int lda,
+                                      const uint16_t* w_hi, const uint16_t* w_lo, int ldw, void* ws, size_t ws_bytes,
+                                      float* colstats, int ld_colstats, void* stream);
+int ddpo_gemm_conv_fwd_f16mx_planes_cs(const ddpo_gemm_desc* d, const uint16_t* a16, const uint16_t* a8, int lda,
+                                       const uint16_t* w16, const uint16_t* w8, void* ws, size_t ws_bytes,
+                                       float* colstats, int ld_colstats, void* stream);
 int ddpo_fold_up2x_weights(const float* w, int Cin, int Cout, float* wf, void* stream);
 int ddpo_conv_up2x_folded_fwd(const ddpo_gemm_desc* d, const uint16_t* a_hi, const uint16_t* a_lo, int lda, const uint16_t* w_hi,
                               const uint16_t* w_lo, int f16mx, void* ws, size_t ws_bytes, void* stream);
```

After: 4.570 images/sec, median of 6. No clear change (+0.9%).
